# clintpgeorge/LDAGroupedGibbsSampler

Measured on AMD Instinct MI355X. Metric: M tokens sampled/sec (whole node) per Gibbs sweep at K=100, higher is better.
Workload: dtype f64

## Files before the change

include/ggs_hip.h:

```cpp
#ifndef GGS_HIP_H
#define GGS_HIP_H

#include <stdint.h>

#ifdef __cplusplus
extern "C" {
#endif

#define GGS_ABI_VERSION 6

typedef struct ggs_handle ggs_handle;

enum {
  GGS_OK = 0,
  GGS_ERR_NEGATIVE_COUNT = 1,
  GGS_ERR_INVALID_TOPIC = 2,
  GGS_ERR_RNG_EXHAUSTED = 3,
  GGS_ERR_BAD_ARG = 4,
  GGS_ERR_HIP = 5,
  GGS_ERR_STATE = 6,
  GGS_ERR_UNSUPPORTED = 7,
  GGS_ERR_INVARIANT = 8
};

// ... 38 lines not shown
} ggs_config;

typedef struct ggs_timings {
  double theta_ms;
  double z_ms;
  double merge_ms;
  double phi_ms;
  int64_t sweeps;
  int64_t tokens_sampled;
  double exchange_ms;
  double exchange_rs_ms;
  double exchange_ag_ms;
} ggs_timings;

int ggs_create(const ggs_config *cfg, ggs_handle **out);
void ggs_destroy(ggs_handle *h);
const char *ggs_last_error(const ggs_handle *h);
int ggs_abi_version(void);
int ggs_set_stream(ggs_handle *h, void *hip_stream);

int ggs_set_corpus(ggs_handle *h, int64_t num_docs, const int64_t *doc_ptr ,
                   const int32_t *tokens , int64_t doc_base, int64_t tok_base);
int ggs_init_z_java_lcg(ggs_handle *h, int32_t seed);
int ggs_java_lcg_next_ints(int32_t seed, int32_t bound, int64_t n, int32_t *out);
int ggs_set_z(ggs_handle *h, const int32_t *z , int32_t redraw_phi);
int ggs_init_phi(ggs_handle *h);
int ggs_set_iteration(ggs_handle *h, int32_t iteration);
int ggs_get_iteration(const ggs_handle *h, int32_t *iteration);

int ggs_sweep(ggs_handle *h, int32_t n_sweeps);
int ggs_sweep_begin(ggs_handle *h);
int ggs_sweep_end(ggs_handle *h);
int ggs_sweep_end_async(ggs_handle *h);
int ggs_collapsed_serial_sweep(ggs_handle *h, int32_t java_seed, int32_t n_sweeps);
int ggs_sample_z_given_phi(ggs_handle *h, int32_t n_sweeps);
int ggs_counts_device_ptr(ggs_handle *h, void **dev_ptr, int64_t *num_elems);
int ggs_set_global_token_count(ggs_handle *h, int64_t n_tokens);
int ggs_synchronize(ggs_handle *h);

typedef struct ggs_exchange_ops {
  int32_t struct_size;
  int32_t reserved;
  void *ctx;
  int (*reduce_scatter_i32)(void *ctx, const void *send, void *recv, int64_t recv_count, void *hip_stream);
  int (*all_gather_f64)(void *ctx, const void *send, void *recv, int64_t send_count, void *hip_stream);
  int (*all_gather_i32)(void *ctx, const void *send, void *recv, int64_t send_count, void *hip_stream);
  int (*all_to_all_v_i32)(void *ctx, const void *send, const int64_t *send_offsets, const int64_t *send_counts, void *recv,
                          const int64_t *recv_offsets, const int64_t *recv_counts, void *hip_stream);
} ggs_exchange_ops;
#define GGS_EXCHANGE_OPS_V3_SIZE ((int32_t)(sizeof(ggs_exchange_ops) - sizeof(void *)))
int ggs_attach_exchange(ggs_handle *h, int32_t rank, int32_t nranks, const ggs_exchange_ops *ops);
#define GGS_RCCL_UNIQUE_ID_BYTES 128
int ggs_rccl_unique_id(void *out_id );
int ggs_attach_rccl(ggs_handle *h, int32_t rank, int32_t nranks, const void *unique_id);
int ggs_attach_rccl_comm(ggs_handle *h, int32_t rank, int32_t nranks, void *nccl_comm);
int ggs_group_create(const ggs_config *cfg, int32_t n, const int32_t *device_ids, ggs_handle **out_handles );
void ggs_group_destroy(ggs_handle **handles, int32_t n);
int ggs_group_set_z(ggs_handle **handles, int32_t n, const int32_t *const *z , int32_t redraw_phi);
int ggs_group_sweep(ggs_handle **handles, int32_t n, int32_t n_sweeps);
int ggs_group_adopt(ggs_handle **handles, int32_t n);
int ggs_group_gather_counts(ggs_handle **handles, int32_t n);
int ggs_attach_null_exchange(ggs_handle *h, int32_t rank, int32_t nranks);
int ggs_set_count_exchange(ggs_handle *h, int32_t mode);
int ggs_get_count_exchange(const ggs_handle *h, int32_t *sparse, int64_t *pairs_last, int64_t *cells);
int ggs_get_exchange_info(const ggs_handle *h, int32_t *rank, int32_t *nranks, int32_t *k_begin, int32_t *k_end);
int ggs_get_exchange_provider(const ggs_handle *h, int32_t *provider, int32_t *comm_nranks, int32_t *comm_rank);

int ggs_get_z(ggs_handle *h, int32_t *z );
int ggs_get_type_topic_counts(ggs_handle *h, int32_t *n_wk );
int ggs_get_topic_totals(ggs_handle *h, int32_t *n_k );
int ggs_get_phi(ggs_handle *h, double *phi );
int ggs_set_phi(ggs_handle *h, const double *phi );
int ggs_get_phi_mean(ggs_handle *h, double *phi_mean , int32_t *n_sampled);
int ggs_get_theta(ggs_handle *h, int64_t doc_begin, int64_t doc_end, double *theta );
int ggs_get_doc_topic_counts(ggs_handle *h, int64_t doc_begin, int64_t doc_end, int32_t *n_dk);
int ggs_get_timings(ggs_handle *h, ggs_timings *out);
int ggs_reset_timings(ggs_handle *h);
int ggs_check_invariants(ggs_handle *h);
int ggs_get_launch_info(ggs_handle *h, int64_t *num_chunks, int32_t *lds_bytes_z, int32_t *docs_per_block_theta);
int ggs_get_num_hot_words(ggs_handle *h, int32_t *num_hot);
int ggs_get_warm_tiers(ggs_handle *h, int32_t *tiers, int32_t *warm_words, int32_t *docs_per_chunk);
int ggs_get_z_parts(ggs_handle *h, int32_t *parts);
int ggs_get_z_form(ggs_handle *h, int32_t *kernel, int32_t *form, int32_t *calibrated);
int ggs_debug_philox(int32_t device_id, int64_t n, const uint32_t *ctr , const uint32_t *key , uint32_t *out );
int ggs_debug_math(int32_t device_id, int32_t op , int64_t n, const double *x, const double *y, double *out);
int ggs_debug_draw(int32_t device_id, int32_t kind , uint64_t seed, uint32_t iteration,
                   uint32_t purpose, uint64_t elem0, int64_t n, const double *shape, double *out, int32_t *status);
int ggs_debug_poisson(int32_t device_id, double beta, int32_t threshold, uint64_t seed, uint32_t iteration, uint32_t purpose, uint64_t elem0,
                      int64_t n, const int32_t *counts, int32_t *out);
int ggs_debug_alias(int32_t device_id, int32_t V, int32_t K, const double *phi, const double *alpha, double *ps, int32_t *a, double *type_norm);
int ggs_get_alias_tables(ggs_handle *h, double *ps , int32_t *a , double *type_norm );
int ggs_set_topic_priors(ggs_handle *h, int64_t n_zero, const int32_t *topic, const int32_t *word);
int ggs_get_topic_priors(ggs_handle *h, double *priors );
int ggs_get_mh_stats(ggs_handle *h, int64_t out[3]);
int ggs_get_word_topic_lists(ggs_handle *h, int32_t *nw , int32_t *topics );
int ggs_get_sparse_stats(ggs_handle *h, int64_t out[4]);
int ggs_set_variable_selection_prior(ggs_handle *h, double pi);
int ggs_get_vs_stats(ggs_handle *h, int64_t out[3]);
int ggs_debug_vs_indicators(int32_t device_id, int32_t V, int32_t K, const int32_t *counts, const double *prev_phi, double beta, double pi, uint64_t seed,
                            uint32_t iteration, const double *u , uint8_t *drawn_out, int32_t *s_end, int32_t *rounds);
int ggs_model_log_likelihood(ggs_handle *h, double *doc_side, double *topic_side);
int ggs_log_posterior(ggs_handle *h, double *doc_side, double *topic_side);
int ggs_min_doc_distances(ggs_handle *h, const double *other , int64_t n_other, double *min_dist );
int ggs_min_topic_distance(ggs_handle *h, double *min_dist);
#define GGS_TOP_WORDS 0
#define GGS_TOP_RELEVANCE 1
#define GGS_TOP_DISTINCTIVE 2
#define GGS_TOP_SALIENT 3
#define GGS_TOP_K1 4
#define GGS_TOP_WORDS_MAX 128
int ggs_top_words(ggs_handle *h, int32_t kind, int32_t n_words, double lambda, int32_t *idx , double *score );
#define GGS_TOPIC_DIAGNOSTICS_MAX_TOPICS 3072
#define GGS_TOPIC_SCORE_ROWS 10
#define GGS_TOPIC_WORD_SCORE_ROWS 4
int ggs_topic_doc_statistics(ggs_handle *h, int32_t n_words, const int32_t *idx , const double *clogc_in ,
                             int32_t *codoc , int32_t *doc_stats , double *clogc_out );
int ggs_topic_scores(ggs_handle *h, int32_t n_words, const int32_t *idx , const int32_t *codoc, const int32_t *doc_stats,
                     const double *clogc, double *topic_scores , double *word_scores );
int ggs_set_test_corpus(ggs_handle *h, int64_t D, const int64_t *doc_ptr , const int32_t *tokens, int64_t doc_base);
int ggs_heldout_log_likelihood(ggs_handle *h, int32_t num_particles, double *doc_ll, double *total);
int ggs_debug_column_sum(int32_t device_id, int32_t V, int32_t K, const double *x , const int32_t *counts ,
                         double beta, double *out );
int ggs_debug_column_sum_guided(int32_t device_id, int32_t V, int32_t K, const double *x, const int32_t *counts, double beta,
                                const double *guess, double *out, double *pref_out, int32_t *n_k_out);
int ggs_debug_min_distances(int32_t device_id, const double *a, int64_t n, const double *b , int64_t m, int64_t len, int32_t element_major,
                            double *min_dist , double *min_sq );
int ggs_debug_topic_summaries(int32_t device_id, int32_t V, int32_t K, const int32_t *counts , double beta, double lambda, int32_t kind,
                              int32_t n_words, int32_t *idx , double *score , double *mass_k ,
                              double *rowsum_w , double *total , double *all_scores );
int ggs_debug_top_words_phases(ggs_handle *h, int32_t kind, int32_t n_words, double lambda, int32_t element_chain, double *ms );

int ggs_debug_topic_doc_statistics(int32_t device_id, int64_t D, const int64_t *doc_ptr, const int32_t *tokens, const int32_t *z, int32_t V, int32_t K,
                                   const double *alpha , int32_t n_words, const int32_t *idx, const double *clogc_in , int32_t *codoc,
                                   int32_t *doc_stats, double *clogc_out);
int ggs_debug_topic_scores(int32_t device_id, int32_t V, int32_t K, const int32_t *counts , double beta, int32_t n_words, const int32_t *idx,
                           const int32_t *codoc, const int32_t *doc_stats, const double *clogc, double *topic_scores, double *word_scores ,
                           int32_t *sorted_ids );
int ggs_debug_topic_diagnostics_phases(ggs_handle *h, int32_t n_words, double *ms );
#ifdef __cplusplus
}
#endif
#endif
```

ldagroupedgibbssampler_amd/_lib.py:

```python
import ctypes as C
import os
import subprocess

_HERE = os.path.dirname(os.path.abspath(__file__))
CSRC = os.path.join(_HERE, "csrc")
LIB_PATH = os.environ.get("GGS_HIP_LIB") or os.path.join(CSRC, "libggs_hip.so")
HEADER_PATH = os.path.join(os.path.dirname(_HERE), "include", "ggs_hip.h")

ABI_VERSION = 6


class GGSConfig(C.Structure):
    _fields_ = [
        ("struct_size", C.c_int32),
        ("num_topics", C.c_int32),
        ("num_types", C.c_int32),
        ("device_id", C.c_int32),
        ("alpha", C.POINTER(C.c_double)),
        ("alpha_scalar", C.c_double),
        ("beta", C.c_double),
        ("seed", C.c_uint64),
        ("flags", C.c_int32),
        ("phi_burn_in", C.c_int32),
        ("phi_mean_thin", C.c_int32),
        ("alias_poisson_threshold", C.c_int32),
    ]


class GGSTimings(C.Structure):
    _fields_ = [
        ("theta_ms", C.c_double),
        ("z_ms", C.c_double),
        ("merge_ms", C.c_double),
        ("phi_ms", C.c_double),
        ("sweeps", C.c_int64),
        ("tokens_sampled", C.c_int64),
        ("exchange_ms", C.c_double),
        ("exchange_rs_ms", C.c_double),
        ("exchange_ag_ms", C.c_double),
    ]


EXCHANGE_CB = C.CFUNCTYPE(C.c_int, C.c_void_p, C.c_void_p, C.c_void_p, C.c_int64, C.c_void_p)


A2AV_CB = C.CFUNCTYPE(C.c_int, C.c_void_p, C.c_void_p, C.POINTER(C.c_int64), C.POINTER(C.c_int64), C.c_void_p, C.POINTER(C.c_int64), C.POINTER(C.c_int64),
                      C.c_void_p)


class GGSExchangeOps(C.Structure):
    _fields_ = [
        ("struct_size", C.c_int32),
        ("reserved", C.c_int32),
        ("ctx", C.c_void_p),
        ("reduce_scatter_i32", EXCHANGE_CB),
        ("all_gather_f64", EXCHANGE_CB),
        ("all_gather_i32", EXCHANGE_CB),
        ("all_to_all_v_i32", A2AV_CB),
    ]


_vp = C.c_void_p
_dp = C.POINTER(C.c_double)
_ip = C.POINTER(C.c_int32)
_lp = C.POINTER(C.c_int64)
_up = C.POINTER(C.c_uint32)

SIGNATURES = {
    "ggs_create": (C.c_int, [C.POINTER(GGSConfig), C.POINTER(_vp)]),
    "ggs_destroy": (None, [_vp]),
    "ggs_last_error": (C.c_char_p, [_vp]),
    "ggs_abi_version": (C.c_int, []),
    "ggs_set_stream": (C.c_int, [_vp, _vp]),
    "ggs_set_corpus": (C.c_int, [_vp, C.c_int64, _lp, _ip, C.c_int64, C.c_int64]),
    "ggs_init_z_java_lcg": (C.c_int, [_vp, C.c_int32]),
    "ggs_java_lcg_next_ints": (C.c_int, [C.c_int32, C.c_int32, C.c_int64, _ip]),
    "ggs_set_z": (C.c_int, [_vp, _ip, C.c_int32]),
    "ggs_init_phi": (C.c_int, [_vp]),
    "ggs_set_iteration": (C.c_int, [_vp, C.c_int32]),
    "ggs_get_iteration": (C.c_int, [_vp, _ip]),
    "ggs_sweep": (C.c_int, [_vp, C.c_int32]),
    "ggs_sweep_begin": (C.c_int, [_vp]),
    "ggs_sweep_end": (C.c_int, [_vp]),
    "ggs_sweep_end_async": (C.c_int, [_vp]),
    "ggs_sample_z_given_phi": (C.c_int, [_vp, C.c_int32]),
    "ggs_collapsed_serial_sweep": (C.c_int, [_vp, C.c_int32, C.c_int32]),
    "ggs_counts_device_ptr": (C.c_int, [_vp, C.POINTER(_vp), _lp]),
    "ggs_set_global_token_count": (C.c_int, [_vp, C.c_int64]),
    "ggs_synchronize": (C.c_int, [_vp]),
    "ggs_get_z": (C.c_int, [_vp, _ip]),
    "ggs_get_type_topic_counts": (C.c_int, [_vp, _ip]),
    "ggs_get_topic_totals": (C.c_int, [_vp, _ip]),
    "ggs_get_phi": (C.c_int, [_vp, _dp]),
    "ggs_set_phi": (C.c_int, [_vp, _dp]),
    "ggs_get_phi_mean": (C.c_int, [_vp, _dp, _ip]),
    "ggs_get_theta": (C.c_int, [_vp, C.c_int64, C.c_int64, _dp]),
    "ggs_get_doc_topic_counts": (C.c_int, [_vp, C.c_int64, C.c_int64, _ip]),
    "ggs_get_timings": (C.c_int, [_vp, C.POINTER(GGSTimings)]),
    "ggs_reset_timings": (C.c_int, [_vp]),
    "ggs_check_invariants": (C.c_int, [_vp]),
    "ggs_get_launch_info": (C.c_int, [_vp, _lp, _ip, _ip]),
    "ggs_get_num_hot_words": (C.c_int, [_vp, _ip]),
    "ggs_get_z_parts": (C.c_int, [_vp, _ip]),
    "ggs_get_z_form": (C.c_int, [_vp, _ip, _ip, _ip]),
    "ggs_get_warm_tiers": (C.c_int, [_vp, _ip, _ip, _ip]),
    "ggs_attach_exchange": (C.c_int, [_vp, C.c_int32, C.c_int32, C.POINTER(GGSExchangeOps)]),
    "ggs_rccl_unique_id": (C.c_int, [_vp]),
    "ggs_attach_rccl": (C.c_int, [_vp, C.c_int32, C.c_int32, _vp]),
    "ggs_attach_rccl_comm": (C.c_int, [_vp, C.c_int32, C.c_int32, _vp]),
    "ggs_group_create": (C.c_int, [C.POINTER(GGSConfig), C.c_int32, _ip, C.POINTER(_vp)]),
    "ggs_group_destroy": (None, [C.POINTER(_vp), C.c_int32]),
    "ggs_group_adopt": (C.c_int, [C.POINTER(_vp), C.c_int32]),
    "ggs_group_set_z": (C.c_int, [C.POINTER(_vp), C.c_int32, C.POINTER(_ip), C.c_int32]),
    "ggs_group_sweep": (C.c_int, [C.POINTER(_vp), C.c_int32, C.c_int32]),
    "ggs_group_gather_counts": (C.c_int, [C.POINTER(_vp), C.c_int32]),
    "ggs_attach_null_exchange": (C.c_int, [_vp, C.c_int32, C.c_int32]),
    "ggs_get_exchange_info": (C.c_int, [_vp, _ip, _ip, _ip, _ip]),
    "ggs_get_exchange_provider": (C.c_int, [_vp, _ip, _ip, _ip]),
    "ggs_set_count_exchange": (C.c_int, [_vp, C.c_int32]),
    "ggs_get_count_exchange": (C.c_int, [_vp, _ip, _lp, _lp]),
    "ggs_debug_philox": (C.c_int, [C.c_int32, C.c_int64, _up, _up, _up]),
    "ggs_debug_math": (C.c_int, [C.c_int32, C.c_int32, C.c_int64, _dp, _dp, _dp]),
    "ggs_debug_draw": (C.c_int, [C.c_int32, C.c_int32, C.c_uint64, C.c_uint32, C.c_uint32, C.c_uint64, C.c_int64,
                                 _dp, _dp, _ip]),
    "ggs_debug_poisson": (C.c_int, [C.c_int32, C.c_double, C.c_int32, C.c_uint64, C.c_uint32, C.c_uint32, C.c_uint64, C.c_int64, _ip, _ip]),
    "ggs_debug_alias": (C.c_int, [C.c_int32, C.c_int32, C.c_int32, _dp, _dp, _dp, _ip, _dp]),
    "ggs_get_alias_tables": (C.c_int, [_vp, _dp, _ip, _dp]),
    "ggs_set_topic_priors": (C.c_int, [_vp, C.c_int64, _ip, _ip]),
    "ggs_get_topic_priors": (C.c_int, [_vp, _dp]),
    "ggs_get_mh_stats": (C.c_int, [_vp, _lp]),
    "ggs_get_word_topic_lists": (C.c_int, [_vp, _ip, _ip]),
    "ggs_get_sparse_stats": (C.c_int, [_vp, _lp]),
    "ggs_set_variable_selection_prior": (C.c_int, [_vp, C.c_double]),
    "ggs_get_vs_stats": (C.c_int, [_vp, _lp]),
    "ggs_debug_vs_indicators": (C.c_int, [C.c_int32, C.c_int32, C.c_int32, _ip, _dp, C.c_double, C.c_double, C.c_uint64, C.c_uint32, _dp,
                                          C.POINTER(C.c_uint8), _ip, _ip]),
    "ggs_model_log_likelihood": (C.c_int, [_vp, _dp, _dp]),
    "ggs_log_posterior": (C.c_int, [_vp, _dp, _dp]),
    "ggs_min_doc_distances": (C.c_int, [_vp, _dp, C.c_int64, _dp]),
    "ggs_min_topic_distance": (C.c_int, [_vp, _dp]),
    "ggs_top_words": (C.c_int, [_vp, C.c_int32, C.c_int32, C.c_double, _ip, _dp]),
    "ggs_topic_doc_statistics": (C.c_int, [_vp, C.c_int32, _ip, _dp, _ip, _ip, _dp]),
    "ggs_topic_scores": (C.c_int, [_vp, C.c_int32, _ip, _ip, _ip, _dp, _dp, _dp]),
    "ggs_set_test_corpus": (C.c_int, [_vp, C.c_int64, _lp, _ip, C.c_int64]),
    "ggs_heldout_log_likelihood": (C.c_int, [_vp, C.c_int32, _dp, _dp]),
    "ggs_debug_column_sum": (C.c_int, [C.c_int32, C.c_int32, C.c_int32, _dp, _ip, C.c_double, _dp]),
    "ggs_debug_column_sum_guided": (C.c_int, [C.c_int32, C.c_int32, C.c_int32, _dp, _ip, C.c_double, _dp, _dp, _dp, _ip]),
    "ggs_debug_min_distances": (C.c_int, [C.c_int32, _dp, C.c_int64, _dp, C.c_int64, C.c_int64, C.c_int32, _dp, _dp]),
    "ggs_debug_top_words_phases": (C.c_int, [_vp, C.c_int32, C.c_int32, C.c_double, C.c_int32, _dp]),
    "ggs_debug_topic_doc_statistics": (C.c_int, [C.c_int32, C.c_int64, _lp, _ip, _ip, C.c_int32, C.c_int32, _dp, C.c_int32, _ip, _dp, _ip, _ip, _dp]),
    "ggs_debug_topic_scores": (C.c_int, [C.c_int32, C.c_int32, C.c_int32, _ip, C.c_double, C.c_int32, _ip, _ip, _ip, _dp, _dp, _dp, _ip]),
    "ggs_debug_topic_diagnostics_phases": (C.c_int, [_vp, C.c_int32, _dp]),
    "ggs_debug_topic_summaries": (C.c_int, [C.c_int32, C.c_int32, C.c_int32, _ip, C.c_double, C.c_double, C.c_int32, C.c_int32, _ip, _dp, _dp, _dp, _dp, _dp]),
}


def build(force=False):
    srcs = [os.path.join(CSRC, f) for f in os.listdir(CSRC) if f.endswith((".hip", ".hpp"))] + [HEADER_PATH]
    if (not force and os.path.exists(LIB_PATH)
            and all(os.path.getmtime(LIB_PATH) >= os.path.getmtime(s) for s in srcs)):
        return LIB_PATH
    subprocess.check_call(["make", "-C", CSRC, "libggs_hip.so"])
    return LIB_PATH


_lib = None


def _share_hip_runtime_with_torch():
    import importlib.util
    import sys
    if "torch" in sys.modules:
        return
    try:
        spec = importlib.util.find_spec("torch")
    except (ImportError, ValueError):
        return
    if spec is None or not spec.origin:
        return
    cand = os.path.join(os.path.dirname(spec.origin), "lib", "libamdhip64.so")
    if os.path.exists(cand):
        C.CDLL(cand, mode=C.RTLD_GLOBAL)


def share_rccl_with_torch():
    import importlib.util
    import sys
    if "torch" in sys.modules:
# ... 29 lines not shown
```

ldagroupedgibbssampler_amd/csrc/ggs_api.hip:

```cpp
#include <hip/hip_runtime.h>

#include <algorithm>
#include <cctype>
#include <cmath>
#include <cstdio>
#include <cstdlib>
#include <cstring>
#include <new>
#include <string>
#include <vector>

#include "ggs_kernels.hpp"
#include "ggs_z_sliced.hpp"
#include "ggs_z_stream.hpp"
#include "ggs_exact_sum.hpp"
#include "ggs_z_pcgs.hpp"
#include "ggs_z_pcgs_wave.hpp"
#include "ggs_z_collapsed.hpp"
#include "ggs_phi_poisson.hpp"
#include "ggs_alias.hpp"
#include "ggs_z_spalias.hpp"
#include "ggs_z_polyaurn_sparse.hpp"
#include "ggs_phi_vs.hpp"
#include "ggs_z_lightpc.hpp"
#include "ggs_z_lightcollapsed.hpp"
#include "ggs_z_lightpcw2.hpp"
#include "ggs_z_adlda.hpp"
#include "ggs_loglik.hpp"
#include "ggs_heldout.hpp"
#include "ggs_exchange.hpp"
#include "ggs_corpus_lists.hpp"
#include "ggs_distances.hpp"
#include "ggs_topic_summaries.hpp"
#include "ggs_topic_diagnostics.hpp"

using namespace ggs;

namespace {

const char *debug_env(const char *name) {
  static const bool enabled = [] { const char *e = std::getenv("GGS_DEBUG"); return e && std::atoi(e) == 1; }();
  return enabled ? std::getenv(name) : nullptr;
}
int64_t debug_shrunk(const char *name, int64_t built_in) {
  const char *e = debug_env(name);
  return e ? std::max<int64_t>(1, std::min<int64_t>(built_in, std::atoll(e))) : built_in;
}

struct Knob {
  bool set = false;
  int v = 0;
  double f = 0;
  explicit Knob(const char *name) { if (const char *e = debug_env(name)) { set = true; v = std::atoi(e); f = std::atof(e); } }
  bool is(int x) const { return set && v == x; }
};
struct Knobs {
  Knob zkernel{"GGS_DEBUG_ZKERNEL"}, group{"GGS_DEBUG_GROUP"}, regck{"GGS_DEBUG_REGCK"}, tworows{"GGS_DEBUG_TWOROWS"}, wpc{"GGS_DEBUG_WPC"};
  Knob phi64{"GGS_DEBUG_PHI64"}, split{"GGS_DEBUG_SPLIT"}, hot{"GGS_DEBUG_HOT"}, tile{"GGS_DEBUG_TILE"};
  Knob warm{"GGS_DEBUG_WARM"}, warm_rows{"GGS_DEBUG_WARM_ROWS"}, warm_fill{"GGS_DEBUG_WARM_FILL"}, warm_cpw{"GGS_DEBUG_WARM_CPW"};
  Knob theta_b{"GGS_DEBUG_THETA_B"}, theta_wgs{"GGS_DEBUG_THETA_WGS"}, zparts{"GGS_DEBUG_ZPARTS"}, beside{"GGS_DEBUG_BESIDE"};
  Knob pcgs_wave{"GGS_DEBUG_PCGS_WAVE"}, pcgs_stream{"GGS_DEBUG_PCGS_STREAM"};
  Knob margin{"GGS_DEBUG_MARGIN"}, replays{"GGS_DEBUG_REPLAYS"}, chain{"GGS_DEBUG_CHAIN"}, guided{"GGS_DEBUG_GUIDED"};
  Knob no_overlap{"GGS_DEBUG_NO_OVERLAP"}, theta_main{"GGS_DEBUG_THETA_MAIN"}, gamma_queue{"GGS_DEBUG_GAMMA_QUEUE"};
  Knob num_cus{"GGS_DEBUG_NUM_CUS"}, vs_global{"GGS_DEBUG_VS_GLOBAL"};
};

constexpr int kThetaBlock = 256;

enum class Scheme { ggs, pcgs, collapsed, polyaurn, spalias, lightpclda, polyaurn_sparse, lightcollapsed, nzvsspalias, adlda, lightpcldaw2 };

struct KernelLaunch {
  const void *fn = nullptr;
  int block = 64, lds = 0, per_cu = 0;
};
struct LaunchPlan {
  int32_t kernel = 0;
  bool sliced() const { return kernel == 1; }
  bool stream() const { return kernel >= 2; }
  KernelLaunch z;
  int32_t tile_tokens = 64;
  bool two_rows = false;
  KernelLaunch cold, hot, warm;
  bool f32 = false;
  bool split = true, split_forced = false;
  int32_t wave_lds = 0, ring_base = 0, hot_wave_lds = 0, warm_wave_lds = 0, hot_pitch = 0, Kp32 = 0;
  int32_t hot_cap = 0, warm_cap = 0, warm_docs = 0;
  int32_t warm_tiers_max = 3, warm_min_fill_pct = 40, warm_min_chunks_per_wave = 3;
  struct ZCfg { int32_t parts = 1, z_per_cu = 0, theta_docs = 0, theta_lds = 0, theta_lds_beside_z = 0; } cfg_plain, cfg_parts;
  bool parts_forced = false;
  KernelLaunch theta;
  int32_t theta_docs_main = 0, theta_lds_main = 0;
  KernelLaunch lane, wave, alias, spalias, lightpc, serial, wordlist, pusparse, countalias, lightcol, lightpcw2;
  KernelLaunch vsbits, vschain, wordmask, nzvs;
  KernelLaunch adhead, adlists, adlda;
  bool wave_forced = false;
  int32_t alias_wpb = 0;
  std::vector<const KernelLaunch *> all() const { return {&z, &cold, &hot, &warm, &theta, &lane, &wave, &alias, &spalias, &lightpc, &serial, &wordlist, &pusparse, &countalias, &lightcol, &lightpcw2, &vsbits, &wordmask, &nzvs, &adlda}; }
};

enum : uint32_t { kHasAlias = 1, kHasTables = 2, kCountForm = 4, kCountsOnly = 8, kHasWordLists = 16, kDoublySparse = 32, kSparseWalk = 64, kHasMh = 128,
                  kPoissonPhi = 256, kSparseStats = 512, kCountTables = 1024, kNoTheta = 2048 };
struct SchemeRow {
  const char *name;
  int32_t flag, refused;
  int32_t z_kernel;
  KernelLaunch LaunchPlan::*entry;
  size_t (*corpus_lds)(int K, int cap);
  const char *invalid_topic;
  uint32_t caps;
};
constexpr const char *kGgsInvalidTopic = "LDAGroupedGibbsSampler: Topic sampled is invalid!";
constexpr int32_t kModelFlags = GGS_FLAG_COLLAPSED | GGS_FLAG_POLYAURN, kLightFlags = kModelFlags | GGS_FLAG_SPALIAS | GGS_FLAG_LIGHTPCLDA | GGS_FLAG_POLYAURN_SPARSE;
constexpr SchemeRow kSchemes[] = {
    {"ggs", 0, 0, 0, nullptr, nullptr, kGgsInvalidTopic, 0},
    {"pcgs", GGS_FLAG_PCGS, 0, 0, nullptr, nullptr, kGgsInvalidTopic, 0},
    {"collapsed", GGS_FLAG_COLLAPSED, 0, 0, nullptr, nullptr, "SimpleLDA: New topic not sampled." , kCountForm},
    {"polyaurn", GGS_FLAG_POLYAURN, 0, 0, nullptr, nullptr, kGgsInvalidTopic, kPoissonPhi},
    {"spalias", GGS_FLAG_SPALIAS, kModelFlags, 6, &LaunchPlan::spalias, spalias_lds_bytes, kGgsInvalidTopic, kHasAlias | kHasTables | kSparseWalk},
    {"lightpclda", GGS_FLAG_LIGHTPCLDA, kModelFlags | GGS_FLAG_SPALIAS, 7, &LaunchPlan::lightpc, nullptr, kGgsInvalidTopic, kHasAlias | kHasTables | kHasMh},
    {"polyaurn_sparse", GGS_FLAG_POLYAURN_SPARSE, kModelFlags | GGS_FLAG_SPALIAS | GGS_FLAG_LIGHTPCLDA, 8, &LaunchPlan::pusparse, spalias_lds_bytes, kGgsInvalidTopic,
     kHasAlias | kHasTables | kHasWordLists | kDoublySparse | kSparseWalk | kPoissonPhi | kSparseStats},
    {"lightcollapsed", GGS_FLAG_LIGHTCOLLAPSED, kLightFlags | GGS_FLAG_PCGS, 9, &LaunchPlan::lightcol, nullptr, "Collapsed Light-LDA: Sampled invalid topic." ,
     kHasTables | kCountForm | kCountsOnly | kHasWordLists | kHasMh | kCountTables},
    {"nzvsspalias", GGS_FLAG_NZVSSPALIAS, kLightFlags | GGS_FLAG_LIGHTCOLLAPSED, 10, &LaunchPlan::nzvs, spalias_lds_bytes, kGgsInvalidTopic,
     kHasAlias | kHasTables | kHasWordLists | kDoublySparse | kSparseWalk | kSparseStats},
    {"adlda", GGS_FLAG_ADLDA, kLightFlags | GGS_FLAG_PCGS | GGS_FLAG_LIGHTCOLLAPSED | GGS_FLAG_NZVSSPALIAS, 11, &LaunchPlan::adlda, adlda_lds_bytes, "ADLDA: New topic not sampled." ,
     kCountForm | kCountsOnly | kHasWordLists | kSparseStats},
    {"lightpcldaw2", GGS_FLAG_LIGHTPCLDAW2, kLightFlags | GGS_FLAG_LIGHTCOLLAPSED | GGS_FLAG_NZVSSPALIAS | GGS_FLAG_ADLDA, 12, &LaunchPlan::lightpcw2, nullptr,
     "Light PC-LDA (Type topic proposal): Sampled invalid topic." , kHasTables | kHasWordLists | kHasMh | kCountTables | kNoTheta},
};
constexpr int kNumSchemes = (int)(sizeof(kSchemes) / sizeof(kSchemes[0]));
static_assert(kNumSchemes == (int)Scheme::lightpcldaw2 + 1, "one row per Scheme, in the enum's order");
constexpr const SchemeRow &row_of(Scheme s) { return kSchemes[(int)s]; }
constexpr bool has(Scheme s, uint32_t cap) { return (row_of(s).caps & cap) != 0; }
constexpr bool pcgs_family(Scheme s) { return row_of(s).flag != 0; }
constexpr bool has_alias(Scheme s) { return has(s, kHasAlias); }
constexpr bool count_form(Scheme s) { return has(s, kCountForm); }
constexpr bool counts_only(Scheme s) { return has(s, kCountsOnly); }
constexpr bool has_tables(Scheme s) { return has(s, kHasTables); }
constexpr bool has_word_lists(Scheme s) { return has(s, kHasWordLists); }
constexpr bool doubly_sparse(Scheme s) { return has(s, kDoublySparse); }
constexpr bool sparse_walk(Scheme s) { return has(s, kSparseWalk); }
constexpr bool has_mh(Scheme s) { return has(s, kHasMh); }
constexpr bool poisson_phi(Scheme s) { return has(s, kPoissonPhi); }
constexpr bool has_sparse_stats(Scheme s) { return has(s, kSparseStats); }
constexpr bool count_tables(Scheme s) { return has(s, kCountTables); }
constexpr bool no_theta(Scheme s) { return has(s, kNoTheta); }
constexpr bool wave_only(Scheme s) { return row_of(s).entry != nullptr; }
std::string needs_flag(const char *fn, uint32_t cap) {
  std::vector<std::string> names;
  for (const SchemeRow &r : kSchemes)
    if (r.caps & cap) { names.push_back("GGS_FLAG_"); for (const char *c = r.name; *c; ++c) names.back() += (char)std::toupper((unsigned char)*c); }
  std::string msg = std::string(fn) + " needs ";
  for (size_t i = 0; i < names.size(); ++i) msg += (i == 0 ? "" : i + 1 == names.size() ? " or " : ", ") + names[i];
  return msg;
}

constexpr int kEvRing = 8;
struct Events {
  hipEvent_t e[6] = {nullptr, nullptr, nullptr, nullptr, nullptr, nullptr};
  hipEvent_t x[3] = {nullptr, nullptr, nullptr};
  hipEvent_t th0 = nullptr, th1 = nullptr;
  bool used_ahead = false, exchanged = false;
  bool e4_is_e3 = false;
  bool theta_on_main = false;
  bool light = false;
// ... 93 lines not shown
  int32_t sum_nseg = 0;
  bool exact_sum = true;
  bool sum_guided = true;
  const void *guess_src = nullptr;
  int32_t guess_cols = 0;
  uint32_t *d_status = nullptr;
  int64_t *d_test_ptr = nullptr;
  int32_t *d_test_tok = nullptr, *d_test_docs = nullptr;
  std::vector<int32_t> test_short, test_long, test_huge;
  void *d_heldout_spill = nullptr;
  size_t heldout_spill_bytes = 0;
  double *d_test_ll = nullptr;
  std::vector<int64_t> test_ptr;
  int64_t test_doc_base = 0;
  bool have_test = false;
  void *d_scratch = nullptr;
  size_t scratch_bytes = 0;

  Exchange *xg = nullptr;
  hipStream_t own_stream = nullptr;
  int32_t Ks = 0, Ksm = 0, k0 = 0;
  int64_t *d_koff = nullptr;
  int32_t *d_cnt_send = nullptr, *d_cnt_own = nullptr, *d_cnt_all = nullptr, *d_n_k_own = nullptr;
  double *d_phi_own = nullptr, *d_phi_all0 = nullptr, *d_phi_all1 = nullptr, *d_mag_own = nullptr;
  int32_t *d_krank = nullptr, *d_kcol = nullptr;
  int32_t seg_split = 0, v_split = 0;
  hipStream_t comm_stream = nullptr;
  hipEvent_t ev_half_drawn = nullptr, ev_half_gathered = nullptr;
  int32_t *d_hseg_word = nullptr, *d_hseg_begin = nullptr, *d_hseg_end = nullptr;
  int64_t HS = 0;
  int32_t detail_every = 4;
  bool force_detail = false;
  int64_t sweeps_enqueued = 0;
  bool have_frac = false;
  double frac[5] = {0, 0, 0, 0, 0};
  int32_t count_mode = 0;
  bool counted_sparse = false;
  bool in_group = false;
  int64_t *d_sp_count = nullptr;
  int32_t *d_sp_cnt32 = nullptr, *d_sp_all = nullptr;
  int32_t *d_sp_wg_count = nullptr;
  int64_t *d_sp_wg_off = nullptr;
  int64_t sp_wgs = 0;
  int32_t *d_sp_send = nullptr, *d_sp_recv = nullptr;
  size_t sp_send_cap = 0, sp_recv_cap = 0;
  int64_t sp_pairs_last = 0;
  bool hot_join_pending = false, hot_counted = false;
  bool z_counted = false;
  bool cnt_send_zeroed = false;
  bool z_counts_forced = false;
  bool z_counts = true;
  SliceMap smap{};
  bool counts_global = true;
  bool cnt_own_valid = false;
  bool n_k_valid = false;
  std::vector<ggs_handle *> group;

  std::vector<void **> owned;
  Events evs[kEvRing];
  int ev_head = 0, ev_pending = 0;
  ggs_timings tm{};
  std::string err;
};

namespace {

int set_err(ggs_handle *h, int code, const std::string &msg) {
  if (h) h->err = msg;
  return code;
}

#define HIP_TRY(h, expr)                                                                       \
  do {                                                                                          \
    hipError_t _e = (expr);                                                                     \
    if (_e != hipSuccess)                                                                       \
      return set_err((h), GGS_ERR_HIP, std::string(#expr) + ": " + hipGetErrorString(_e));      \
  } while (0)

int bind_device(ggs_handle *h) {
  HIP_TRY(h, hipSetDevice(h->device));
  return GGS_OK;
}

template <typename T>
int dev_alloc(ggs_handle *h, T **p, size_t count) {
  void **slot = reinterpret_cast<void **>(p);
  if (std::find(h->owned.begin(), h->owned.end(), slot) == h->owned.end()) h->owned.push_back(slot);
  if (*p) { (void)hipFree(*p); *p = nullptr; }
  HIP_TRY(h, hipMalloc(slot, std::max<size_t>(count, 1) * sizeof(T)));
  return GGS_OK;
}
template <typename T>
int dev_alloc_zeroed(ggs_handle *h, T **p, size_t count) {
  const int rc = dev_alloc(h, p, count);
  if (rc) return rc;
  HIP_TRY(h, hipMemset(*p, 0, sizeof(T) * count));
  return GGS_OK;
}
template <typename T>
int upload(ggs_handle *h, T **p, const T *src, size_t count) {
  const int rc = dev_alloc(h, p, count);
  if (rc) return rc;
  if (count) HIP_TRY(h, hipMemcpy(*p, src, sizeof(T) * count, hipMemcpyHostToDevice));
  return GGS_OK;
}
template <typename T>
int upload(ggs_handle *h, T **p, const std::vector<T> &v) { return upload(h, p, v.data(), v.size()); }

hipError_t launch(const ggs_handle *h, const KernelLaunch &l, int64_t items, void **args, hipStream_t st, int table_lds = 0) {
  const int waves = l.block / 64;
  const int64_t grid = std::max<int64_t>(1, std::min<int64_t>((items + waves - 1) / waves, (int64_t)h->num_cus * l.per_cu));
  return hipLaunchKernel(l.fn, dim3((unsigned)grid), dim3((unsigned)l.block), args, (size_t)(l.lds + table_lds), st);
}

void build_poisson_table(double beta, int32_t L, std::vector<double> &T) {
  const int n = 2 * L;
  T.assign((size_t)L * n, 0.0);
  std::vector<double> S((size_t)n);
  for (int32_t c = 0; c < L; ++c) {
    const double lambda = beta + (double)c;
    double pj = std::exp(-lambda), acc = 0.0;
    for (int j = 0; j < n; ++j) {
      if (j > 0) pj = pj * lambda / (double)j;
      acc += pj;
      S[(size_t)j] = acc;
    }
    for (int j = 0; j < n - 1; ++j) T[(size_t)c * n + j] = S[(size_t)j] / S[(size_t)n - 1];
    T[(size_t)c * n + n - 1] = 1.0;
  }
}

int ensure_scratch(ggs_handle *h, size_t bytes) {
  if (h->scratch_bytes >= bytes) return GGS_OK;
  if (h->d_scratch) (void)hipFree(h->d_scratch);
  h->d_scratch = nullptr; h->scratch_bytes = 0;
  HIP_TRY(h, hipMalloc(&h->d_scratch, bytes));
  h->scratch_bytes = bytes;
  return GGS_OK;
}

int grid_for(int64_t n, int block, int per_thread = 1) {
  const int64_t want = (n + (int64_t)block * per_thread - 1) / ((int64_t)block * per_thread);
  return (int)std::max<int64_t>(1, std::min<int64_t>(want, 256 * 8));
}

int check_status(ggs_handle *h) {
  uint32_t st = 0;
  HIP_TRY(h, hipMemcpyAsync(&st, h->d_status, sizeof st, hipMemcpyDeviceToHost, h->stream));
  HIP_TRY(h, hipStreamSynchronize(h->stream));
  if (!st) return GGS_OK;
  HIP_TRY(h, hipMemsetAsync(h->d_status, 0, sizeof(uint32_t), h->stream));
  if (st & ST_INVALID_TOPIC) return set_err(h, GGS_ERR_INVALID_TOPIC, row_of(h->scheme).invalid_topic);
  if (st & ST_NEGATIVE_COUNT) return set_err(h, GGS_ERR_NEGATIVE_COUNT, "Negative count for topic (Invalid count!)");
  if (st & ST_BAD_SHAPE) return set_err(h, GGS_ERR_BAD_ARG, "alpha and beta must be strictly positive (gamma shape <= 0)");
  if (st & ST_INVARIANT) return set_err(h, GGS_ERR_INVARIANT, "Inconsistent Indicator probability");
  return set_err(h, GGS_ERR_RNG_EXHAUSTED, "a gamma rejection loop exceeded GGS_MAX_BLOCKS Philox blocks");
}

int launch_permute_z(ggs_handle *h) {
  if (h->N > 0)
    hipLaunchKernelGGL(permute_z_kernel, dim3(grid_for(h->N, 256)), dim3(256), 0, h->stream, h->d_perm, h->d_z, h->d_zw, h->N);
  HIP_TRY(h, hipGetLastError());
  return GGS_OK;
}

bool use_sparse(const ggs_handle *h) {
// ... 163 lines not shown
  HIP_TRY(h, hipStreamSynchronize(h->stream));
  h->cnt_own_valid = true;
  return GGS_OK;
}
int launch_count_rebuild(ggs_handle *h);
int exchange_reduce_scatter(ggs_handle *h) {
  if (h->cnt_own_valid) return GGS_OK;
  if (use_sparse(h) != h->counted_sparse) {
    int rc = launch_count_rebuild(h);
    if (rc) return rc;
  }
  if (use_sparse(h)) return sparse_exchange(h);
  int rc = xcall(h, h->xg->ops.reduce_scatter_i32(h->xg->ops.ctx, h->d_cnt_send, h->d_cnt_own, (int64_t)h->V * h->Ksm, h->stream), "reduce_scatter_i32");
  if (rc) return rc;
  h->cnt_own_valid = true;
  h->cnt_send_zeroed = false;
  return GGS_OK;
}
int clear_send_buffer_if_dead(ggs_handle *h, hipStream_t on) {
  if (!h->xg || h->cnt_send_zeroed || !h->cnt_own_valid || use_sparse(h)) return GGS_OK;
  return clear_send_buffer(h, on);
}

int gather_counts_step_gather(ggs_handle *h) {
  const size_t cells = (size_t)h->xg->nranks * h->V * h->Ksm;
  int rc;
  if (!h->d_cnt_all && (rc = dev_alloc(h, &h->d_cnt_all, cells))) return rc;
  return xcall(h, h->xg->ops.all_gather_i32(h->xg->ops.ctx, h->d_cnt_own, h->d_cnt_all, (int64_t)h->V * h->Ksm, h->stream), "all_gather_i32");
}
int gather_counts_step_unslice(ggs_handle *h) {
  hipLaunchKernelGGL(counts_unslice_kernel, dim3(grid_for((int64_t)h->K * h->V, 256)), dim3(256), 0, h->stream, h->d_cnt_all, h->d_koff, h->Ksm, h->d_n_wk,
                     h->K, h->V);
  HIP_TRY(h, hipGetLastError());
  h->counts_global = true; h->n_k_valid = false;
  return GGS_OK;
}
int ensure_global_counts(ggs_handle *h) {
  if (!h->xg || h->counts_global) return GGS_OK;
  int rc;
  if ((rc = exchange_reduce_scatter(h)) || (rc = clear_send_buffer_if_dead(h, h->stream)) || (rc = gather_counts_step_gather(h))) return rc;
  return gather_counts_step_unslice(h);
}

int launch_magnitude(ggs_handle *h) {
  int rc = ensure_global_counts(h);
  if (rc) return rc;
  if (h->n_k_valid) return GGS_OK;
  if ((rc = launch_magnitude_on(h, h->d_n_wk, h->K, h->K, h->d_mag, h->d_n_k))) return rc;
  h->n_k_valid = true;
  return GGS_OK;
}

bool conditional_phi(const ggs_handle *h, bool initial) { return h->have_priors && !initial; }
bool vs_phi(const ggs_handle *h, bool initial) { return h->scheme == Scheme::nzvsspalias && !initial; }
void vs_note_draw(ggs_handle *h, bool initial) {
  if (h->scheme == Scheme::nzvsspalias) { h->vs_lists = initial ? ggs_handle::VsLists::empty : ggs_handle::VsLists::drawn; if (initial) h->vs_drawn = false; }
}
int launch_vs_chain(ggs_handle *h, const int32_t *cnt, int32_t cnt_pitch, int32_t Ks, int32_t k0, const int32_t *n_k) {
  if (Ks <= 0) return GGS_OK;
  VsBitsParams bp{};
  bp.cnt = cnt; bp.phiT = h->d_phiT; bp.cz = h->d_vs_cz; bp.pz = h->d_vs_pz;
  bp.cnt_pitch = cnt_pitch; bp.Kp = h->Kp; bp.k0 = k0; bp.Ks = Ks; bp.V = h->V; bp.W = h->vs_W;
  void *bargs[] = {&bp};
  HIP_TRY(h, launch(h, h->plan.vsbits, (int64_t)h->vs_W * ((Ks + 63) / 64), bargs, h->stream));
  VsChainParams cp{};
  cp.cz = h->d_vs_cz; cp.pz = h->d_vs_pz; cp.und = h->d_vs_und; cp.work = h->d_vs_work; cp.n_k = n_k; cp.u = nullptr;
  cp.s_end = h->d_vs_s_end; cp.rounds = h->d_vs_rounds; cp.status = h->d_status; cp.seed = h->seed; cp.iteration = (uint32_t)h->iteration;
  cp.Ks = Ks; cp.k0 = k0; cp.V = h->V; cp.W = h->vs_W; cp.beta = h->beta; cp.odds = h->vs_pi / (1 - h->vs_pi);
  void *cargs[] = {&cp};
  HIP_TRY(h, hipLaunchKernel(h->plan.vschain.fn, dim3((unsigned)Ks), dim3(kVsBlock), cargs, (size_t)h->plan.vschain.lds, h->stream));
  hipLaunchKernelGGL(vs_mask_kernel, dim3(grid_for((int64_t)h->V * h->vs_pitch, 256)), dim3(256), 0, h->stream, h->d_vs_und, h->vs_W, k0, Ks, h->V, h->vs_pitch,
                     h->d_vs_mask);
  HIP_TRY(h, hipGetLastError());
  h->vs_drawn = true;
  return GGS_OK;
}
int launch_sum_phi(ggs_handle *h) {
  launch_column_sum<double, false>(h, h->d_phiT, h->Kp, h->K, h->d_pr_sum_phi, nullptr, false, false, h->d_pr_pref, h->d_pr_fn);
  HIP_TRY(h, hipGetLastError());
  return GGS_OK;
}
int phi_apply_priors(ggs_handle *h) {
  hipLaunchKernelGGL(phi_apply_priors_kernel, dim3(grid_for((int64_t)h->K * h->V, 256, 2)), dim3(256), 0, h->stream, h->d_phiT, h->d_pr_mask, h->pr_pitch, h->K,
                     h->Kp, h->V, h->d_phiT32, h->plan.Kp32);
  HIP_TRY(h, hipGetLastError());
  h->alias_stale = true;
  return GGS_OK;
}

int phi_slice_gamma(ggs_handle *h, bool initial, const int32_t *cnt, int32_t cnt_pitch, int32_t Ks, int32_t k0, double *out, int32_t out_pitch,
                    const double *mag, int32_t seg0, int32_t seg1) {
  if (Ks <= 0 || seg1 <= seg0) return GGS_OK;
  PhiGammaParams gp{};
  gp.n_wk = cnt; gp.mag = mag; gp.phiT = out; gp.status = h->d_status;
  gp.seed = h->seed; gp.iteration = (uint32_t)h->iteration;
  gp.purpose = initial ? GGS_PURPOSE_INIT_PHI : GGS_PURPOSE_PHI;
  gp.K = Ks; gp.Kp = out_pitch; gp.V = h->V; gp.cnt_pitch = cnt_pitch; gp.k0 = k0; gp.beta = h->beta;
  gp.prior_pm = (1.0 / (double)h->V) * ((double)h->V * h->beta);
  gp.initial = initial ? 1 : 0;
  const int64_t want_tiles = (int64_t)h->num_cus * 4 * 4;
  int kc_cap = (int)std::min<int64_t>(kPhiCols, std::max<int64_t>(2, (int64_t)Ks * (seg1 - seg0) / want_tiles));
  if (const char *e = debug_env("GGS_DEBUG_PHICOLS")) kc_cap = std::max(1, std::min(kPhiCols, std::atoi(e)));
  gp.ncg = (Ks + kc_cap - 1) / kc_cap;
  gp.kc = (Ks + gp.ncg - 1) / gp.ncg;
  gp.ncg = (Ks + gp.kc - 1) / gp.kc;
  gp.seg_begin = seg0; gp.seg_end = seg1;
  gp.queue_cap = std::min(kPhiQueue, h->gamma_queue_cap);
  gp.prio = h->xg ? 1 : 0;
  gp.guess = h->exact_sum ? h->d_sum_pref : nullptr; gp.fn = h->d_sum_fn;
  const int64_t tiles = (int64_t)(seg1 - seg0) * gp.ncg;
  const dim3 grid((unsigned)std::min<int64_t>(tiles, (int64_t)h->num_cus * 32));
  if (conditional_phi(h, initial)) {
    gp.zero_mask = h->d_pr_mask; gp.mask_pitch = h->pr_pitch;
    hipLaunchKernelGGL(phi_gamma_kernel<true>, grid, dim3(64), 0, h->stream, gp);
  } else if (vs_phi(h, initial)) {
    gp.zero_mask = h->d_vs_mask; gp.mask_pitch = h->vs_pitch;
    gp.undrawn_negative = h->xg ? 1 : 0;
    hipLaunchKernelGGL(phi_gamma_vs_kernel, grid, dim3(64), 0, h->stream, gp);
  } else {
    hipLaunchKernelGGL(phi_gamma_kernel<false>, grid, dim3(64), 0, h->stream, gp);
  }
  HIP_TRY(h, hipGetLastError());
  return GGS_OK;
}
int phi_slice_total(ggs_handle *h, const double *out, int32_t out_pitch, int32_t Ks, double *tot) {
  if (Ks <= 0) return GGS_OK;
  if (h->exact_sum) {
    SumParams sp{};
    sp.src = out; sp.guess = h->d_sum_pref; sp.fn = h->d_sum_fn; sp.out = tot; sp.beta = h->beta; sp.n_k = nullptr;
    sp.pitch = out_pitch; sp.K = Ks; sp.V = h->V; sp.nseg = h->sum_nseg; sp.write_pref = 0;
    hipLaunchKernelGGL((sum_walk_kernel<double, false>), dim3((unsigned)Ks), dim3(64), 0, h->stream, sp);
  } else {
    launch_column_sum<double, false>(h, out, out_pitch, Ks, tot, nullptr, false, false);
  }
  HIP_TRY(h, hipGetLastError());
  return GGS_OK;
}
int phi_slice_poisson(ggs_handle *h, bool initial, const int32_t *cnt, int32_t cnt_pitch, int32_t Ks, int32_t k0, double *out, int32_t out_pitch,
                      int32_t seg0, int32_t seg1, bool first) {
  if (Ks <= 0) return GGS_OK;
  if (first) HIP_TRY(h, hipMemsetAsync(h->d_pa_acc, 0, sizeof(unsigned long long) * kPoissonAccStride * (size_t)Ks, h->stream));
  if (seg1 <= seg0) return GGS_OK;
  PhiPoissonParams pp{};
  pp.cnt = cnt; pp.out = out; pp.table = h->d_pa_table; pp.acc = h->d_pa_acc; pp.status = h->d_status;
  pp.seed = h->seed; pp.iteration = (uint32_t)h->iteration; pp.purpose = initial ? GGS_PURPOSE_INIT_PHI : GGS_PURPOSE_PHI;
  pp.Ks = Ks; pp.out_pitch = out_pitch; pp.cnt_pitch = cnt_pitch; pp.k0 = k0; pp.V = h->V;
  pp.row_begin = seg0 * kSumSegRows; pp.row_end = std::min(h->V, seg1 * kSumSegRows);
  pp.L = h->pa_L; pp.beta = h->beta; pp.t00 = h->pa_t00;
  const int64_t rows = pp.row_end - pp.row_begin, cells = rows * Ks;
  const int64_t want = std::max<int64_t>(kPoissonThreads, cells / ((int64_t)h->num_cus * 8));
  pp.rows_per_tile = (int32_t)std::max<int64_t>(1, std::min<int64_t>(rows, (want + Ks - 1) / Ks));
  const int64_t tiles = (rows + pp.rows_per_tile - 1) / pp.rows_per_tile;
  hipLaunchKernelGGL(phi_poisson_kernel, dim3((unsigned)std::min<int64_t>(tiles, (int64_t)h->num_cus * 2)), dim3(kPoissonThreads), (size_t)Ks * 12, h->stream, pp);
  HIP_TRY(h, hipGetLastError());
  return GGS_OK;
}
int phi_slice_poisson_totals(ggs_handle *h, int32_t Ks, double *tot, int32_t *n_k) {
  if (Ks <= 0) return GGS_OK;
  hipLaunchKernelGGL(phi_poisson_totals_kernel, dim3((unsigned)((Ks + 255) / 256)), dim3(256), 0, h->stream, h->d_pa_acc, Ks, tot, n_k);
  HIP_TRY(h, hipGetLastError());
  return GGS_OK;
}
int launch_phi_slice(ggs_handle *h, bool initial, const int32_t *cnt, int32_t cnt_pitch, int32_t Ks, int32_t k0, double *out, int32_t out_pitch,
                     double *mag, double *tot, int32_t *n_k, double *phi_mean) {
  if (Ks <= 0) return GGS_OK;
  int rc;
  if (poisson_phi(h->scheme)) {
    if ((rc = phi_slice_poisson(h, initial, cnt, cnt_pitch, Ks, k0, out, out_pitch, 0, h->sum_nseg, true)) || (rc = phi_slice_poisson_totals(h, Ks, tot, n_k)))
      return rc;
    hipLaunchKernelGGL(phi_normalise_polyaurn_kernel, dim3(grid_for((int64_t)Ks * h->V, 256, 2)), dim3(256), 0, h->stream, out, tot, Ks, out_pitch, h->V,
                       phi_mean, out == h->d_phiT ? h->d_phiT32 : nullptr, h->plan.Kp32);
    HIP_TRY(h, hipGetLastError());
    return GGS_OK;
  }
  if ((rc = launch_magnitude_on(h, cnt, cnt_pitch, Ks, mag, n_k)) || (vs_phi(h, initial) && (rc = launch_vs_chain(h, cnt, cnt_pitch, Ks, k0, n_k))) ||
      (rc = phi_slice_gamma(h, initial, cnt, cnt_pitch, Ks, k0, out, out_pitch, mag, 0, h->sum_nseg)) || (rc = phi_slice_total(h, out, out_pitch, Ks, tot)))
    return rc;
  if (vs_phi(h, initial))
    hipLaunchKernelGGL(phi_normalise_polyaurn_kernel, dim3(grid_for((int64_t)Ks * h->V, 256, 2)), dim3(256), 0, h->stream, out, tot, Ks, out_pitch, h->V,
                       static_cast<double *>(nullptr), out == h->d_phiT ? h->d_phiT32 : nullptr, h->plan.Kp32);
  else if (conditional_phi(h, initial))
    hipLaunchKernelGGL(phi_normalise_conditional_kernel, dim3(grid_for((int64_t)Ks * h->V, 256, 2)), dim3(256), 0, h->stream, out, tot, h->d_pr_sum_phi, Ks,
                       out_pitch, h->V, phi_mean, out == h->d_phiT ? h->d_phiT32 : nullptr, h->plan.Kp32);
  else
    hipLaunchKernelGGL(phi_normalise_kernel, dim3(grid_for((int64_t)Ks * h->V, 256, 2)), dim3(256), 0, h->stream, out, tot, Ks, out_pitch, h->V, phi_mean,
                       out == h->d_phiT ? h->d_phiT32 : nullptr, h->plan.Kp32);
  HIP_TRY(h, hipGetLastError());
  return GGS_OK;
}

size_t half0_elems(const ggs_handle *h) { return (size_t)h->v_split * h->Ksm; }
size_t half1_elems(const ggs_handle *h) { return (size_t)(h->V - h->v_split) * h->Ksm + (size_t)h->Ksm; }
int phi_step_a(ggs_handle *h) { return exchange_reduce_scatter(h); }
int phi_step_a_clear(ggs_handle *h) { return h->seg_split > 0 ? GGS_OK : clear_send_buffer_if_dead(h, h->stream); }
int phi_step_b1(ggs_handle *h, bool initial) {
  int rc;
  if (conditional_phi(h, initial) && (rc = launch_sum_phi(h))) return rc;
  if (poisson_phi(h->scheme)) {
    if ((rc = phi_slice_poisson(h, initial, h->d_cnt_own, h->Ksm, h->Ks, h->k0, h->d_phi_own, h->Ksm, 0, h->seg_split, true))) return rc;
  } else if ((rc = launch_magnitude_on(h, h->d_cnt_own, h->Ksm, h->Ks, h->d_mag_own, h->d_n_k_own))) {
    return rc;
  }
  if (vs_phi(h, initial) && (rc = launch_vs_chain(h, h->d_cnt_own, h->Ksm, h->Ks, h->k0, h->d_n_k_own))) return rc;
  if (h->seg_split > 0) {
    if (!poisson_phi(h->scheme) && (rc = phi_slice_gamma(h, initial, h->d_cnt_own, h->Ksm, h->Ks, h->k0, h->d_phi_own, h->Ksm, h->d_mag_own, 0, h->seg_split))) return rc;
    HIP_TRY(h, hipEventRecord(h->ev_half_drawn, h->stream));
    HIP_TRY(h, hipStreamWaitEvent(h->comm_stream, h->ev_half_drawn, 0));
  }
  return GGS_OK;
}
int phi_step_g0(ggs_handle *h) {
  if (h->seg_split <= 0) return GGS_OK;
  return xcall(h, h->xg->ops.all_gather_f64(h->xg->ops.ctx, h->d_phi_own, h->d_phi_all0, (int64_t)half0_elems(h), h->comm_stream), "all_gather_f64");
}
int phi_step_b2(ggs_handle *h, bool initial) {
  int rc;
  if (h->seg_split > 0) {
    if ((rc = clear_send_buffer_if_dead(h, h->comm_stream))) return rc;
    HIP_TRY(h, hipEventRecord(h->ev_half_gathered, h->comm_stream));
  }
  if (poisson_phi(h->scheme)) {
    if ((rc = phi_slice_poisson(h, initial, h->d_cnt_own, h->Ksm, h->Ks, h->k0, h->d_phi_own, h->Ksm, h->seg_split, h->sum_nseg, false))) return rc;
    return phi_slice_poisson_totals(h, h->Ks, h->d_phi_own + (size_t)h->V * h->Ksm, h->d_n_k_own);
  }
  if ((rc = phi_slice_gamma(h, initial, h->d_cnt_own, h->Ksm, h->Ks, h->k0, h->d_phi_own, h->Ksm, h->d_mag_own, h->seg_split, h->sum_nseg))) return rc;
  return phi_slice_total(h, h->d_phi_own, h->Ksm, h->Ks, h->d_phi_own + (size_t)h->V * h->Ksm);
}
int phi_step_g1(ggs_handle *h) {
  return xcall(h, h->xg->ops.all_gather_f64(h->xg->ops.ctx, h->d_phi_own + half0_elems(h), h->d_phi_all1, (int64_t)half1_elems(h), h->stream), "all_gather_f64");
}
int phi_join_halves(ggs_handle *h) {
  if (h->seg_split > 0) HIP_TRY(h, hipStreamWaitEvent(h->stream, h->ev_half_gathered, 0));
  return GGS_OK;
}
int phi_step_c(ggs_handle *h, bool initial, bool accumulate_mean) {
  PhiRepackParams rp{};
  rp.all0 = h->d_phi_all0; rp.all1 = h->d_phi_all1; rp.krank = h->d_krank; rp.kcol = h->d_kcol; rp.phiT = h->d_phiT;
  rp.phi_mean = accumulate_mean ? h->d_phi_mean : nullptr;
  rp.c0 = (int64_t)half0_elems(h); rp.c1 = (int64_t)half1_elems(h); rp.K = h->K; rp.Kp = h->Kp; rp.V = h->V; rp.Ksm = h->Ksm; rp.v_split = h->v_split;
  rp.phiT32 = h->d_phiT32; rp.Kp32 = h->plan.Kp32; rp.sum_phi = h->d_pr_sum_phi;
  if (vs_phi(h, initial)) {
    rp.phi_mean = nullptr;
    hipLaunchKernelGGL(vs_mask_gathered_kernel, dim3(grid_for((int64_t)h->V * h->vs_pitch, 256)), dim3(256), 0, h->stream, rp, h->d_vs_mask, h->vs_pitch);
    hipLaunchKernelGGL(phi_repack_vs_kernel, dim3(grid_for((int64_t)h->K * h->V, 256, 2)), dim3(256), 0, h->stream, rp);
  } else if (poisson_phi(h->scheme)) hipLaunchKernelGGL(phi_repack_polyaurn_kernel, dim3(grid_for((int64_t)h->K * h->V, 256, 2)), dim3(256), 0, h->stream, rp);
  else if (conditional_phi(h, initial)) hipLaunchKernelGGL(phi_repack_conditional_kernel, dim3(grid_for((int64_t)h->K * h->V, 256, 2)), dim3(256), 0, h->stream, rp);
  else hipLaunchKernelGGL(phi_repack_kernel, dim3(grid_for((int64_t)h->K * h->V, 256, 2)), dim3(256), 0, h->stream, rp);
  HIP_TRY(h, hipGetLastError());
  h->have_phi = true;
  h->alias_stale = true;
  vs_note_draw(h, initial);
  if (h->have_priors && initial) return phi_apply_priors(h);
  return GGS_OK;
}

int launch_alias_build(ggs_handle *h) {
  if (!has_alias(h->scheme)) return GGS_OK;
  AliasParams ap{};
  ap.phiT = h->d_phiT; ap.alpha = h->d_alpha; ap.ps = h->d_alias_ps; ap.a = h->d_alias_a; ap.type_norm = h->d_alias_tn;
  ap.V = h->V; ap.K = h->K; ap.Kp = h->Kp; ap.wpb = h->plan.alias_wpb;
  void *args[] = {&ap};
  HIP_TRY(h, launch(h, h->plan.alias, ((int64_t)h->V + ap.wpb - 1) / ap.wpb, args, h->stream));
  if (h->scheme == Scheme::nzvsspalias && h->vs_lists == ggs_handle::VsLists::empty) {
    HIP_TRY(h, hipMemsetAsync(h->d_nw, 0, (size_t)h->V * sizeof(int32_t), h->stream));
  } else if (doubly_sparse(h->scheme)) {
    const bool from_mask = h->vs_lists == ggs_handle::VsLists::drawn;
    WordListParams wp{};
    wp.phiT = h->d_phiT; wp.nzw = h->d_nzw; wp.nw = h->d_nw; wp.V = h->V; wp.K = h->K; wp.Kp = h->Kp;
    wp.zero_mask = h->d_vs_mask; wp.mask_pitch = h->vs_pitch;
    void *wargs[] = {&wp};
    HIP_TRY(h, launch(h, from_mask ? h->plan.wordmask : h->plan.wordlist, h->V, wargs, h->stream));
  }
  h->alias_stale = false;
  return GGS_OK;
}

int launch_count_alias_build(ggs_handle *h) {
  CountAliasParams cp{};
  cp.n_wk = h->d_n_wk; cp.n_k = h->d_n_k; cp.ps = h->d_alias_ps; cp.a = h->d_alias_a; cp.type_norm = h->d_alias_tn;
  cp.nzw = h->d_nzw; cp.nw = h->d_nw; cp.tpt = h->d_tpt; cp.beta_sum = h->beta * (double)h->V;
  cp.V = h->V; cp.K = h->K; cp.wpb = h->plan.alias_wpb;
  void *args[] = {&cp};
  HIP_TRY(h, launch(h, h->plan.countalias, ((int64_t)h->V + cp.wpb - 1) / cp.wpb, args, h->stream));
  return GGS_OK;
}

int launch_adlda_head(ggs_handle *h) {
  AdldaHeadParams hp{};
  hp.n_k = h->d_n_k; hp.alpha = h->d_alpha; hp.den0 = h->d_ad_den0; hp.s0 = h->d_ad_s0; hp.beta = h->beta; hp.beta_sum = h->beta * (double)h->V; hp.K = h->K;
  void *hargs[] = {&hp};
  HIP_TRY(h, launch(h, h->plan.adhead, 1, hargs, h->stream));
  WordListParams wp{};
  wp.counts = h->d_n_wk; wp.nzw = h->d_nzw; wp.nw = h->d_nw; wp.V = h->V; wp.K = h->K; wp.Kp = h->Kp;
  void *wargs[] = {&wp};
  HIP_TRY(h, launch(h, h->plan.adlists, h->V, wargs, h->stream));
  return GGS_OK;
}

int launch_sweep_head(ggs_handle *h) {
  const int rc = launch_magnitude(h);
  if (rc) return rc;
  if (count_tables(h->scheme)) return launch_count_alias_build(h);
  if (h->scheme == Scheme::adlda) return launch_adlda_head(h);
  hipLaunchKernelGGL(psi_kernel, dim3(grid_for((int64_t)h->K * h->V, 256, 2)), dim3(256), 0, h->stream, h->d_n_wk, h->d_n_k, h->beta, h->beta * (double)h->V, h->d_phiT,
                     h->K, h->Kp, h->V);
  HIP_TRY(h, hipGetLastError());
  return GGS_OK;
}

int launch_phi(ggs_handle *h, bool initial, bool accumulate_mean, Events *E = nullptr) {
  int rc;
  if (h->xg) {
    if ((rc = phi_step_a(h)) || (rc = phi_step_a_clear(h))) return rc;
    if (E) HIP_TRY(h, hipEventRecord(E->x[0], h->stream));
    if ((rc = phi_step_b1(h, initial)) || (rc = phi_step_g0(h)) || (rc = phi_step_b2(h, initial))) return rc;
    if (E) HIP_TRY(h, hipEventRecord(E->x[1], h->stream));
    if ((rc = phi_join_halves(h)) || (rc = phi_step_g1(h))) return rc;
    if (E) HIP_TRY(h, hipEventRecord(E->x[2], h->stream));
    if ((rc = phi_step_c(h, initial, accumulate_mean))) return rc;
    return launch_alias_build(h);
  }
  if (conditional_phi(h, initial) && (rc = launch_sum_phi(h))) return rc;
  if ((rc = launch_phi_slice(h, initial, h->d_n_wk, h->K, h->K, 0, h->d_phiT, h->Kp, h->d_mag, h->d_tot, h->d_n_k, accumulate_mean ? h->d_phi_mean : nullptr)))
// ... 32 lines not shown
    case 15: return reinterpret_cast<const void *>(KERNEL<120>);   case 16: return reinterpret_cast<const void *>(KERNEL<128>);     \
    case 17: return reinterpret_cast<const void *>(KERNEL<136>);   case 18: return reinterpret_cast<const void *>(KERNEL<144>);     \
    case 19: return reinterpret_cast<const void *>(KERNEL<152>);   case 20: return reinterpret_cast<const void *>(KERNEL<160>);     \
    case 21: return reinterpret_cast<const void *>(KERNEL<168>);   case 22: return reinterpret_cast<const void *>(KERNEL<176>);     \
    case 23: return reinterpret_cast<const void *>(KERNEL<184>);   default: return reinterpret_cast<const void *>(KERNEL<192>);     \
  }
const void *sliced_kernel_for(int K) { GGS_KMAX_SWITCH(z_sliced_kernel) }
const void *sliced32_kernel_for(int K) { GGS_KMAX_SWITCH(z_sliced32_kernel) }

const void *hot_kernel_for(int K) { GGS_KMAX_SWITCH(z_hot_kernel) }
const void *warm_kernel_for(int K) { GGS_KMAX_SWITCH(z_warm_kernel) }
const void *pcgs_kernel_for(int K) { GGS_KMAX_SWITCH(pcgs_sliced_kernel) }
const void *polyaurn_kernel_for(int K) { GGS_KMAX_SWITCH(polyaurn_sliced_kernel) }
const void *collapsed_kernel_for(int K) {
  switch ((K + 7) / 8) {
#define GGS_CK(N) case N: return reinterpret_cast<const void *>(pcgs_sliced_kernel<8 * N, true>);
    GGS_CK(1) GGS_CK(2) GGS_CK(3) GGS_CK(4) GGS_CK(5) GGS_CK(6) GGS_CK(7) GGS_CK(8) GGS_CK(9) GGS_CK(10) GGS_CK(11) GGS_CK(12)
    GGS_CK(13) GGS_CK(14) GGS_CK(15) GGS_CK(16) GGS_CK(17) GGS_CK(18) GGS_CK(19) GGS_CK(20) GGS_CK(21) GGS_CK(22) GGS_CK(23)
#undef GGS_CK
    default: return reinterpret_cast<const void *>(pcgs_sliced_kernel<192, true>);
  }
}

const void *pcgs_wave_kernel_for(int nb, bool collapsed, bool polyaurn) {
#define GGS_WK(N) if (nb <= N) return polyaurn ? reinterpret_cast<const void *>(polyaurn_wave_kernel<N>) : collapsed ? reinterpret_cast<const void *>(pcgs_wave_kernel<N, true>) : reinterpret_cast<const void *>(pcgs_wave_kernel<N, false>);
  GGS_WK(1) GGS_WK(2) GGS_WK(4) GGS_WK(8) GGS_WK(16)
#undef GGS_WK
  return polyaurn ? reinterpret_cast<const void *>(polyaurn_wave_kernel<32>) : collapsed ? reinterpret_cast<const void *>(pcgs_wave_kernel<32, true>) : reinterpret_cast<const void *>(pcgs_wave_kernel<32, false>);
}
constexpr int kPcgsWaveMaxTopics = 32 * 128;
constexpr int kPcgsWaveFromTopics = 176, kCollapsedWaveFromTopics = 96;
constexpr int kPolyaurnWaveFromTopics = 168;

const void *tile_kernel_for(int K) {
  const int nt = (K + 63) / 64;
  return nt <= 1 ? reinterpret_cast<const void *>(z_kernel<1>) : nt <= 2 ? reinterpret_cast<const void *>(z_kernel<2>)
       : nt <= 4 ? reinterpret_cast<const void *>(z_kernel<4>) : nt <= 8 ? reinterpret_cast<const void *>(z_kernel<8>)
       : nt <= 16 ? reinterpret_cast<const void *>(z_kernel<16>) : reinterpret_cast<const void *>(z_kernel<20>);
}
const void *stream_kernel_for(bool two_pass, bool regck, int group) {
  if (two_pass) return reinterpret_cast<const void *>(z_stream_kernel);
  if (!regck) return reinterpret_cast<const void *>(z_stream1_kernel<false, 4>);
  return group == 1 ? reinterpret_cast<const void *>(z_stream1_kernel<true, 1>) : group == 2 ? reinterpret_cast<const void *>(z_stream1_kernel<true, 2>)
                                                                                             : reinterpret_cast<const void *>(z_stream1_kernel<true, 4>);
}
const void *pcgs_lane_kernel_for(int K, bool sliced, bool collapsed, bool polyaurn) {
  if (sliced) return collapsed ? collapsed_kernel_for(K) : polyaurn ? polyaurn_kernel_for(K) : pcgs_kernel_for(K);
  return collapsed ? reinterpret_cast<const void *>(pcgs_z_kernel<true>) : polyaurn ? reinterpret_cast<const void *>(polyaurn_z_kernel) : reinterpret_cast<const void *>(pcgs_z_kernel<false>);
}

int resident_waves_per_cu(const void *fn, int lds) {
  int by_regs = 0;
  if (hipOccupancyMaxActiveBlocksPerMultiprocessor(&by_regs, fn, 64, (size_t)lds) != hipSuccess || by_regs < 1) by_regs = 1;
  return lds_workgroups_per_cu(lds, std::min(by_regs, 32));
}

int plan_launches(const int K, const int V, const Scheme scheme, const Knobs &kn, LaunchPlan &pl) {
  const int Kp = (K + 1) & ~1, pitch16 = (Kp / 2) | 1;
  if (scheme == Scheme::ggs) {
    const bool sliced_ok = K <= kSlicedMaxTopics && V < (1 << kSlotShift);
    bool sliced = sliced_ok && K <= kSlicedDefaultTopics, stream = !sliced && K > 2 * kSliceTopics, two_pass = false;
    if (kn.zkernel.set) {
      const int mode = kn.zkernel.v;
      sliced = sliced_ok && mode == 1;
      stream = (mode == 2 || mode == 3) ? K > 2 * kSliceTopics : (stream && mode != 0);
      two_pass = mode == 3;
      if (sliced) stream = false;
    }
    pl.kernel = sliced ? 1 : stream ? (two_pass ? 3 : 2) : 0;
    if (stream) {
      const int ns = stream_slices(K);
      int group = ns <= kRegCheckpoints ? 1 : ns <= 2 * kRegCheckpoints ? 2 : 4;
      if (kn.group.set && (kn.group.v == 1 || kn.group.v == 2 || kn.group.v == 4)) group = kn.group.v;
      bool regck = !two_pass && z_stream1_groups(K, group) <= kRegCheckpoints;
      if (kn.regck.set) regck = regck && kn.regck.v != 0;
      if (!regck) group = 4;
      pl.two_rows = !two_pass && (kn.tworows.set ? kn.tworows.v != 0 : K <= 512);
      pl.z.fn = stream_kernel_for(two_pass, regck, group);
      pl.z.lds = two_pass ? z_stream_lds_bytes(K) : z_stream1_lds_bytes(K, group, pl.two_rows, regck);
      if (pl.z.lds > kMaxLdsBytes) return GGS_ERR_UNSUPPORTED;
    } else if (sliced) {
      pl.f32 = !kn.phi64.is(1);
      pl.Kp32 = round_up(K, kSlice32Topics);
      pl.ring_base = sliced_ring_base(K); pl.wave_lds = sliced_wave_lds(K); pl.hot_pitch = table_row_pitch(K);
      pl.hot_wave_lds = hot_wave_lds(K); pl.warm_wave_lds = warm_wave_lds(K);
      if (kn.split.set) { pl.split = kn.split.v != 0; pl.split_forced = kn.split.v == 2; }
      pl.hot_cap = pl.split ? table_rows_beside_cold(K, pl.hot_wave_lds) : table_rows_fused(K);
      if (kn.hot.set) pl.hot_cap = std::max(0, std::min(pl.hot_cap, kn.hot.v));
      pl.cold = {pl.f32 ? sliced32_kernel_for(K) : sliced_kernel_for(K), kSlicedWaves * 64, sliced_cold_lds(K), 1};
      pl.hot = {hot_kernel_for(K), kSlicedWaves * 64, table_lds(K, pl.hot_wave_lds, 0), 1};
      pl.warm = {warm_kernel_for(K), kSlicedWaves * 64, table_lds(K, pl.warm_wave_lds, 0), 1};
      pl.warm_docs = warm_docs_for(sliced_kmax(K));
      pl.warm_cap = table_rows_beside_cold(K, pl.warm_wave_lds);
      if (pl.warm_cap < 16) pl.warm_cap = 0;
      if (kn.warm.set) pl.warm_tiers_max = std::max(0, std::min(kWarmMaxTiers, kn.warm.v));
      if (kn.warm_rows.set) pl.warm_cap = std::max(0, std::min(pl.warm_cap, kn.warm_rows.v));
      if (kn.warm_fill.set) pl.warm_min_fill_pct = std::max(1, std::min(100, kn.warm_fill.v));
      if (kn.warm_cpw.set) pl.warm_min_chunks_per_wave = std::max(0, kn.warm_cpw.v);
    } else {
      int T = z_tile_rows_in(kMaxLdsBytes / 6 / kLdsGranule * kLdsGranule, Kp, pitch16);
      if (kn.tile.set) T = kn.tile.v;
      pl.tile_tokens = std::max(8, std::min(64, T));
      pl.z.fn = tile_kernel_for(K);
      pl.z.lds = z_tile_lds_bytes(Kp, pitch16, pl.tile_tokens);
      if (pl.z.lds > kMaxLdsBytes) return GGS_ERR_UNSUPPORTED;
    }
    if (!sliced) {
      pl.z.per_cu = lds_workgroups_per_cu(pl.z.lds, 8);
      if (kn.wpc.set) pl.z.per_cu = std::max(1, kn.wpc.v);
    }
  }
  const int theta_quarter = (kMaxLdsBytes - 24 * 1024) / 4;
  int B = 64;
  while (B > 1 && (theta_cells_lds_bytes(K, B) > 32 * 1024 || (B > 16 && theta_lds_bytes(K, B) > theta_quarter))) B >>= 1;
  if (theta_lds_bytes(K, B) > kMaxLdsBytes) return GGS_ERR_UNSUPPORTED;
  pl.theta.fn = reinterpret_cast<const void *>(theta_kernel<kThetaBlock>); pl.theta.block = kThetaBlock;
  pl.cfg_plain = {1, pl.z.per_cu, B, std::max(theta_lds_bytes(K, B), theta_quarter), 0};
  pl.theta_docs_main = kn.theta_b.set ? std::max(1, std::min(B, kn.theta_b.v)) : std::min(B, 16);
  pl.theta_lds_main = std::max(theta_lds_bytes(K, pl.theta_docs_main), (kMaxLdsBytes - 24 * 1024) / (kn.theta_wgs.set ? std::max(1, kn.theta_wgs.v) : 5));
  pl.cfg_parts = pl.cfg_plain;
  if (scheme == Scheme::ggs) {
    pl.parts_forced = kn.zparts.set;
    int parts = kn.zparts.set ? std::max(1, std::min(8, kn.zparts.v)) : pl.kernel == 2 ? 8 : 1;
    if (parts > 1 && pl.kernel == 2) {
      const int kBeside = kn.beside.set ? std::max(1, kn.beside.v) : 4;
      const int z_alloc = lds_alloc_of(pl.z.lds);
      auto z_waves_beside = [&](int theta_lds) { return std::min(pl.z.per_cu, (kMaxLdsBytes - kLdsGranule - kBeside * lds_alloc_of(theta_lds)) / z_alloc); };
      int Bt = 64;
      while (Bt > 1 && theta_cells_lds_bytes(K, Bt) > 10 * 1024) Bt >>= 1;
      const int zw = z_waves_beside(theta_cells_lds_bytes(K, Bt));
      const int t_lds = theta_lds_bytes(K, Bt);
      if (theta_cells_lds_bytes(K, Bt) <= 12 * 1024 && zw >= 2)
        pl.cfg_parts = {parts, zw, Bt, std::max(t_lds, theta_quarter), std::max(t_lds, (kMaxLdsBytes - kLdsGranule - zw * z_alloc) / kBeside / kLdsGranule * kLdsGranule)};
      else
        parts = 1;
    }
    pl.cfg_parts.parts = parts;
    return GGS_OK;
  }

  const bool collapsed = scheme == Scheme::collapsed, polyaurn = scheme == Scheme::polyaurn;
  if (K <= kPcgsWaveMaxTopics) {
    const int nb = pcgs_wave_blocks(Kp);
    pl.wave.fn = pcgs_wave_kernel_for(nb, collapsed, polyaurn);
    pl.wave.lds = pcgs_wave_lds_bytes(nb);
    pl.wave.per_cu = resident_waves_per_cu(pl.wave.fn, pl.wave.lds);
  }
  pl.wave_forced = kn.pcgs_wave.set ? kn.pcgs_wave.v != 0 : K > (collapsed ? kCollapsedWaveFromTopics : polyaurn ? kPolyaurnWaveFromTopics : kPcgsWaveFromTopics);
  if (pl.wave_forced && !pl.wave.fn) return GGS_ERR_UNSUPPORTED;
  const bool lane_sliced = K <= kSlicedMaxTopics && !(kn.pcgs_stream.set && kn.pcgs_stream.v != 0);
  pl.lane.lds = lane_sliced ? pcgs_sliced_lds_bytes(K) : pcgs_z_lds_bytes(K);
  if (pl.lane.lds > kMaxLdsBytes && !pl.wave_forced) return GGS_ERR_UNSUPPORTED;
  pl.lane.per_cu = lds_workgroups_per_cu(pl.lane.lds, 8);
  if (!pl.wave_forced) pl.lane.fn = pcgs_lane_kernel_for(K, lane_sliced, collapsed, polyaurn);
  if (collapsed) pl.serial.fn = reinterpret_cast<const void *>(collapsed_serial_kernel);
  if (has_alias(scheme)) {
    pl.alias_wpb = alias_words_per_block(K);
    pl.alias = {reinterpret_cast<const void *>(alias_build_kernel), 64, (int)alias_lds_bytes(K, pl.alias_wpb), 0};
    pl.alias.per_cu = lds_workgroups_per_cu(pl.alias.lds, 16);
  }
  if (doubly_sparse(scheme)) pl.wordlist = {reinterpret_cast<const void *>(word_list_build_kernel), kWordListBlock, 0, 8};
  if (scheme == Scheme::spalias) pl.spalias.fn = reinterpret_cast<const void *>(spalias_wave_kernel);
  if (scheme == Scheme::polyaurn_sparse) pl.pusparse.fn = reinterpret_cast<const void *>(polyaurn_sparse_wave_kernel);
  if (scheme == Scheme::nzvsspalias) {
    pl.wordmask = {reinterpret_cast<const void *>(word_list_mask_kernel), kWordListBlock, 0, 8};
    pl.vsbits = {reinterpret_cast<const void *>(vs_bits_kernel), 64, 0, 32};
// ... 9 lines not shown
  if (count_tables(scheme)) {
    pl.alias_wpb = alias_words_per_block(K);
    pl.countalias = {reinterpret_cast<const void *>(count_alias_build_kernel), 64, (int)count_alias_lds_bytes(K, pl.alias_wpb), 0};
    pl.countalias.per_cu = lds_workgroups_per_cu(pl.countalias.lds, 16);
  }
  if (scheme == Scheme::lightpcldaw2) {
    pl.lightpcw2 = {reinterpret_cast<const void *>(lightpcw2_wave_kernel), 64, (int)light_lds_bytes(K), 0};
    pl.lightpcw2.per_cu = resident_waves_per_cu(pl.lightpcw2.fn, pl.lightpcw2.lds);
  }
  if (scheme == Scheme::lightcollapsed) {
    pl.lightcol = {reinterpret_cast<const void *>(lightcollapsed_wave_kernel), 64, (int)light_lds_bytes(K), 0};
    pl.lightcol.per_cu = resident_waves_per_cu(pl.lightcol.fn, pl.lightcol.lds);
  }
  if (scheme == Scheme::adlda) {
    pl.adhead = {reinterpret_cast<const void *>(adlda_head_kernel), 64, 0, 1};
    pl.adlists = {reinterpret_cast<const void *>(word_list_counts_kernel), kWordListBlock, 0, 8};
    pl.adlda.fn = reinterpret_cast<const void *>(adlda_wave_kernel);
  }
  return GGS_OK;
}

const KernelLaunch &pcgs_entry(const LaunchPlan &pl, Scheme s, bool wave) {
  return row_of(s).entry ? pl.*row_of(s).entry : wave ? pl.wave : pl.lane;
}
int launch_pcgs_z(ggs_handle *h) {
  if (h->N == 0) return GGS_OK;
  PcgsParams pp{};
  pp.tok = h->d_tok; pp.inv_perm = h->d_inv_perm; pp.z = h->d_z; pp.zw = h->d_zw; pp.doc_ptr = h->d_doc_ptr; pp.order = h->d_order;
  pp.alpha = h->d_alpha; pp.phiT = h->d_phiT; pp.status = h->d_status;
  pp.num_docs = h->pcgs_order_len; pp.tok_base = h->tok_base; pp.seed = h->seed; pp.iteration = (uint32_t)h->iteration;
  pp.K = h->K; pp.Kp = h->Kp;
  int rc;
  if (h->alias_stale && (rc = launch_alias_build(h))) return rc;
  if (count_form(h->scheme)) {
    if ((rc = launch_sweep_head(h))) return rc;
    pp.n_wk = h->d_n_wk; pp.n_k = h->d_n_k; pp.beta = h->beta; pp.beta_sum = h->beta * (double)h->V;
  } else if (count_tables(h->scheme)) {
    if ((rc = launch_sweep_head(h))) return rc;
    pp.n_wk = h->d_n_wk; pp.n_k = h->d_n_k; pp.beta = h->beta; pp.beta_sum = h->beta * (double)h->V;
  }
  PolyaurnSparseParams sp{};
  LightCountParams lp{};
  AdldaParams ad{};
  void *args[] = {&pp, &h->margin_scale};
  if (sparse_walk(h->scheme)) {
    sp.b = pp; sp.ps = h->d_alias_ps; sp.a = h->d_alias_a; sp.type_norm = h->d_alias_tn; sp.cap = h->sp_cap; sp.margin_scale = h->margin_scale;
    sp.nzw = h->d_nzw; sp.nw = h->d_nw; sp.stats = h->d_ps_stats;
    args[0] = static_cast<SpaliasParams *>(&sp);
  } else if (has_mh(h->scheme)) {
    lp.b = pp; lp.ps = h->d_alias_ps; lp.a = h->d_alias_a; lp.mh = h->d_mh; lp.alpha_sum = h->alpha_sum;
    lp.nzw = h->d_nzw; lp.nw = h->d_nw; lp.tpt = h->d_tpt;
    args[0] = static_cast<LightpcParams *>(&lp);
  } else if (h->scheme == Scheme::adlda) {
    ad.b = pp; ad.den0 = h->d_ad_den0; ad.s0 = h->d_ad_s0; ad.nzw = h->d_nzw; ad.nw = h->d_nw; ad.stats = h->d_ps_stats; ad.cap = h->sp_cap; ad.margin_scale = h->margin_scale;
    args[0] = &ad;
  }
  HIP_TRY(h, launch(h, h->pcgs_z, h->pcgs_items, args, h->stream));
  return GGS_OK;
}

bool z_counts_itself(const ggs_handle *h) {
  return h->xg && h->z_counts && h->plan.sliced() && (h->z_counts_forced || h->N <= (int64_t)64 * h->V) && !use_sparse(h);
}
int launch_count_hot(ggs_handle *h);
int launch_z(ggs_handle *h, bool force_fused = false, int64_t c0 = 0, int64_t c1 = -1, bool count = false, bool defer_join = false) {
  h->hot_join_pending = false;
  if (h->N == 0) return GGS_OK;
  const LaunchPlan &pl = h->plan;
  ZParams zp{};
  zp.tok = h->d_tok; zp.inv_perm = h->d_inv_perm; zp.z = h->d_z; zp.zw = h->d_zw; zp.chunk_start = h->d_chunk_start; zp.chunk_doc = h->d_chunk_doc; zp.chunk_len = h->d_chunk_len;
  zp.theta = h->d_theta; zp.phiT = h->d_phiT; zp.status = h->d_status;
  zp.tok_base = h->tok_base; zp.seed = h->seed; zp.iteration = (uint32_t)h->iteration;
  zp.K = h->K; zp.Kp = h->Kp; zp.pitch16 = h->pitch16; zp.tile_tokens = pl.tile_tokens;
  zp.margin_scale = h->margin_scale;
  zp.chunk_doc1 = h->d_chunk_doc1; zp.two_rows = (pl.two_rows && h->d_chunk_doc1) ? 1 : 0;
  zp.ct_tok = h->d_ct_tok; zp.ct_idx = h->d_ct_idx; zp.ct_ip = h->d_ct_ip; zp.c_docs = h->d_c_docs; zp.num_cold = h->Cc;
  zp.hot_words = h->d_hot_words; zp.num_hot = h->num_hot; zp.hot_pitch = pl.hot_pitch;
  zp.wave_lds = pl.wave_lds; zp.hot_off = kSlicedWaves * pl.wave_lds; zp.ring_base = pl.ring_base;
  zp.cnt_send = (count && z_counts_itself(h)) ? h->d_cnt_send : nullptr;
  zp.smap = h->smap;
  zp.ht_pack = reinterpret_cast<const int4 *>(h->d_ht_pack); zp.h_docs = h->d_h_docs;
  zp.wt_pack = reinterpret_cast<const int4 *>(h->d_wt_pack); zp.w_docs = h->d_w_docs; zp.warm_words = h->d_warm_words;
  zp.warm_meta = h->d_warm_meta; zp.warm_tiers = h->warm_tiers; zp.warm_rows = pl.warm_cap;
  zp.phiT32 = h->d_phiT32; zp.Kp32 = pl.Kp32; zp.replays = h->d_replays; zp.margin_scale32 = h->margin_scale32;
  void *args[] = {&zp};
  if (!pl.sliced()) {
    if (c1 < 0) c1 = h->C;
    if (c1 <= c0) return GGS_OK;
    zp.chunk_start += c0; zp.chunk_doc += c0; zp.chunk_len += c0; zp.num_chunks = c1 - c0;
    if (zp.chunk_doc1) zp.chunk_doc1 += c0;
    KernelLaunch z = pl.z;
    z.per_cu = h->cfg->z_per_cu;
    HIP_TRY(h, launch(h, z, zp.num_chunks, args, h->stream));
    return GGS_OK;
  }
  zp.num_chunks = h->Cs;
  const int hot_rows_lds = h->num_hot * pl.hot_pitch;
  ZParams wp = zp;
  wp.wave_lds = pl.warm_wave_lds; wp.hot_off = kSlicedWaves * pl.warm_wave_lds;
  void *wargs[] = {&wp};
  auto launch_warm = [&](hipStream_t st) { return h->Cw == 0 ? hipSuccess : launch(h, pl.warm, h->warm_chunks_max, wargs, st, h->warm_rows_max * pl.hot_pitch); };
  if (h->z_split && !force_fused && h->Cs > h->Cc && h->Cc > 0) {
    ZParams hp = zp;
    hp.wave_lds = pl.hot_wave_lds; hp.hot_off = kSlicedWaves * pl.hot_wave_lds;
    void *hargs[] = {&hp};
    if (h->hot_fork_from) {
      HIP_TRY(h, hipStreamWaitEvent(h->side_hot, h->hot_fork_from, 0));
    } else {
      HIP_TRY(h, hipEventRecord(h->ev_hot_fork, h->stream));
      HIP_TRY(h, hipStreamWaitEvent(h->side_hot, h->ev_hot_fork, 0));
    }
    zp.num_chunks = h->Cc; zp.num_hot = 0;
    HIP_TRY(h, launch(h, pl.cold, h->Cc, args, h->stream));
    HIP_TRY(h, launch(h, pl.hot, h->Cs - h->Cc, hargs, h->side_hot, hot_rows_lds));
    HIP_TRY(h, launch_warm(h->side_hot));
    if (defer_join && zp.cnt_send) {
      hipStream_t main_stream = h->stream;
      h->stream = h->side_hot;
      const int rc = launch_count_hot(h);
      h->stream = main_stream;
      if (rc) return rc;
      h->hot_counted = true;
    }
    HIP_TRY(h, hipEventRecord(h->ev_hot_join, h->side_hot));
    if (defer_join) h->hot_join_pending = true;
    else HIP_TRY(h, hipStreamWaitEvent(h->stream, h->ev_hot_join, 0));
  } else {
    HIP_TRY(h, launch(h, pl.cold, std::max(h->Cc, h->Cs - h->Cc), args, h->stream, hot_rows_lds));
    HIP_TRY(h, launch_warm(h->stream));
  }
  if (pl.f32) ++h->z_f32_launches;
  return GGS_OK;
}

bool sample_phi_this_iteration(const ggs_handle *h) {
  return h->phi_burn_in > 0 && h->iteration > h->phi_burn_in && (h->iteration % h->phi_thin) == 0;
}

uint64_t java_lcg_next_ints(int32_t seed, int32_t bound, int64_t n, int32_t *out) {
  constexpr uint64_t kMult = 0x5DEECE66DULL, kMask = (1ULL << 48) - 1;
  uint64_t s = ((uint64_t)(int64_t)seed ^ kMult) & kMask;
  auto next31 = [&]() { s = (s * kMult + 0xBULL) & kMask; return (int32_t)(s >> 17); };
  const int32_t m = bound - 1;
  for (int64_t i = 0; i < n; ++i) {
    int32_t r = next31();
    if ((bound & m) == 0) r = (int32_t)(((int64_t)bound * (int64_t)r) >> 31);
    else
      for (int32_t u = r;; u = next31()) {
        r = u % bound;
        if ((int32_t)((uint32_t)u - (uint32_t)r + (uint32_t)m) >= 0) break;
      }
    out[i] = r;
  }
  return s;
}

int require_ready(ggs_handle *h, bool need_phi) {
  if (!h) return GGS_ERR_BAD_ARG;
  if (!h->have_corpus) return set_err(h, GGS_ERR_STATE, "no corpus: call ggs_set_corpus first");
  if (need_phi && !h->have_phi) return set_err(h, GGS_ERR_STATE, "no Phi: call ggs_init_phi / ggs_set_z / ggs_set_phi first");
  return bind_device(h);
}

int drop_theta_ahead(ggs_handle *h) {
  if (h->side) HIP_TRY(h, hipStreamSynchronize(h->side));
  h->theta_ahead_iter = INT64_MIN;
  return GGS_OK;
// ... 308 lines not shown
  return r;
}

int scheme_of(const ggs_config *cfg, Scheme &scheme, int32_t &poisson_L) {
  const int32_t f = cfg->flags;
  scheme = Scheme::ggs;
  for (int i = 0; i < kNumSchemes; ++i) {
    if (!(f & kSchemes[i].flag)) continue;
    if (f & kSchemes[i].refused) return GGS_ERR_BAD_ARG;
    scheme = (Scheme)i;
  }
  poisson_L = cfg->alias_poisson_threshold == 0 ? 100 : cfg->alias_poisson_threshold;
  if (poisson_phi(scheme) && ((f & GGS_FLAG_COLLAPSED) || poisson_L < 1 || poisson_L > kPoissonMaxThreshold)) return GGS_ERR_BAD_ARG;
  if (wave_only(scheme) && cfg->num_topics > kPcgsWaveMaxTopics) return GGS_ERR_UNSUPPORTED;
  return GGS_OK;
}

}

extern "C" {

int ggs_abi_version(void) { return GGS_ABI_VERSION; }

const char *ggs_last_error(const ggs_handle *h) { return h ? h->err.c_str() : "null handle"; }

int ggs_create(const ggs_config *cfg, ggs_handle **out) {
  if (!cfg || !out) return GGS_ERR_BAD_ARG;
  *out = nullptr;
  if (cfg->struct_size != (int32_t)sizeof(ggs_config)) return GGS_ERR_BAD_ARG;
  if (cfg->num_topics <= 0 || cfg->num_types <= 0 || !(cfg->beta > 0)) return GGS_ERR_BAD_ARG;
  Scheme scheme = Scheme::ggs; int32_t poisson_L = 0;
  if (const int rc = scheme_of(cfg, scheme, poisson_L)) return rc;
  int ndev = 0;
  if (hipGetDeviceCount(&ndev) != hipSuccess || ndev <= 0 || cfg->device_id < 0 || cfg->device_id >= ndev) return GGS_ERR_HIP;
  ggs_handle *h = new (std::nothrow) ggs_handle();
  if (!h) return GGS_ERR_HIP;
  const Knobs kn;
  h->K = cfg->num_topics; h->V = cfg->num_types; h->device = cfg->device_id;
  h->Ks = h->Ksm = h->K; h->k0 = 0;
  h->Kp = (h->K + 1) & ~1;
  h->pitch16 = (h->Kp / 2) | 1;
  h->beta = cfg->beta; h->seed = cfg->seed; h->flags = cfg->flags;
  h->scheme = scheme; h->pa_L = poisson_L;
  h->phi_burn_in = cfg->phi_burn_in; h->phi_thin = cfg->phi_mean_thin > 0 ? cfg->phi_mean_thin : 1;
  h->alpha.assign(h->K, cfg->alpha_scalar);
  if (cfg->alpha) std::copy(cfg->alpha, cfg->alpha + h->K, h->alpha.begin());
  for (double a : h->alpha)
    if (!(a > 0)) { delete h; return GGS_ERR_BAD_ARG; }
  for (double a : h->alpha) h->alpha_sum = h->alpha_sum + a;
  h->alpha_symmetric = std::all_of(h->alpha.begin(), h->alpha.end(), [&](double a) { return std::memcmp(&a, &h->alpha[0], sizeof a) == 0; });
  if (kn.margin.set) { h->margin_scale = std::max(1.0, kn.margin.f); h->margin_scale32 = std::max(0.0, kn.margin.f); }
  if (kn.chain.set) h->exact_sum = kn.chain.v == 0;
  if (kn.guided.set) h->sum_guided = kn.guided.v != 0;
  if (kn.no_overlap.set) h->overlap_theta = kn.no_overlap.v == 0;
  if (kn.theta_main.set) { h->theta_main = kn.theta_main.v != 0; h->theta_main_always = kn.theta_main.v == 2; }
  if (kn.gamma_queue.set) h->gamma_queue_cap = std::max(0, kn.gamma_queue.v);
  h->sum_nseg = (h->V + kSumSegRows - 1) / kSumSegRows;

  int rc = GGS_OK;
  auto bail = [&](int code) { ggs_destroy(h); return code; };
  if (hipSetDevice(h->device) != hipSuccess) return bail(GGS_ERR_HIP);
  {
    hipDeviceProp_t prop;
    if (hipGetDeviceProperties(&prop, h->device) != hipSuccess) return bail(GGS_ERR_HIP);
    h->num_cus = prop.multiProcessorCount > 0 ? prop.multiProcessorCount : 256;
    if (kn.num_cus.set) h->num_cus = std::max(1, std::min(h->num_cus, kn.num_cus.v));
  }
  if ((rc = plan_launches(h->K, h->V, h->scheme, kn, h->plan))) return bail(rc);
  h->cfg = &h->plan.cfg_parts;
  h->z_split = h->plan.split;
  if (pcgs_family(h->scheme)) h->pcgs_z = pcgs_entry(h->plan, h->scheme, h->plan.wave_forced);
  for (const KernelLaunch *l : h->plan.all())
    if (l->fn && hipFuncSetAttribute(l->fn, hipFuncAttributeMaxDynamicSharedMemorySize, kMaxLdsBytes) != hipSuccess) return bail(GGS_ERR_HIP);
  for (const void *f : {reinterpret_cast<const void *>(ll_docs_kernel), reinterpret_cast<const void *>(lp_docs_kernel)})
    if (hipFuncSetAttribute(f, hipFuncAttributeMaxDynamicSharedMemorySize, kMaxLdsBytes) != hipSuccess) return bail(GGS_ERR_HIP);
  const bool with_phi = !counts_only(h->scheme);
  const size_t kv = (size_t)h->K * h->V, phi_elems = (size_t)h->V * h->Kp + kPhiTailPadBytes / 8;
  if ((rc = upload(h, &h->d_alpha, h->alpha)) || (with_phi && (rc = dev_alloc_zeroed(h, &h->d_phiT, phi_elems))) ||
      (rc = dev_alloc(h, &h->d_mag, h->K)) || (rc = dev_alloc(h, &h->d_tot, h->K)) || (rc = dev_alloc_zeroed(h, &h->d_n_wk, kv)) ||
      (rc = dev_alloc_zeroed(h, &h->d_n_k, h->K)) || (rc = dev_alloc_zeroed(h, &h->d_status, 4)))
    return bail(rc);
  if ((h->flags & GGS_FLAG_SAVE_PHI_MEAN) && (rc = dev_alloc_zeroed(h, &h->d_phi_mean, kv))) return bail(rc);
  if (h->plan.sliced() && h->plan.f32) {
    if ((rc = dev_alloc_zeroed(h, &h->d_phiT32, (size_t)h->V * h->plan.Kp32 + kPhiTailPadBytes / 4))) return bail(rc);
    if (kn.replays.is(1) && (rc = dev_alloc_zeroed(h, &h->d_replays, 1))) return bail(rc);
  }
  if (h->exact_sum && ((rc = dev_alloc(h, &h->d_sum_pref, ((size_t)h->sum_nseg + 1) * h->K)) ||
                       (rc = dev_alloc(h, &h->d_sum_fn, (size_t)h->sum_nseg * h->K * 4))))
    return bail(rc);
  if (has_tables(h->scheme) && ((rc = dev_alloc_zeroed(h, &h->d_alias_ps, kv)) || (rc = dev_alloc_zeroed(h, &h->d_alias_a, kv)) || (rc = dev_alloc_zeroed(h, &h->d_alias_tn, (size_t)h->V)))) return bail(rc);
  if (has_mh(h->scheme) && (rc = dev_alloc_zeroed(h, &h->d_mh, 3))) return bail(rc);
  if (has_word_lists(h->scheme) && ((rc = dev_alloc_zeroed(h, &h->d_nzw, kv)) || (rc = dev_alloc_zeroed(h, &h->d_nw, (size_t)h->V)))) return bail(rc);
  if (has_sparse_stats(h->scheme) && (rc = dev_alloc_zeroed(h, &h->d_ps_stats, 4))) return bail(rc);
  if (h->scheme == Scheme::nzvsspalias) {
    h->vs_W = (h->V + 31) / 32; h->vs_pitch = (h->K + 31) / 32;
    h->vs_global = h->plan.vschain.lds == 0;
    const size_t kw = (size_t)h->K * h->vs_W, vm = (size_t)h->V * h->vs_pitch;
    if ((rc = dev_alloc(h, &h->d_vs_cz, kw)) || (rc = dev_alloc(h, &h->d_vs_pz, kw)) || (rc = dev_alloc_zeroed(h, &h->d_vs_und, kw)) ||
        (rc = dev_alloc_zeroed(h, &h->d_vs_mask, vm)) || (rc = dev_alloc(h, &h->d_vs_s_end, (size_t)h->K)) || (rc = dev_alloc_zeroed(h, &h->d_vs_rounds, (size_t)h->K)) ||
        (rc = dev_alloc(h, &h->d_vs_zero, 1)) || (h->vs_global && (rc = dev_alloc(h, &h->d_vs_work, 2 * kw))))
      return bail(rc);
  }
  if (poisson_phi(h->scheme)) {
    std::vector<double> T;
    build_poisson_table(h->beta, h->pa_L, T);
    h->pa_t00 = T[0];
    if ((rc = upload(h, &h->d_pa_table, T)) || (rc = dev_alloc(h, &h->d_pa_acc, (size_t)h->K * kPoissonAccStride))) return bail(rc);
  }
  if (count_tables(h->scheme) && (rc = dev_alloc_zeroed(h, &h->d_tpt, (size_t)h->V))) return bail(rc);
  if (h->scheme == Scheme::adlda && ((rc = dev_alloc_zeroed(h, &h->d_ad_den0, (size_t)h->K)) || (rc = dev_alloc_zeroed(h, &h->d_ad_s0, 1)))) return bail(rc);
  if (h->scheme == Scheme::collapsed && (rc = dev_alloc(h, &h->d_lcg, 2))) return bail(rc);
  for (auto &e : h->ev_part)
    if (hipEventCreateWithFlags(&e, hipEventDisableTiming) != hipSuccess) return bail(GGS_ERR_HIP);
  for (auto &E : h->evs) {
    for (auto &e : E.e)
      if (hipEventCreate(&e) != hipSuccess) return bail(GGS_ERR_HIP);
    for (auto &e : E.x)
      if (hipEventCreate(&e) != hipSuccess) return bail(GGS_ERR_HIP);
    if (hipEventCreate(&E.th0) != hipSuccess || hipEventCreate(&E.th1) != hipSuccess) return bail(GGS_ERR_HIP);
  }
  {
    int lo = 0, hi = 0;
    (void)hipDeviceGetStreamPriorityRange(&lo, &hi);
    if (hipStreamCreateWithPriority(&h->side, hipStreamNonBlocking, lo) != hipSuccess) return bail(GGS_ERR_HIP);
    if (hipStreamCreateWithPriority(&h->side_hot, hipStreamNonBlocking, hi) != hipSuccess || hipEventCreate(&h->ev_hot_fork) != hipSuccess ||
        hipEventCreate(&h->ev_hot_join) != hipSuccess || hipEventCreateWithFlags(&h->ev_chain_done, hipEventDisableTiming) != hipSuccess)
      return bail(GGS_ERR_HIP);
  }
  if (hipDeviceSynchronize() != hipSuccess) return bail(GGS_ERR_HIP);
  *out = h;
  return GGS_OK;
}

void ggs_destroy(ggs_handle *h) {
  if (!h) return;
  (void)hipSetDevice(h->device);
  (void)hipDeviceSynchronize();
  if (h->d_replays) {
    unsigned long long n = 0;
    if (hipMemcpy(&n, h->d_replays, sizeof(n), hipMemcpyDeviceToHost) == hipSuccess)
      fprintf(stderr, "[ggs] z replays: %llu tokens in %lld launches of z_sliced32_kernel (%.2f per launch)\n", n, (long long)h->z_f32_launches,
              h->z_f32_launches ? (double)n / (double)h->z_f32_launches : 0.0);
  }
  for (void **slot : h->owned)
    if (*slot) (void)hipFree(*slot);
  if (h->d_scratch) (void)hipFree(h->d_scratch);
  if (h->d_heldout_spill) (void)hipFree(h->d_heldout_spill);
  exchange_free(h->xg);
  if (h->own_stream) (void)hipStreamDestroy(h->own_stream);
  if (h->comm_stream) (void)hipStreamDestroy(h->comm_stream);
  if (h->ev_half_drawn) (void)hipEventDestroy(h->ev_half_drawn);
  if (h->ev_half_gathered) (void)hipEventDestroy(h->ev_half_gathered);
  for (auto &e : h->ev_part)
    if (e) (void)hipEventDestroy(e);
  for (auto &E : h->evs) {
    for (auto &e : E.e)
      if (e) (void)hipEventDestroy(e);
    for (auto &e : E.x)
      if (e) (void)hipEventDestroy(e);
    if (E.th0) (void)hipEventDestroy(E.th0);
    if (E.th1) (void)hipEventDestroy(E.th1);
  }
  if (h->side) (void)hipStreamDestroy(h->side);
  if (h->side_hot) (void)hipStreamDestroy(h->side_hot);
  if (h->ev_hot_fork) (void)hipEventDestroy(h->ev_hot_fork);
  if (h->ev_hot_join) (void)hipEventDestroy(h->ev_hot_join);
  if (h->ev_chain_done) (void)hipEventDestroy(h->ev_chain_done);
// ... 538 lines not shown
      }
    } else if ((rc = group_phi(hs, n, false, true))) return rc;
    if (s == n_sweeps - 1 || (hs[0]->flags & GGS_FLAG_PARANOID))
      for (int32_t i = 0; i < n; ++i)
        if ((rc = bind_device(hs[i])) || (rc = check_status(hs[i])) || (rc = settle_sweeps(hs[i]))) return rc;
  }
  return GGS_OK;
}

static int copy_out(ggs_handle *h, void *dst, const void *src, size_t bytes) {
  if (!bytes) return GGS_OK;
  HIP_TRY(h, hipMemcpyAsync(dst, src, bytes, hipMemcpyDeviceToHost, h->stream));
  HIP_TRY(h, hipStreamSynchronize(h->stream));
  return GGS_OK;
}

int ggs_synchronize(ggs_handle *h) {
  if (!h) return GGS_ERR_BAD_ARG;
  int rc = bind_device(h);
  if (rc) return rc;
  return check_status(h);
}

int ggs_get_z(ggs_handle *h, int32_t *z) {
  int rc = require_ready(h, false);
  if (rc) return rc;
  if (h->N > 0 && !z) return GGS_ERR_BAD_ARG;
  return copy_out(h, z, h->d_z, sizeof(int32_t) * (size_t)h->N);
}
int ggs_get_type_topic_counts(ggs_handle *h, int32_t *n_wk) {
  if (!h || !n_wk) return GGS_ERR_BAD_ARG;
  int rc = bind_device(h);
  if (rc) return rc;
  if ((rc = ensure_global_counts(h))) return rc;
  return copy_out(h, n_wk, h->d_n_wk, sizeof(int32_t) * (size_t)h->K * h->V);
}
int ggs_get_topic_totals(ggs_handle *h, int32_t *n_k) {
  if (!h || !n_k) return GGS_ERR_BAD_ARG;
  int rc = bind_device(h);
  if (rc) return rc;
  h->n_k_valid = h->n_k_valid && h->xg != nullptr;
  if ((rc = launch_magnitude(h))) return rc;
  return copy_out(h, n_k, h->d_n_k, sizeof(int32_t) * (size_t)h->K);
}

static int phi_out(ggs_handle *h, const double *src_T, int32_t pitch, double *dst, double scale) {
  const size_t kv = (size_t)h->K * h->V;
  int rc = ensure_scratch(h, kv * sizeof(double));
  if (rc) return rc;
  hipLaunchKernelGGL(phiT_to_phi_kernel, dim3(grid_for((int64_t)kv, 256)), dim3(256), 0, h->stream, src_T, static_cast<double *>(h->d_scratch),
                     h->K, pitch, h->V, scale);
  HIP_TRY(h, hipGetLastError());
  return copy_out(h, dst, h->d_scratch, kv * sizeof(double));
}
int ggs_get_phi(ggs_handle *h, double *phi) {
  if (!h || !phi) return GGS_ERR_BAD_ARG;
  int rc = bind_device(h);
  if (rc) return rc;
  if (count_form(h->scheme)) {
    if (!h->d_phiT && (rc = dev_alloc(h, &h->d_phiT, (size_t)h->V * h->Kp + kPhiTailPadBytes / 8))) return rc;
    if ((rc = launch_magnitude(h))) return rc;
    hipLaunchKernelGGL(psi_kernel, dim3(grid_for((int64_t)h->K * h->V, 256, 2)), dim3(256), 0, h->stream, h->d_n_wk, h->d_n_k, h->beta, h->beta * (double)h->V,
                       h->d_phiT, h->K, h->Kp, h->V);
    HIP_TRY(h, hipGetLastError());
  }
  return phi_out(h, h->d_phiT, h->Kp, phi, 1.0);
}
int ggs_set_phi(ggs_handle *h, const double *phi) {
  if (!h || !phi) return GGS_ERR_BAD_ARG;
  int rc = bind_device(h);
  if (rc) return rc;
  if (counts_only(h->scheme)) return set_err(h, GGS_ERR_UNSUPPORTED, "scheme=lightcollapsed and scheme=adlda have no Phi to set");
  const size_t kv = (size_t)h->K * h->V;
  if (h->have_priors) {
    for (int32_t v = 0; v < h->V; ++v)
      for (int32_t j = 0; j < h->pr_pitch; ++j)
        for (uint32_t bits = h->pr_mask[(size_t)v * h->pr_pitch + j]; bits; bits &= bits - 1)
          if (phi[(size_t)(j * 32 + __builtin_ctz(bits)) * h->V + v] != 0.0)
            return set_err(h, GGS_ERR_BAD_ARG, "ggs_set_phi: phi is not zero in a cell the topic priors zero");
  }
  if ((rc = ensure_scratch(h, kv * sizeof(double)))) return rc;
  HIP_TRY(h, hipMemcpyAsync(h->d_scratch, phi, kv * sizeof(double), hipMemcpyHostToDevice, h->stream));
  hipLaunchKernelGGL(phi_to_phiT_kernel, dim3(grid_for((int64_t)kv, 256)), dim3(256), 0, h->stream, static_cast<const double *>(h->d_scratch),
                     h->d_phiT, h->K, h->Kp, h->V, h->d_phiT32, h->plan.Kp32);
  HIP_TRY(h, hipGetLastError());
  if (h->d_phi_mean) HIP_TRY(h, hipMemsetAsync(h->d_phi_mean, 0, kv * sizeof(double), h->stream));
  h->alias_stale = true;
  h->vs_lists = ggs_handle::VsLists::nonzero;
  h->vs_drawn = false;
  if ((rc = launch_alias_build(h))) return rc;
  HIP_TRY(h, hipStreamSynchronize(h->stream));
  h->have_phi = true;
  return GGS_OK;
}

int ggs_set_topic_priors(ggs_handle *h, int64_t n_zero, const int32_t *topic, const int32_t *word) {
  if (!h) return GGS_ERR_BAD_ARG;
  int rc = bind_device(h);
  if (rc) return rc;
  if (h->scheme != Scheme::spalias) return set_err(h, GGS_ERR_STATE, "ggs_set_topic_priors needs GGS_FLAG_SPALIAS");
  if (h->have_phi) return set_err(h, GGS_ERR_STATE, "ggs_set_topic_priors: the handle already has a Phi");
  if (n_zero < 0 || (n_zero > 0 && (!topic || !word))) return set_err(h, GGS_ERR_BAD_ARG, "bad topic prior arguments");
  const int32_t pitch = (h->K + 31) / 32;
  std::vector<uint32_t> mask((size_t)h->V * pitch, 0u);
  std::vector<int32_t> per_topic((size_t)h->K, 0), per_word((size_t)h->V, 0);
  for (int64_t i = 0; i < n_zero; ++i) {
    const int32_t k = topic[i], v = word[i];
    if (k < 0 || k >= h->K || v < 0 || v >= h->V) return set_err(h, GGS_ERR_BAD_ARG, "topic prior cell outside [0, num_topics) x [0, num_types)");
    uint32_t &m = mask[(size_t)v * pitch + (k >> 5)];
    if (m & (1u << (k & 31))) continue;
    m |= 1u << (k & 31);
    per_topic[(size_t)k] += 1; per_word[(size_t)v] += 1;
  }
  for (int32_t k = 0; k < h->K; ++k)
    if (per_topic[(size_t)k] == h->V) return set_err(h, GGS_ERR_BAD_ARG, "Inconsistent prior spec, one topic has all Zero priors!");
  for (int32_t v = 0; v < h->V; ++v)
    if (per_word[(size_t)v] == h->K) return set_err(h, GGS_ERR_BAD_ARG, "Inconsistent prior spec, word " + std::to_string(v) + " has all Zero priors!");
  HIP_TRY(h, hipStreamSynchronize(h->stream));
  if ((rc = upload(h, &h->d_pr_mask, mask)) || (rc = dev_alloc(h, &h->d_pr_sum_phi, (size_t)h->K))) return rc;
  if (h->exact_sum && ((rc = dev_alloc(h, &h->d_pr_pref, ((size_t)h->sum_nseg + 1) * h->K)) || (rc = dev_alloc(h, &h->d_pr_fn, (size_t)h->sum_nseg * h->K * 4))))
    return rc;
  h->pr_mask.swap(mask);
  h->pr_pitch = pitch;
  h->have_priors = true;
  return GGS_OK;
}

int ggs_get_topic_priors(ggs_handle *h, double *priors) {
  if (!h || !priors) return GGS_ERR_BAD_ARG;
  int rc = bind_device(h);
  if (rc) return rc;
  if (h->scheme != Scheme::spalias) return set_err(h, GGS_ERR_STATE, "ggs_get_topic_priors needs GGS_FLAG_SPALIAS");
  std::fill(priors, priors + (size_t)h->K * h->V, 1.0);
  if (!h->have_priors) return GGS_OK;
  std::vector<uint32_t> mask((size_t)h->V * h->pr_pitch);
  if ((rc = copy_out(h, mask.data(), h->d_pr_mask, mask.size() * sizeof(uint32_t)))) return rc;
  for (int32_t v = 0; v < h->V; ++v)
    for (int32_t j = 0; j < h->pr_pitch; ++j)
      for (uint32_t bits = mask[(size_t)v * h->pr_pitch + j]; bits; bits &= bits - 1)
        priors[(size_t)(j * 32 + __builtin_ctz(bits)) * h->V + v] = 0.0;
  return GGS_OK;
}

static int refresh_tables(ggs_handle *h) {
  int rc;
  if (count_form(h->scheme) || count_tables(h->scheme)) return (rc = require_ready(h, false)) ? rc : launch_sweep_head(h);
  if (!h->have_phi) return set_err(h, GGS_ERR_STATE, "no Phi yet: call ggs_init_phi or ggs_set_phi first");
  return h->alias_stale ? launch_alias_build(h) : GGS_OK;
}
int ggs_get_alias_tables(ggs_handle *h, double *ps, int32_t *a, double *type_norm) {
  if (!h) return GGS_ERR_BAD_ARG;
  int rc = bind_device(h);
  if (rc) return rc;
  if (!has_tables(h->scheme))
    return counts_only(h->scheme) ? set_err(h, GGS_ERR_UNSUPPORTED, "scheme=adlda builds no alias tables") : set_err(h, GGS_ERR_STATE, needs_flag("ggs_get_alias_tables", kHasTables));
  if ((rc = refresh_tables(h))) return rc;
  const size_t kv = (size_t)h->K * h->V;
  std::vector<int32_t> n(count_tables(h->scheme) ? (size_t)h->V : 0);
  if (!n.empty()) HIP_TRY(h, hipMemcpyAsync(n.data(), h->d_nw, n.size() * sizeof(int32_t), hipMemcpyDeviceToHost, h->stream));
  if (ps) HIP_TRY(h, hipMemcpyAsync(ps, h->d_alias_ps, kv * sizeof(double), hipMemcpyDeviceToHost, h->stream));
  if (a) HIP_TRY(h, hipMemcpyAsync(a, h->d_alias_a, kv * sizeof(int32_t), hipMemcpyDeviceToHost, h->stream));
  if (type_norm) HIP_TRY(h, hipMemcpyAsync(type_norm, h->d_alias_tn, (size_t)h->V * sizeof(double), hipMemcpyDeviceToHost, h->stream));
  HIP_TRY(h, hipStreamSynchronize(h->stream));
  for (size_t w = 0; w < n.size(); ++w)
    for (int32_t i = n[w]; i < h->K; ++i) {
      if (ps) ps[w * h->K + i] = 1.0;
      if (a) a[w * h->K + i] = i;
// ... 687 lines not shown
  }
  HIP_TRY(h, hipGetLastError());
  std::vector<double> ll((size_t)D);
  if (D) HIP_TRY(h, hipMemcpyAsync(ll.data(), h->d_test_ll, sizeof(double) * (size_t)D, hipMemcpyDeviceToHost, h->stream));
  if ((rc = check_status(h))) return rc;
  double t = 0;
  for (int64_t d = 0; d < D; ++d) t += ll[(size_t)d];
  *total = t;
  if (doc_ll && D) std::memcpy(doc_ll, ll.data(), sizeof(double) * (size_t)D);
  return GGS_OK;
}

int ggs_get_timings(ggs_handle *h, ggs_timings *out) { if (!h || !out) return GGS_ERR_BAD_ARG; *out = h->tm; return GGS_OK; }
int ggs_reset_timings(ggs_handle *h) { if (!h) return GGS_ERR_BAD_ARG; h->tm = ggs_timings{}; return GGS_OK; }

int ggs_check_invariants(ggs_handle *h) {
  int rc = require_ready(h, false);
  if (rc) return rc;
  const int K = h->K;
  const size_t bytes = 16 + sizeof(int32_t) * (size_t)K;
  if ((rc = ensure_global_counts(h))) return rc;
  if ((rc = ensure_scratch(h, bytes))) return rc;
  auto *d_total = static_cast<unsigned long long *>(h->d_scratch);
  auto *d_flags = reinterpret_cast<uint32_t *>(static_cast<char *>(h->d_scratch) + 8);
  auto *d_col = reinterpret_cast<int32_t *>(static_cast<char *>(h->d_scratch) + 16);
  HIP_TRY(h, hipMemsetAsync(h->d_scratch, 0, bytes, h->stream));
  const int64_t kv = (int64_t)K * h->V;
  hipLaunchKernelGGL(invariants_kernel, dim3(grid_for(kv, 256)), dim3(256), 0, h->stream, h->d_n_wk, kv, K, d_total, d_col, d_flags);
  HIP_TRY(h, hipGetLastError());
  if ((rc = launch_magnitude(h))) return rc;
  std::vector<unsigned char> host(bytes);
  std::vector<int32_t> nk((size_t)K);
  if ((rc = copy_out(h, host.data(), h->d_scratch, bytes))) return rc;
  if ((rc = copy_out(h, nk.data(), h->d_n_k, sizeof(int32_t) * (size_t)K))) return rc;
  unsigned long long total; uint32_t fl;
  std::memcpy(&total, host.data(), 8); std::memcpy(&fl, host.data() + 8, 4);
  const int32_t *col = reinterpret_cast<const int32_t *>(host.data() + 16);
  if (fl & 1u) return set_err(h, GGS_ERR_INVARIANT, "negative type-topic count");
  if ((int64_t)total != (h->global_tokens >= 0 ? h->global_tokens : h->N)) return set_err(h, GGS_ERR_INVARIANT, "type-topic counts do not sum to the corpus size");
  for (int k = 0; k < K; ++k)
    if (col[k] != nk[(size_t)k]) return set_err(h, GGS_ERR_INVARIANT, "column sum differs from tokensPerTopic");
  return GGS_OK;
}

int ggs_get_launch_info(ggs_handle *h, int64_t *num_chunks, int32_t *lds_bytes_z, int32_t *docs_per_block_theta) {
  if (!h) return GGS_ERR_BAD_ARG;
  const LaunchPlan &pl = h->plan;
  const bool pcgs = pcgs_family(h->scheme);
  if (num_chunks) *num_chunks = pcgs ? h->pcgs_items : pl.sliced() ? h->Cs + h->Cw : h->C;
  if (lds_bytes_z) *lds_bytes_z = pcgs ? h->pcgs_z.lds : pl.sliced() ? sliced_fused_lds(h->K, pl.hot_cap) : pl.z.lds;
  if (docs_per_block_theta) *docs_per_block_theta = h->cfg->theta_docs;
  return GGS_OK;
}

int ggs_get_num_hot_words(ggs_handle *h, int32_t *num_hot) {
  if (!h || !num_hot) return GGS_ERR_BAD_ARG;
  *num_hot = h->plan.sliced() ? h->num_hot + h->num_warm : 0;
  return GGS_OK;
}

int ggs_get_z_parts(ggs_handle *h, int32_t *parts) {
  if (!h || !parts) return GGS_ERR_BAD_ARG;
  const int32_t P = (int32_t)h->part_doc.size() - 1;
  *parts = (h->plan.stream() && h->overlap_theta && P > 1) ? P : 1;
  return GGS_OK;
}

int ggs_get_warm_tiers(ggs_handle *h, int32_t *tiers, int32_t *warm_words, int32_t *docs_per_chunk) {
  if (!h) return GGS_ERR_BAD_ARG;
  const bool on = h->have_corpus && h->plan.sliced();
  if (tiers) *tiers = on ? h->warm_tiers : 0;
  if (warm_words) *warm_words = on ? h->num_warm : 0;
  if (docs_per_chunk) *docs_per_chunk = on && h->warm_tiers ? h->plan.warm_docs : 0;
  return GGS_OK;
}

int ggs_get_z_form(ggs_handle *h, int32_t *kernel, int32_t *form, int32_t *calibrated) {
  if (!h) return GGS_ERR_BAD_ARG;
  const bool splittable = h->plan.sliced() && h->Cs > h->Cc && h->Cc > 0;
  const int32_t own = row_of(h->scheme).z_kernel;
  if (kernel) *kernel = own ? own : pcgs_family(h->scheme) ? (h->pcgs_wave ? 5 : 4) : h->plan.kernel;
  if (form) *form = h->plan.sliced() ? (splittable && h->z_split ? 1 : 2) : 0;
  if (calibrated) *calibrated = (splittable && h->z_split_tried && !h->plan.split_forced && h->plan.split) ? 1 : 0;
  return GGS_OK;
}

int ggs_java_lcg_next_ints(int32_t seed, int32_t bound, int64_t n, int32_t *out) {
  if (bound <= 0 || n < 0 || (n > 0 && !out)) return GGS_ERR_BAD_ARG;
  java_lcg_next_ints(seed, bound, n, out);
  return GGS_OK;
}

namespace {
struct TmpDev {
  std::vector<void *> p;
  ~TmpDev() { for (void *q : p) if (q) (void)hipFree(q); }
  void *get(size_t bytes) { void *q = nullptr; if (hipMalloc(&q, std::max<size_t>(bytes, 16)) != hipSuccess) return nullptr; p.push_back(q); return q; }
};
}

int ggs_debug_philox(int32_t device_id, int64_t n, const uint32_t *ctr, const uint32_t *key, uint32_t *out) {
  if (n <= 0 || !ctr || !key || !out || hipSetDevice(device_id) != hipSuccess) return GGS_ERR_BAD_ARG;
  TmpDev t;
  auto *dc = static_cast<uint32_t *>(t.get(n * 16)); auto *dk = static_cast<uint32_t *>(t.get(n * 8)); auto *dou = static_cast<uint32_t *>(t.get(n * 16));
  if (!dc || !dk || !dou) return GGS_ERR_HIP;
  if (hipMemcpy(dc, ctr, n * 16, hipMemcpyHostToDevice) != hipSuccess || hipMemcpy(dk, key, n * 8, hipMemcpyHostToDevice) != hipSuccess) return GGS_ERR_HIP;
  hipLaunchKernelGGL(debug_philox_kernel, dim3((unsigned)((n + 255) / 256)), dim3(256), 0, nullptr, n, dc, dk, dou);
  if (hipMemcpy(out, dou, n * 16, hipMemcpyDeviceToHost) != hipSuccess) return GGS_ERR_HIP;
  return GGS_OK;
}

int ggs_debug_math(int32_t device_id, int32_t op, int64_t n, const double *x, const double *y, double *out) {
  if (n <= 0 || !x || !out || hipSetDevice(device_id) != hipSuccess) return GGS_ERR_BAD_ARG;
  TmpDev t;
  auto *dx = static_cast<double *>(t.get(n * 8)); auto *dy = static_cast<double *>(t.get(n * 8)); auto *dou = static_cast<double *>(t.get(n * 8));
  if (!dx || !dy || !dou) return GGS_ERR_HIP;
  if (hipMemcpy(dx, x, n * 8, hipMemcpyHostToDevice) != hipSuccess) return GGS_ERR_HIP;
  if (hipMemcpy(dy, y ? y : x, n * 8, hipMemcpyHostToDevice) != hipSuccess) return GGS_ERR_HIP;
  hipLaunchKernelGGL(debug_math_kernel, dim3((unsigned)((n + 255) / 256)), dim3(256), 0, nullptr, op, n, dx, dy, dou);
  if (hipMemcpy(out, dou, n * 8, hipMemcpyDeviceToHost) != hipSuccess) return GGS_ERR_HIP;
  return GGS_OK;
}

int ggs_debug_draw(int32_t device_id, int32_t kind, uint64_t seed, uint32_t iteration, uint32_t purpose, uint64_t elem0, int64_t n,
                   const double *shape, double *out, int32_t *status) {
  if (n <= 0 || !out || (kind == 2 && !shape) || hipSetDevice(device_id) != hipSuccess) return GGS_ERR_BAD_ARG;
  TmpDev t;
  auto *ds = static_cast<double *>(t.get(n * 8)); auto *dou = static_cast<double *>(t.get(n * 8)); auto *dst = static_cast<uint32_t *>(t.get(16));
  if (!ds || !dou || !dst) return GGS_ERR_HIP;
  if (shape && hipMemcpy(ds, shape, n * 8, hipMemcpyHostToDevice) != hipSuccess) return GGS_ERR_HIP;
  if (hipMemset(dst, 0, 16) != hipSuccess) return GGS_ERR_HIP;
  hipLaunchKernelGGL(debug_draw_kernel, dim3((unsigned)((n + 255) / 256)), dim3(256), 0, nullptr, kind, seed, iteration, purpose, elem0, n, ds, dou, dst);
  uint32_t st = 0;
  if (hipMemcpy(out, dou, n * 8, hipMemcpyDeviceToHost) != hipSuccess || hipMemcpy(&st, dst, 4, hipMemcpyDeviceToHost) != hipSuccess) return GGS_ERR_HIP;
  if (status) *status = (int32_t)st;
  return GGS_OK;
}

int ggs_debug_poisson(int32_t device_id, double beta, int32_t threshold, uint64_t seed, uint32_t iteration, uint32_t purpose, uint64_t elem0, int64_t n,
                      const int32_t *counts, int32_t *out) {
  const int32_t L = threshold == 0 ? 100 : threshold;
  if (n <= 0 || !counts || !out || !(beta > 0) || L < 1 || L > kPoissonMaxThreshold || hipSetDevice(device_id) != hipSuccess) return GGS_ERR_BAD_ARG;
  for (int64_t i = 0; i < n; ++i)
    if (counts[i] < 0) return GGS_ERR_BAD_ARG;
  std::vector<double> T;
  build_poisson_table(beta, L, T);
  TmpDev t;
  auto *dt = static_cast<double *>(t.get(T.size() * 8)); auto *dc = static_cast<int32_t *>(t.get(n * 4));
  auto *dou = static_cast<int32_t *>(t.get(n * 4)); auto *dst = static_cast<uint32_t *>(t.get(16));
  if (!dt || !dc || !dou || !dst) return GGS_ERR_HIP;
  if (hipMemcpy(dt, T.data(), T.size() * 8, hipMemcpyHostToDevice) != hipSuccess || hipMemcpy(dc, counts, n * 4, hipMemcpyHostToDevice) != hipSuccess ||
      hipMemset(dst, 0, 16) != hipSuccess)
    return GGS_ERR_HIP;
  hipLaunchKernelGGL(debug_poisson_kernel, dim3((unsigned)((n + 255) / 256)), dim3(256), 0, nullptr, seed, iteration, purpose, elem0, n, dc, L, beta, dt, T[0],
                     dou, dst);
  uint32_t st = 0;
  if (hipGetLastError() != hipSuccess || hipMemcpy(out, dou, n * 4, hipMemcpyDeviceToHost) != hipSuccess || hipMemcpy(&st, dst, 4, hipMemcpyDeviceToHost) != hipSuccess)
    return GGS_ERR_HIP;
  return st ? GGS_ERR_RNG_EXHAUSTED : GGS_OK;
}

int ggs_debug_alias(int32_t device_id, int32_t V, int32_t K, const double *phi, const double *alpha, double *ps, int32_t *a, double *type_norm) {
  if (V <= 0 || K <= 0 || K > kPcgsWaveMaxTopics || !phi || !alpha || !ps || !a || !type_norm || hipSetDevice(device_id) != hipSuccess) return GGS_ERR_BAD_ARG;
  const size_t kv = (size_t)K * V;
  std::vector<double> phiT(kv);
  for (int32_t k = 0; k < K; ++k)
// ... 197 lines not shown
```

ldagroupedgibbssampler_amd/csrc/ggs_kernels.hpp:

```cpp
#pragma once
#include "ggs_device_math.hpp"
#include "ggs_exact_sum.hpp"

namespace ggs {

constexpr double kJavaMinValue = 4.9e-324;

__device__ __forceinline__ uint32_t udiv_magic(uint32_t d) { return d > 1 ? (uint32_t)((0x100000000ull + d - 1) / d) : 0u; }
__device__ __forceinline__ int udiv_small(int x, uint32_t m) { return m ? (int)__umulhi((uint32_t)x, m) : x; }

enum StatusBits : uint32_t {
  ST_NEGATIVE_COUNT = 1u << 0,
  ST_INVALID_TOPIC = 1u << 1,
  ST_RNG_EXHAUSTED = 1u << 2,
  ST_BAD_SHAPE = 1u << 3,
  ST_INVARIANT = 1u << 4,
};

struct ThetaParams {
  const int64_t *doc_ptr;
  const int32_t *z;
  const double *alpha;
  double *theta;
  uint32_t *status;
// ... 398 lines not shown
    const int si = udiv_small((int)tile, m_ncg), cg = (int)tile - si * p.ncg;
    const int seg = p.seg_begin + si, v0 = seg * 64, kb = cg * p.kc, kw = min(p.kc, p.K - kb);
    const int rows = min(64, p.V - v0), n = rows * kw;
    const uint32_t m_kw = udiv_magic((uint32_t)kw);
    __syncthreads();
    if (lane < kw) {
      SegCand c{kSegNoGuess, true};
      if (p.guess) c = seg_candidates(p.guess[(size_t)seg * p.K + kb + lane], p.guess[(size_t)(seg + 1) * p.K + kb + lane]);
      e_los[lane] = c.e_lo; aheads[lane] = c.ahead ? 1 : 0; acc_lo[lane] = 0; acc_hi[lane] = 0; flag_s[lane] = 0;
      ctab[lane] = gamma_consts(shape_of_count(0, kb + lane));
    }
    if (lane == 0) qn = 0;
    int n_a = 0, n_b = 0;
#pragma unroll 1
    for (int j0 = 0; j0 < n; j0 += 64) {
      const int j = j0 + lane;
      bool listed = false, a = false;
      if (j < n) {
        const int dv = udiv_small(j, m_kw), v = v0 + dv, k = kb + (j - dv * kw);
        listed = true;
        if constexpr (MASKED) {
          const int kg = p.k0 + k;
          if ((p.zero_mask[(size_t)v * p.mask_pitch + (kg >> 5)] >> (kg & 31)) & 1u) {
            p.phiT[(size_t)v * p.Kp + k] = (MODE == kDrawVS && p.undrawn_negative) ? -0.0 : 0.0;
            listed = false;
          }
        }
        a = listed && p.n_wk[(size_t)v * p.cnt_pitch + k] == 0;
      }
      const unsigned long long ma = __ballot(a), mb = __ballot(listed && !a), mine = a ? ma : mb;
      const int rank = (int)__builtin_amdgcn_mbcnt_hi((uint32_t)(mine >> 32), __builtin_amdgcn_mbcnt_lo((uint32_t)mine, 0u));
      if (a) list[n_a + rank] = (uint16_t)j;
      else if (listed) list[n - 1 - (n_b + rank)] = (uint16_t)j;
      n_a += (int)__popcll(ma); n_b += (int)__popcll(mb);
    }
    __syncthreads();
    auto emit = [&](int v, int c, double g) {
      if constexpr (PRIORS) { if (g <= 0) g = kConditionalMinGamma; }
      p.phiT[(size_t)v * p.Kp + kb + c] = g;
      const int e_lo = e_los[c];
      if (e_lo == kSegNoGuess) return;
      double q_lo, q_hi;
      int fl;
      seg_quantise(g, e_lo, q_lo, q_hi, fl);
      seg_accumulate(&acc_lo[c], &acc_hi[c], &flag_s[c], q_lo, q_hi, fl);
    };
#pragma unroll 1
    for (int pos = lane; pos < n_a + n_b; pos += 64) {
      const int j = list[pos < n_a ? pos : n - n_b + (pos - n_a)];
      const int dv = udiv_small(j, m_kw), v = v0 + dv, c = j - dv * kw, k = kb + c;
      const bool table = __ballot(pos >= n_a) == 0;
      const double shape = table ? ctab[c].shape : shape_of(v, k);
      double g;
      if (shape > 0) {
        const uint64_t elem = (uint64_t)(p.k0 + k) * (uint64_t)p.V + (uint64_t)v;
        const bool drawn = table ? rgamma_first_try(p.seed, p.iteration, p.purpose, elem, ctab[c], g)
                                 : rgamma_first_try(p.seed, p.iteration, p.purpose, elem, shape, g);
        if (!drawn) {
          const int slot = atomicAdd(&qn, 1);
          if (slot < p.queue_cap) { queue[slot] = (uint16_t)j; continue; }
          g = draw_general(v, k, shape);
        }
      } else {
        g = __builtin_nan("");
        atomicOr(p.status, ST_BAD_SHAPE);
      }
      emit(v, c, g);
    }
    __syncthreads();
    for (int q = lane, m = min(qn, p.queue_cap); q < m; q += 64) {
      const int j = queue[q], dv = udiv_small(j, m_kw), v = v0 + dv, c = j - dv * kw;
      emit(v, c, draw_general(v, kb + c, shape_of(v, kb + c)));
    }
    __syncthreads();
    if (p.guess && lane < kw)
      seg_compose(SegCand{e_los[lane], aheads[lane] != 0}, acc_lo[lane], acc_hi[lane], flag_s[lane], 0.0, p.fn + ((size_t)seg * p.K + kb + lane) * 4);
  }
}
template <bool PRIORS>
__global__ __launch_bounds__(64) void phi_gamma_kernel(PhiGammaParams p) { phi_gamma_body<PRIORS ? kDrawPriors : kDrawPlain>(p); }
__global__ __launch_bounds__(64) void phi_gamma_vs_kernel(PhiGammaParams p) { phi_gamma_body<kDrawVS>(p); }

__device__ __forceinline__ float phi32_of(const double x) { return (x >= 0.0 && x <= 1.0) ? (float)x : __builtin_nanf(""); }

enum PhiNorm { kPhiDirichlet, kPhiPolyaurn, kPhiConditional, kPhiVS };
template <int MODE>
__device__ __forceinline__ void phi_normalise_body(double *phiT, const double *tot, int32_t K, int32_t Kp, int32_t V, double *phi_mean, float *phiT32,
                                                   int32_t Kp32, const double *sum_phi = nullptr) {
  __builtin_amdgcn_s_setprio(3);
  const int64_t n = (int64_t)V * K;
  const int64_t stride = (int64_t)gridDim.x * blockDim.x;
  for (int64_t i = (int64_t)blockIdx.x * blockDim.x + threadIdx.x; i < n; i += stride) {
    const int v = (int)(i / K), k = (int)(i - (int64_t)v * K);
    double x = phiT[(size_t)v * Kp + k];
    const double s = tot[k];
    if constexpr (MODE == kPhiPolyaurn) {
      x = s > 0 ? x / s : 0.0;
      phiT[(size_t)v * Kp + k] = x;
    } else if constexpr (MODE == kPhiConditional) {
      x = (x / s) * sum_phi[k];
      phiT[(size_t)v * Kp + k] = x;
    } else if (s != 0) {
      x = x / s;
      if (x <= 0) x = kJavaMinValue;
      phiT[(size_t)v * Kp + k] = x;
    }
    if (phiT32) phiT32[(size_t)v * Kp32 + k] = phi32_of(x);
    if (phi_mean) phi_mean[i] += x;
  }
}
__global__ __launch_bounds__(256) void phi_normalise_kernel(double *phiT, const double *tot, int32_t K, int32_t Kp, int32_t V,
                                                            double *phi_mean , float *phiT32 , int32_t Kp32) {
  phi_normalise_body<kPhiDirichlet>(phiT, tot, K, Kp, V, phi_mean, phiT32, Kp32);
}
__global__ __launch_bounds__(256) void phi_normalise_polyaurn_kernel(double *phiT, const double *tot, int32_t K, int32_t Kp, int32_t V, double *phi_mean,
                                                                     float *phiT32, int32_t Kp32) {
  phi_normalise_body<kPhiPolyaurn>(phiT, tot, K, Kp, V, phi_mean, phiT32, Kp32);
}
__global__ __launch_bounds__(256) void phi_normalise_conditional_kernel(double *phiT, const double *tot, const double *sum_phi, int32_t K, int32_t Kp, int32_t V,
                                                                        double *phi_mean, float *phiT32, int32_t Kp32) {
  phi_normalise_body<kPhiConditional>(phiT, tot, K, Kp, V, phi_mean, phiT32, Kp32, sum_phi);
}
__global__ __launch_bounds__(256) void phi_apply_priors_kernel(double *phiT, const uint32_t *zero_mask, int32_t mask_pitch, int32_t K, int32_t Kp, int32_t V,
                                                               float *phiT32, int32_t Kp32) {
  const int64_t n = (int64_t)V * K;
  const int64_t stride = (int64_t)gridDim.x * blockDim.x;
  for (int64_t i = (int64_t)blockIdx.x * blockDim.x + threadIdx.x; i < n; i += stride) {
    const int v = (int)(i / K), k = (int)(i - (int64_t)v * K);
    const double prior = ((zero_mask[(size_t)v * mask_pitch + (k >> 5)] >> (k & 31)) & 1u) ? 0.0 : 1.0;
    const double x = phiT[(size_t)v * Kp + k] * prior;
    phiT[(size_t)v * Kp + k] = x;
    if (phiT32) phiT32[(size_t)v * Kp32 + k] = phi32_of(x);
  }
}

struct PhiRepackParams {
  const double *all0, *all1;
  const int32_t *krank, *kcol;
  double *phiT, *phi_mean;
  int64_t c0, c1;
  int32_t K, Kp, V, Ksm, v_split;
  float *phiT32;
  int32_t Kp32;
  const double *sum_phi;
};
template <int MODE>
__device__ __forceinline__ void phi_repack_body(const PhiRepackParams &p) {
  __builtin_amdgcn_s_setprio(3);
  const int64_t n = (int64_t)p.V * p.K;
  const int64_t stride = (int64_t)gridDim.x * blockDim.x;
  const int64_t tot_off = (int64_t)(p.V - p.v_split) * p.Ksm;
  for (int64_t i = (int64_t)blockIdx.x * blockDim.x + threadIdx.x; i < n; i += stride) {
    const int v = (int)(i / p.K), k = (int)(i - (int64_t)v * p.K);
    const int r = p.krank[k], j = p.kcol[k];
    const double *h1 = p.all1 + (int64_t)r * p.c1;
    double x = v < p.v_split ? p.all0[(int64_t)r * p.c0 + (int64_t)v * p.Ksm + j] : h1[(int64_t)(v - p.v_split) * p.Ksm + j];
    const double s = h1[tot_off + j];
    if constexpr (MODE == kPhiPolyaurn) {
      x = s > 0 ? x / s : 0.0;
    } else if constexpr (MODE == kPhiVS) {
      x = (s > 0 && x != 0.0) ? x / s : 0.0;
    } else if constexpr (MODE == kPhiConditional) {
      x = (x / s) * p.sum_phi[k];
    } else if (s != 0) {
      x = x / s;
      if (x <= 0) x = kJavaMinValue;
    }
    p.phiT[(size_t)v * p.Kp + k] = x;
    if (p.phiT32) p.phiT32[(size_t)v * p.Kp32 + k] = phi32_of(x);
    if (p.phi_mean) p.phi_mean[i] += x;
  }
}
__global__ __launch_bounds__(256) void phi_repack_kernel(PhiRepackParams p) { phi_repack_body<kPhiDirichlet>(p); }
__global__ __launch_bounds__(256) void phi_repack_polyaurn_kernel(PhiRepackParams p) { phi_repack_body<kPhiPolyaurn>(p); }
__global__ __launch_bounds__(256) void phi_repack_conditional_kernel(PhiRepackParams p) { phi_repack_body<kPhiConditional>(p); }
__global__ __launch_bounds__(256) void phi_repack_vs_kernel(PhiRepackParams p) { phi_repack_body<kPhiVS>(p); }
__global__ __launch_bounds__(256) void vs_mask_gathered_kernel(PhiRepackParams p, uint32_t *mask, int32_t pitch) {
  const int64_t n = (int64_t)p.V * pitch, stride = (int64_t)gridDim.x * blockDim.x;
  for (int64_t i = (int64_t)blockIdx.x * blockDim.x + threadIdx.x; i < n; i += stride) {
    const int v = (int)(i / pitch), m = (int)(i - (int64_t)v * pitch);
    uint32_t word = 0;
    for (int b = 0; b < 32; ++b) {
      const int k = m * 32 + b;
      if (k >= p.K) break;
      const int r = p.krank[k], j = p.kcol[k];
      const double x = v < p.v_split ? p.all0[(int64_t)r * p.c0 + (int64_t)v * p.Ksm + j] : p.all1[(int64_t)r * p.c1 + (int64_t)(v - p.v_split) * p.Ksm + j];
      word |= (uint32_t)(x == 0.0 && __builtin_signbit(x)) << b;
    }
    mask[i] = word;
  }
}
__global__ __launch_bounds__(256) void counts_unslice_kernel(const int32_t *cnt_all, const int64_t *koff, int32_t Ksm, int32_t *n_wk, int32_t K,
                                                             int32_t V) {
  const int64_t n = (int64_t)V * K;
  const int64_t stride = (int64_t)gridDim.x * blockDim.x;
  for (int64_t i = (int64_t)blockIdx.x * blockDim.x + threadIdx.x; i < n; i += stride) {
    const int v = (int)(i / K), k = (int)(i - (int64_t)v * K);
    n_wk[i] = cnt_all[koff[k] + (int64_t)v * Ksm];
  }
}
__global__ __launch_bounds__(256) void counts_slice_kernel(const int32_t *n_wk, const int64_t *koff, int32_t Ksm, int32_t *cnt_send, int32_t K,
                                                           int32_t V) {
  const int64_t n = (int64_t)V * K;
  const int64_t stride = (int64_t)gridDim.x * blockDim.x;
  for (int64_t i = (int64_t)blockIdx.x * blockDim.x + threadIdx.x; i < n; i += stride) {
    const int v = (int)(i / K), k = (int)(i - (int64_t)v * K);
    cnt_send[koff[k] + (int64_t)v * Ksm] = n_wk[i];
  }
}

__global__ __launch_bounds__(256) void phiT_to_phi_kernel(const double *phiT, double *phi, int32_t K, int32_t Kp, int32_t V, double scale) {
  const int64_t n = (int64_t)V * K;
  const int64_t stride = (int64_t)gridDim.x * blockDim.x;
  for (int64_t i = (int64_t)blockIdx.x * blockDim.x + threadIdx.x; i < n; i += stride) {
    const int k = (int)(i / V), v = (int)(i - (int64_t)k * V);
    const double x = phiT[(size_t)v * Kp + k];
    phi[i] = (scale == 1.0) ? x : x / scale;
  }
}
__global__ __launch_bounds__(256) void phi_to_phiT_kernel(const double *phi, double *phiT, int32_t K, int32_t Kp, int32_t V, float *phiT32, int32_t Kp32) {
  const int64_t n = (int64_t)V * K;
  const int64_t stride = (int64_t)gridDim.x * blockDim.x;
  for (int64_t i = (int64_t)blockIdx.x * blockDim.x + threadIdx.x; i < n; i += stride) {
    const int v = (int)(i / K), k = (int)(i - (int64_t)v * K);
    const double x = phi[(size_t)k * V + v];
    phiT[(size_t)v * Kp + k] = x;
    if (phiT32) phiT32[(size_t)v * Kp32 + k] = phi32_of(x);
  }
}

__global__ __launch_bounds__(64) void doc_topic_kernel(const int64_t *doc_ptr, const int32_t *z, int64_t d_begin, int32_t K, int32_t *n_dk) {
  const int64_t d = d_begin + blockIdx.x;
  int32_t *row = n_dk + (size_t)blockIdx.x * K;
  for (int64_t i = doc_ptr[d] + threadIdx.x; i < doc_ptr[d + 1]; i += 64) atomicAdd(&row[z[i]], 1);
}

__global__ __launch_bounds__(256) void invariants_kernel(const int32_t *n_wk, int64_t n, int32_t K, unsigned long long *total,
                                                         int32_t *colsum, uint32_t *flags) {
  const int64_t stride = (int64_t)gridDim.x * blockDim.x;
  unsigned long long t = 0;
  for (int64_t i = (int64_t)blockIdx.x * blockDim.x + threadIdx.x; i < n; i += stride) {
    const int32_t c = n_wk[i];
    if (c < 0) atomicOr(flags, 1u);
    if (c) { t += (unsigned long long)c; atomicAdd(&colsum[i % K], c); }
  }
  if (t) atomicAdd(total, t);
}

__global__ void debug_philox_kernel(int64_t n, const uint32_t *ctr, const uint32_t *key, uint32_t *out) {
  const int64_t i = (int64_t)blockIdx.x * blockDim.x + threadIdx.x;
  if (i >= n) return;
  const U4 o = philox4x32_10(ctr[4 * i], ctr[4 * i + 1], ctr[4 * i + 2], ctr[4 * i + 3], key[2 * i], key[2 * i + 1]);
  out[4 * i] = o.x; out[4 * i + 1] = o.y; out[4 * i + 2] = o.z; out[4 * i + 3] = o.w;
}
__global__ void debug_math_kernel(int op, int64_t n, const double *x, const double *y, double *out) {
  const int64_t i = (int64_t)blockIdx.x * blockDim.x + threadIdx.x;
  if (i >= n) return;
  double r;
  switch (op) {
    case 0: r = strict_log(x[i]); break;
    case 1: r = strict_pow(x[i], y[i]); break;
    case 2: r = sqrt(x[i]); break;
    case 4: r = strict_exp(x[i]); break;
    case 5: r = boost_pow(x[i], y[i]); break;
    case 6: r = u53((uint32_t)x[i], (uint32_t)y[i]); break;
    default: r = x[i] / y[i]; break;
  }
  out[i] = r;
}
__global__ void debug_draw_kernel(int kind, uint64_t seed, uint32_t iteration, uint32_t purpose, uint64_t elem0, int64_t n,
                                  const double *shape, double *out, uint32_t *status) {
  const int64_t i = (int64_t)blockIdx.x * blockDim.x + threadIdx.x;
  if (i >= n) return;
  DrawStream rs(seed, iteration, purpose, elem0 + (uint64_t)i);
  double r;
  if (kind == 0) r = rs.next_double();
  else if (kind == 1) r = rs.next_gaussian();
  else if (kind == 2 || !(shape[i] > 0)) {
    if (shape[i] > 0) r = rgamma(rs, shape[i]);
    else { r = __builtin_nan(""); atomicOr(status, ST_BAD_SHAPE); }
  } else {
    if (!rgamma_first_try(seed, iteration, purpose, elem0 + (uint64_t)i, shape[i], r)) r = rgamma(rs, shape[i]);
    else if (kind == 4) r = -r;
  }
  if (rs.exhausted) atomicOr(status, ST_RNG_EXHAUSTED);
  out[i] = r;
}

}

#include "ggs_z_kernel.hpp"
```

ldagroupedgibbssampler_amd/csrc/ggs_z_kernel.hpp:

```cpp
#pragma once
#include "ggs_kernels.hpp"

namespace ggs {

struct SliceMap {
  int32_t rem, size, ksm;
  uint32_t m_size, m_size1;
  int64_t rank_stride;
};
__device__ __forceinline__ int64_t slice_cell(const SliceMap &m, int k, int w) {
  const int cut = m.rem * (m.size + 1);
  int r, c;
  if (k < cut) { r = udiv_small(k, m.m_size1); c = k - r * (m.size + 1); }
  else { const int q = udiv_small(k - cut, m.m_size); r = m.rem + q; c = k - cut - q * m.size; }
  return (int64_t)r * m.rank_stride + (int64_t)w * m.ksm + c;
}

__device__ __forceinline__ void slice_rank_col(const SliceMap &m, int k, int &r, int &c) {
  const int cut = m.rem * (m.size + 1);
  if (k < cut) { r = udiv_small(k, m.m_size1); c = k - r * (m.size + 1); }
  else { const int q = udiv_small(k - cut, m.m_size); r = m.rem + q; c = k - cut - q * m.size; }
}

struct ZParams {
  const int32_t *tok;
  const int32_t *inv_perm;
  int32_t *z;
  int32_t *zw;
  const int64_t *chunk_start;
  const int32_t *chunk_doc;
  const int32_t *chunk_len;
  const double *theta;
  const double *phiT;
  uint32_t *status;
  int64_t num_chunks;
  int64_t tok_base;
  uint64_t seed;
  uint32_t iteration;
  int32_t K, Kp, pitch16, tile_tokens;
  const int32_t *ct_tok;
  const int32_t *ct_idx;
  const int32_t *ct_ip;
  const int32_t *c_docs;
  int64_t num_cold;
  const int32_t *hot_words;
  int32_t num_hot, hot_pitch;
  int32_t hot_off, wave_lds;
  int32_t ring_base;
  double margin_scale;
  const int32_t *chunk_doc1;
  int32_t two_rows;
  int32_t *cnt_send;
  SliceMap smap;
  const int4 *ht_pack;
  const int32_t *h_docs;
  const int4 *wt_pack;
  const int32_t *w_docs;
  const int32_t *warm_words;
  const int64_t *warm_meta;
  int32_t warm_tiers, warm_rows;
  const float *phiT32;
  int32_t Kp32;
  unsigned long long *replays;
  double margin_scale32;
};

struct alignas(16) D2 { double a, b; };

typedef __attribute__((address_space(3))) void lds_void_t;
typedef __attribute__((address_space(1))) const void glb_cvoid_t;
typedef __attribute__((address_space(4))) const int64_t const_i64_t;
typedef __attribute__((address_space(4))) const int32_t const_i32_t;

__device__ __forceinline__ D2 lds_d2(const unsigned char *p) { return *reinterpret_cast<const D2 *>(p); }

constexpr int z_tile_theta_bytes(const int Kp) { return (Kp * 8 + 15) / 16 * 16; }
constexpr int z_tile_lds_bytes(const int Kp, const int pitch16, const int T) { return T * pitch16 * 16 + z_tile_theta_bytes(Kp); }
constexpr int z_tile_rows_in(const int bytes, const int Kp, const int pitch16) { return (bytes - z_tile_theta_bytes(Kp)) / (pitch16 * 16); }

template <int NT>
__global__ __launch_bounds__(64) void z_kernel(ZParams p) {
  extern __shared__ __align__(16) unsigned char smem[];
  const int lane = threadIdx.x;
  const int K = p.K, Kp = p.Kp;
  const int upr = Kp >> 1;
  const int pitch = p.pitch16 * 16;
  unsigned char *thb = smem + (size_t)p.tile_tokens * pitch;
  const unsigned char *phib = reinterpret_cast<const unsigned char *>(p.phiT);
  const size_t rowbytes = (size_t)Kp * 8;
  const const_i64_t *cstart = (const const_i64_t *)p.chunk_start;
  const const_i32_t *clen = (const const_i32_t *)p.chunk_len;
  const const_i32_t *cdoc = (const const_i32_t *)p.chunk_doc;
  const int64_t stride = gridDim.x;
  const int64_t C = p.num_chunks;

  int64_t c = blockIdx.x;
  if (c >= C) return;
  int64_t start = cstart[c];
  int len = clen[c], doc = cdoc[c];
  int64_t nstart = 0;
  int nlen = 0, ndoc = 0;
  if (c + stride < C) { nstart = cstart[c + stride]; nlen = clen[c + stride]; ndoc = cdoc[c + stride]; }
  int w = (lane < len) ? p.tok[start + lane] : 0;
  double tv[NT];
  {
    const double *thg = p.theta + (size_t)doc * K;
#pragma unroll
    for (int t = 0; t < NT; ++t) tv[t] = (t * 64 + lane < K) ? thg[t * 64 + lane] : 0.0;
  }

  for (;;) {
#pragma unroll
    for (int t = 0; t < NT; ++t)
      if (t * 64 + lane < Kp) reinterpret_cast<double *>(thb)[t * 64 + lane] = tv[t];

    const bool has_next = c + stride < C;
    int64_t nnstart = 0;
    int nnlen = 0, nndoc = 0, wn = 0;
    if (has_next) {
      if (c + 2 * stride < C) { nnstart = cstart[c + 2 * stride]; nnlen = clen[c + 2 * stride]; nndoc = cdoc[c + 2 * stride]; }
      wn = (lane < nlen) ? p.tok[nstart + lane] : 0;
      const double *thg = p.theta + (size_t)ndoc * K;
#pragma unroll
      for (int t = 0; t < NT; ++t) tv[t] = (t * 64 + lane < K) ? thg[t * 64 + lane] : 0.0;
    }

    for (int i = 0; i < len; ++i) {
      const int wi = __builtin_amdgcn_readlane(w, i);
      const unsigned char *rb = phib + (size_t)wi * rowbytes;
      unsigned char *dst = smem + (size_t)i * pitch;
      for (int u0 = 0; u0 < upr; u0 += 64) {
        const int u = u0 + lane;
        if (u < upr)
          __builtin_amdgcn_global_load_lds((glb_cvoid_t *)(rb + (size_t)u * 16), (lds_void_t *)(dst + (size_t)u0 * 16), 16, 0, 0);
      }
    }
    asm volatile("s_waitcnt vmcnt(0)");
    __syncthreads();

    if (lane < len) {
      const unsigned char *rowp = smem + lane * pitch;

#define GGS_LD8(A, P) { A##0 = lds_d2(P); A##1 = lds_d2((P) + 16); A##2 = lds_d2((P) + 32); A##3 = lds_d2((P) + 48); }
#define GGS_SUM8(A, S) { \
        sum += (S##0).a * (A##0).a; sum += (S##0).b * (A##0).b; sum += (S##1).a * (A##1).a; sum += (S##1).b * (A##1).b; \
// ... 90 lines not shown
```

ldagroupedgibbssampler_amd/csrc/ggs_z_sliced.hpp:

```cpp
#pragma once
#include <type_traits>

#include "ggs_z_kernel.hpp"

#ifndef GGS_ABL
#define GGS_ABL 0
#endif

namespace ggs {

constexpr int kSliceTopics = 16;
constexpr int kSliceUnits = 8;
constexpr int kSlice32Topics = 32;
constexpr int kSliceBytes = 64 * 128;
#ifndef GGS_RING_SLOTS
#define GGS_RING_SLOTS 2
#endif
constexpr int kRingSlots = GGS_RING_SLOTS;
constexpr int kSlicedMaxTopics = 192;
constexpr int kSlicedDefaultTopics = 160;
constexpr int kPhiTailPadBytes = 1024;
constexpr int kHotTailBytes = 64;

constexpr int kWarmThetaPad = 16;
#ifndef GGS_WARM_UNITS
#define GGS_WARM_UNITS 4
#endif
#ifndef GGS_WARM_LANE_DOUBLES
#define GGS_WARM_LANE_DOUBLES 12
#endif
constexpr int warm_docs_for(const int kmax) {
  const int rowd = (kmax + kSliceTopics - 1) / kSliceTopics * kSliceTopics;
  const int d = rowd <= 112 ? GGS_WARM_LANE_DOUBLES / 2 : rowd <= 128 ? GGS_WARM_LANE_DOUBLES / 2 - 1 : 2;
  return d < 2 ? 2 : d > 8 ? 8 : d;
}

constexpr int sliced_kmax(const int K) { return (K + 7) / 8 * 8; }
constexpr int sliced_slices(const int K) { return (sliced_kmax(K) + kSliceTopics - 1) / kSliceTopics; }
constexpr int sliced_ring_base(const int K) { return round_up(imax(kChunkDocs * sliced_kmax(K) * 8, sliced_slices(K) * 128), 256); }
constexpr int sliced_wave_lds(const int K) { return sliced_ring_base(K) + kRingSlots * kSliceBytes; }
constexpr int sliced_cold_lds(const int K) { return kSlicedWaves * sliced_wave_lds(K); }
constexpr int table_row_pitch(const int K) { return sliced_kmax(K) / 8 * 64 + 16; }
constexpr int sliced_fused_lds(const int K, const int rows) { return sliced_cold_lds(K) + rows * table_row_pitch(K); }
constexpr int hot_wave_lds(const int K) { return round_up(kChunkDocs * sliced_slices(K) * kSliceTopics * 8, 256); }
constexpr int warm_wave_lds(const int K) { return round_up(warm_docs_for(sliced_kmax(K)) * (sliced_slices(K) * kSliceTopics * 8 + kWarmThetaPad), 256); }
constexpr int table_lds(const int K, const int wave_lds, const int rows) { return kSlicedWaves * wave_lds + rows * table_row_pitch(K) + kHotTailBytes; }
constexpr int table_rows_beside_cold(const int K, const int wave_lds) {
  return imax(0, imin(255, ((kMaxLdsBytes - lds_alloc_of(sliced_cold_lds(K)) - kSlicedWaves * wave_lds) / kLdsGranule * kLdsGranule - kHotTailBytes) / table_row_pitch(K)));
}
constexpr int table_rows_fused(const int K) { return imax(0, imin(255, (kMaxLdsBytes - sliced_cold_lds(K)) / table_row_pitch(K))); }

struct alignas(8) D2u { double a, b; };

template <int S, int N, class F>
__device__ __forceinline__ void static_for(F &&f) {
  if constexpr (S < N) {
    f(std::integral_constant<int, S>{});
    static_for<S + 1, N>(f);
  }
}

typedef float f2_t __attribute__((ext_vector_type(2)));
typedef float f4_t __attribute__((ext_vector_type(4)));
template <int KMAX>
__device__ __forceinline__ void cold_chunks32(const ZParams &p, unsigned char *thb, unsigned char *ring, const int64_t wid, const int64_t stride, const int lane) {
  constexpr int NS = (KMAX + kSlice32Topics - 1) / kSlice32Topics;
  constexpr int kAhead = NS < kRingSlots - 1 ? NS : kRingSlots - 1;
  constexpr int NT = (KMAX + 63) / 64;
  constexpr int kThetaRow = KMAX * 4;
  const int K = p.K;
  const unsigned char *phib = reinterpret_cast<const unsigned char *>(p.phiT32);
  const size_t rowbytes = (size_t)p.Kp32 * 4;
  const const_i32_t *cdocs = (const const_i32_t *)p.c_docs;
  double *prod = reinterpret_cast<double *>(thb + kChunkDocs * kThetaRow);
  const int lrow = lane >> 3, lslot = lane & 7;
  const unsigned char *my_row = ring + lane * 128;
  const int rot = lane >> 1;
  const float mscale = (float)p.margin_scale32;

  auto load_theta = [&](const int d0, const int d1, double (&tv)[kChunkDocs][NT]) {
    const double *t0 = p.theta + (size_t)d0 * K, *t1 = p.theta + (size_t)d1 * K;
#pragma unroll
    for (int t = 0; t < NT; ++t) {
      tv[0][t] = (t * 64 + lane < K) ? t0[t * 64 + lane] : 0.0;
      tv[1][t] = (t * 64 + lane < K) ? t1[t * 64 + lane] : 0.0;
    }
  };
  auto stage_theta = [&](const double (&tv)[kChunkDocs][NT]) {
#pragma unroll
    for (int r = 0; r < kChunkDocs; ++r)
#pragma unroll
      for (int t = 0; t < NT; ++t)
        if (t * 64 + lane < KMAX) reinterpret_cast<float *>(thb + r * kThetaRow)[t * 64 + lane] = phi32_of(tv[r][t]);
  };
  auto row_addresses = [&](const int w, const unsigned char *(&ra)[8]) {
#pragma unroll
    for (int m = 0; m < 8; ++m) {
      const int row = 8 * m + lrow;
      const int wm = __shfl(w, row) & ((1 << kSlotShift) - 1);
      ra[m] = phib + (size_t)wm * rowbytes + (size_t)(((lslot - (row >> 1)) & 7) << 4);
    }
  };
  auto issue_slice = [&](auto sc, const int slot, const unsigned char *const (&ra)[8]) {
    constexpr int s = decltype(sc)::value;
#pragma unroll
    for (int m = 0; m < 8; ++m)
      __builtin_amdgcn_global_load_lds((glb_cvoid_t *)ra[m], (lds_void_t *)(ring + slot * kSliceBytes + m * 1024 - s * 128), 16, s * 128, 0);
  };
  auto finish = [&](const float (&a)[KMAX], const int64_t c, const int idx, const int ip, const int w) {
    const uint64_t gtok = (uint64_t)(p.tok_base + idx);
    const double U = z_uniform(gtok, p.iteration, p.seed);
    const float A = a[KMAX - 1];
    const float t0 = (float)(U * (double)A);
    const float delta = ((float)(2 * K + 8) * 0x1p-24f * A) * mscale;
    const f2_t nt0 = {-t0, -t0};
    int cnt = 0;
    float m = t0;
    bool live = true;
#pragma unroll
    for (int kb = 0; kb < KMAX; kb += 16) {
// ... 62 lines not shown
  if (c + stride < C) {
    const int64_t c1 = c + stride;
    w1 = p.ct_tok[c1 * 64 + lane]; id1 = p.ct_idx[c1 * 64 + lane]; ip1 = p.ct_ip[c1 * 64 + lane];
    load_theta(cdocs[2 * c1], cdocs[2 * c1 + 1], tv1);
  } else {
    load_theta(0, 0, tv1);
  }
#pragma unroll
  for (int r = 0; r < kChunkDocs; ++r)
#pragma unroll
    for (int t = 0; t < NT; ++t) tv2[r][t] = 0.0;
  const unsigned char *ra[8], *ran[8];
  row_addresses(w0, ra);
  row_addresses(w1, ran);
  int g = 0;
  static_for<0, kAhead>([&](auto sc) { issue_slice(sc, decltype(sc)::value % kRingSlots, ra); });

  for (;;) {
    const bool has1 = c + stride < C, has2 = c + 2 * stride < C;
    g = __builtin_amdgcn_readfirstlane(g);
    stage_theta(tv0);
    const unsigned char *trow = thb + ((unsigned)w0 >> kSlotShift) * kThetaRow;

    float a[KMAX];
    float acc = 0.0f;
    static_for<0, NS>([&](auto sidx) {
      constexpr int s = decltype(sidx)::value;
      const int cur = (g + s) % kRingSlots;
      const int nxt = (g + s + kAhead) % kRingSlots;
      if constexpr (s + kAhead < NS) issue_slice(std::integral_constant<int, s + kAhead>{}, nxt, ra);
      else if (has1) issue_slice(std::integral_constant<int, s + kAhead - NS>{}, nxt, ran);
      if (has1 || s + kAhead < NS) asm volatile("s_waitcnt vmcnt(%0)" ::"n"(8 * kAhead) : "memory");
      else asm volatile("s_waitcnt vmcnt(%0)" ::"n"(8 * (NS - 1 - s)) : "memory");
      {
        const unsigned char *rb = my_row + cur * kSliceBytes;
        f4_t ph[kSliceUnits], th[kSliceUnits];
#pragma unroll
        for (int u = 0; u < kSliceUnits; ++u)
          if (s * kSlice32Topics + 4 * u < KMAX) {
            ph[u] = *reinterpret_cast<const f4_t *>(rb + (((u + rot) & 7) << 4));
            th[u] = *reinterpret_cast<const f4_t *>(trow + s * (kSlice32Topics * 4) + u * 16);
          }
#pragma unroll
        for (int u = 0; u < kSliceUnits; ++u) {
          constexpr int k0 = s * kSlice32Topics;
          const int k = k0 + 4 * u;
          if (k < KMAX) {
            const f2_t q0 = f2_t{th[u].x, th[u].y} * f2_t{ph[u].x, ph[u].y};
            const f2_t q1 = f2_t{th[u].z, th[u].w} * f2_t{ph[u].z, ph[u].w};
            acc += q0.x; a[k] = acc;
            acc += q0.y; a[k + 1] = acc;
            acc += q1.x; a[k + 2] = acc;
            acc += q1.y; a[k + 3] = acc;
          }
        }
      }
      asm volatile("s_waitcnt lgkmcnt(0)" ::: "memory");
    });
    g = (g + NS) % kRingSlots;

    if (has2) {
      const int64_t c2 = c + 2 * stride;
      w2 = p.ct_tok[c2 * 64 + lane]; id2 = p.ct_idx[c2 * 64 + lane]; ip2 = p.ct_ip[c2 * 64 + lane];
      load_theta(cdocs[2 * c2], cdocs[2 * c2 + 1], tv2);
    } else {
      w2 = 0; id2 = -1; ip2 = 0;
    }

    finish(a, c, id0, ip0, w0);
    if (!has1) break;
    c += stride;
    w0 = w1; id0 = id1; ip0 = ip1;
    w1 = w2; id1 = id2; ip1 = ip2;
#pragma unroll
    for (int r = 0; r < kChunkDocs; ++r)
#pragma unroll
      for (int t = 0; t < NT; ++t) { tv0[r][t] = tv1[r][t]; tv1[r][t] = tv2[r][t]; }
#pragma unroll
    for (int m = 0; m < 8; ++m) ra[m] = ran[m];
    row_addresses(w1, ran);
  }
}

template <int KMAX, bool F32>
__device__ __forceinline__ void z_sliced_body(const ZParams &p) {
  constexpr int NS = (KMAX + kSliceTopics - 1) / kSliceTopics;
  constexpr int kAhead = NS < kRingSlots - 1 ? NS : kRingSlots - 1;
  constexpr int NT = (KMAX + 63) / 64;
  constexpr int kThetaRow = KMAX * 8;
  extern __shared__ __align__(16) unsigned char smem[];
  const int lane = threadIdx.x & 63, wave = __builtin_amdgcn_readfirstlane(threadIdx.x >> 6);
  const int K = p.K;
  unsigned char *thb = smem + wave * p.wave_lds;
  unsigned char *ring = thb + p.ring_base;
  const unsigned char *phib = reinterpret_cast<const unsigned char *>(p.phiT);
  const size_t rowbytes = (size_t)p.Kp * 8;
  const const_i32_t *cdocs = (const const_i32_t *)p.c_docs;
  const int64_t stride = (int64_t)gridDim.x * kSlicedWaves;
  const int64_t wid = (int64_t)blockIdx.x * kSlicedWaves + wave;

  {
    constexpr int upr = KMAX / 2;
    for (int i = threadIdx.x; i < p.num_hot * upr; i += kSlicedWaves * 64) {
      const int r = i / upr, u = i - r * upr;
      *reinterpret_cast<D2 *>(smem + p.hot_off + r * p.hot_pitch + u * 16) =
          *reinterpret_cast<const D2 *>(phib + (size_t)p.hot_words[r] * rowbytes + (size_t)u * 16);
    }
  }
  __syncthreads();

  const int lrow = lane >> 3, lslot = lane & 7;
  const unsigned char *my_row = ring + lane * 128;
  const int rot = lane >> 1;

  auto load_theta = [&](const int d0, const int d1, double (&tv)[kChunkDocs][NT]) {
    const double *t0 = p.theta + (size_t)d0 * K, *t1 = p.theta + (size_t)d1 * K;
#pragma unroll
    for (int t = 0; t < NT; ++t) {
      tv[0][t] = (t * 64 + lane < K) ? t0[t * 64 + lane] : 0.0;
      tv[1][t] = (t * 64 + lane < K) ? t1[t * 64 + lane] : 0.0;
    }
  };
  auto stage_theta = [&](const double (&tv)[kChunkDocs][NT]) {
#pragma unroll
    for (int r = 0; r < kChunkDocs; ++r)
#pragma unroll
      for (int t = 0; t < NT; ++t)
        if (t * 64 + lane < KMAX) reinterpret_cast<double *>(thb + r * kThetaRow)[t * 64 + lane] = tv[r][t];
  };
  auto finish = [&](const double (&sc)[KMAX], const double sum, const int idx, const int ip, const int word) {
    if (idx < 0) return;
    const uint64_t gtok = (uint64_t)(p.tok_base + idx);
    const double U = z_uniform(gtok, p.iteration, p.seed);
    double t = 0.0 - U * sum;
    int cnt = 0;
    bool live = true;
#pragma unroll
    for (int kb = 0; kb < KMAX; kb += 16) {
      if (live) {
        uint32_t bits = 0;
#pragma unroll
        for (int j = 0; j < 16; ++j)
          if (kb + j < KMAX) {
            bits = __builtin_amdgcn_alignbit(bits, (uint32_t)hi32(t), 31);
            t += sc[kb + j];
          }
        cnt += __popc(bits);
        live = __any(hi32(t) < 0);
      }
    }
    int new_topic = cnt - 1;
    if (new_topic < 0 || hi32(t) < 0) {
      if (!GGS_ABL) atomicOr(p.status, ST_INVALID_TOPIC);
      new_topic = new_topic < 0 ? 0 : K - 1;
    }
    p.z[idx] = new_topic;
    p.zw[ip] = new_topic;
    if (p.cnt_send && word >= 0) __hip_atomic_fetch_add(&p.cnt_send[slice_cell(p.smap, new_topic, word)], 1, __ATOMIC_RELAXED, __HIP_MEMORY_SCOPE_AGENT);
  };

  auto cold_chunks = [&]() {
    const int64_t C = p.num_cold;
    auto row_addresses = [&](const int w, const unsigned char *(&ra)[8]) {
#pragma unroll
      for (int m = 0; m < 8; ++m) {
        const int row = 8 * m + lrow;
// ... 78 lines not shown
        const int64_t c2 = c + 2 * stride;
        w2 = p.ct_tok[c2 * 64 + lane]; id2 = p.ct_idx[c2 * 64 + lane]; ip2 = p.ct_ip[c2 * 64 + lane];
        load_theta(cdocs[2 * c2], cdocs[2 * c2 + 1], tv2);
      } else {
        w2 = 0; id2 = -1; ip2 = 0;
      }

      finish(sc, sum, id0, ip0, w0 & ((1 << kSlotShift) - 1));
      if (!has1) break;
      c += stride;
      w0 = w1; id0 = id1; ip0 = ip1;
      w1 = w2; id1 = id2; ip1 = ip2;
#pragma unroll
      for (int r = 0; r < kChunkDocs; ++r)
#pragma unroll
        for (int t = 0; t < NT; ++t) { tv0[r][t] = tv1[r][t]; tv1[r][t] = tv2[r][t]; }
#pragma unroll
      for (int m = 0; m < 8; ++m) ra[m] = ran[m];
      row_addresses(w1, ran);
    }
  };

  auto hot_chunks = [&]() {
    const int64_t C = p.num_chunks;
    int64_t c = p.num_cold + wid;
    if (c >= C) return;
    int w0 = p.ct_tok[c * 64 + lane], id0 = p.ct_idx[c * 64 + lane], ip0 = p.ct_ip[c * 64 + lane];
    double tv0[kChunkDocs][NT];
    load_theta(cdocs[2 * c], cdocs[2 * c + 1], tv0);
    for (;;) {
      const bool has1 = c + stride < C;
      int w1 = 0, id1 = -1, ip1 = 0;
      double tv1[kChunkDocs][NT];
      if (has1) {
        const int64_t c1 = c + stride;
        w1 = p.ct_tok[c1 * 64 + lane]; id1 = p.ct_idx[c1 * 64 + lane]; ip1 = p.ct_ip[c1 * 64 + lane];
        load_theta(cdocs[2 * c1], cdocs[2 * c1 + 1], tv1);
      } else {
        load_theta(0, 0, tv1);
      }
      stage_theta(tv0);
      const unsigned char *trow = thb + ((unsigned)w0 >> kSlotShift) * kThetaRow;
      const unsigned char *hrow = smem + p.hot_off + (w0 & ((1 << kSlotShift) - 1)) * p.hot_pitch;

      double sc[KMAX];
      double sum = 0.0;
      if (id0 >= 0) {
        static_for<0, NS>([&](auto sidx) {
          constexpr int s = decltype(sidx)::value;
          D2 ph[kSliceUnits], th[kSliceUnits];
#pragma unroll
          for (int u = 0; u < kSliceUnits; ++u)
            if (s * kSliceTopics + 2 * u + 1 < KMAX) {
              ph[u] = lds_d2(hrow + s * (kSliceTopics * 8) + u * 16);
              th[u] = lds_d2(trow + s * (kSliceTopics * 8) + u * 16);
            }
#pragma unroll
          for (int u = 0; u < kSliceUnits; ++u) {
            constexpr int k0 = s * kSliceTopics;
            const int k = k0 + 2 * u;
            if (k + 1 < KMAX) {
              sc[k] = th[u].a * ph[u].a;
              sum += sc[k];
              sc[k + 1] = th[u].b * ph[u].b;
              sum += sc[k + 1];
            }
          }
        });
      }
      finish(sc, sum, id0, ip0, -1);
      if (!has1) break;
      c += stride;
      w0 = w1; id0 = id1; ip0 = ip1;
#pragma unroll
      for (int r = 0; r < kChunkDocs; ++r)
#pragma unroll
        for (int t = 0; t < NT; ++t) tv0[r][t] = tv1[r][t];
    }
  };

#pragma unroll 1
  for (int phase = 0; phase < 2; ++phase) {
    if ((phase ^ wave) & 1) hot_chunks();
    else if constexpr (F32) cold_chunks32<KMAX>(p, thb, ring, wid, stride, lane);
    else cold_chunks();
  }
}

template <int KMAX>
__global__ __launch_bounds__(kSlicedWaves * 64) void z_sliced_kernel(ZParams p) { z_sliced_body<KMAX, false>(p); }
template <int KMAX>
__global__ __launch_bounds__(kSlicedWaves * 64) void z_sliced32_kernel(ZParams p) { z_sliced_body<KMAX, true>(p); }

template <int KMAX>
__device__ __forceinline__ void load_phi_table(unsigned char *table, const int pitch, const unsigned char *phib, const size_t rowbytes,
                                               const int32_t *words_g, const int nrows, const int wave, const int lane, const int tid) {
  constexpr int upr = KMAX / 2 + 1, kRowsAhead = 6, NP = (upr + 63) / 64;
  const const_i32_t *words = (const const_i32_t *)words_g;
  for (int r0 = wave; r0 < nrows; r0 += kSlicedWaves * kRowsAhead) {
    D2 v[kRowsAhead][NP];
#pragma unroll
    for (int a = 0; a < kRowsAhead; ++a) {
      const int r = r0 + kSlicedWaves * a;
      const unsigned char *src = phib + (size_t)words[r < nrows ? r : r0] * rowbytes;
#pragma unroll
      for (int q = 0; q < NP; ++q) {
        const int u = q * 64 + lane;
        v[a][q] = u < upr - 1 ? *reinterpret_cast<const D2 *>(src + (size_t)u * 16) : D2{0.0, 0.0};
      }
    }
#pragma unroll
    for (int a = 0; a < kRowsAhead; ++a) {
      const int r = r0 + kSlicedWaves * a;
#pragma unroll
      for (int q = 0; q < NP; ++q) {
        const int u = q * 64 + lane;
        if (r < nrows && u < upr) *reinterpret_cast<D2 *>(table + r * pitch + u * 16) = v[a][q];
      }
    }
  }
  if (tid < kHotTailBytes / 8) reinterpret_cast<double *>(table + nrows * pitch)[tid] = 0.0;
}

template <int KMAX, int UB = kSliceUnits>
__device__ __forceinline__ int hot_token(const ZParams &p, const int K, const unsigned char *hrow, const unsigned char *trow, const int id0) {
  constexpr int NS = (KMAX + kSliceTopics - 1) / kSliceTopics;
  double sum = 0.0, ck[NS];
  static_for<0, NS>([&](auto sidx) {
    constexpr int s = decltype(sidx)::value;
#pragma unroll
    for (int b = 0; b < kSliceUnits / UB; ++b) {
      D2 ph[UB], th[UB];
#pragma unroll
      for (int u = 0; u < UB; ++u)
        if (s * kSliceTopics + 2 * (b * UB + u) + 1 < KMAX) {
          ph[u] = lds_d2(hrow + s * (kSliceTopics * 8) + (b * UB + u) * 16);
          th[u] = lds_d2(trow + s * (kSliceTopics * 8) + (b * UB + u) * 16);
        }
#pragma unroll
      for (int u = 0; u < UB; ++u)
        if (s * kSliceTopics + 2 * (b * UB + u) + 1 < KMAX) {
          sum += th[u].a * ph[u].a;
          sum += th[u].b * ph[u].b;
        }
      asm volatile("" : "+v"(sum) : : "memory");
    }
    ck[s] = sum;
  });
  const uint64_t gtok = (uint64_t)(p.tok_base + id0);
  const double t0 = z_uniform(gtok, p.iteration, p.seed) * sum;
  const double delta = (sum * (double)K) * 0x1p-51 * p.margin_scale;
  int gsel = NS;
  static_for<0, NS>([&](auto sidx) {
    constexpr int s = NS - 1 - decltype(sidx)::value;
    if (t0 - ck[s] < -delta) gsel = s;
  });
  bool undecided = gsel == NS;
  if (undecided) gsel = 0;
  double s = 0.0;
  static_for<0, NS - 1>([&](auto sidx) {
    constexpr int q = decltype(sidx)::value;
    if (gsel == q + 1) s = ck[q];
  });
  undecided |= fabs(t0 - s) <= delta;
  int ahead = 0;
  {
// ... 162 lines not shown
```

ldagroupedgibbssampler_amd/native.py:

```python
import ctypes as C

import numpy as np

from . import _lib

OK = 0
ERR_NEGATIVE_COUNT, ERR_INVALID_TOPIC, ERR_RNG_EXHAUSTED, ERR_BAD_ARG = 1, 2, 3, 4
ERR_HIP, ERR_STATE, ERR_UNSUPPORTED, ERR_INVARIANT = 5, 6, 7, 8
FLAG_PARANOID, FLAG_SAVE_PHI_MEAN, FLAG_PCGS, FLAG_COLLAPSED, FLAG_POLYAURN, FLAG_SPALIAS, FLAG_LIGHTPCLDA = 1, 2, 4, 8, 16, 32, 64
FLAG_POLYAURN_SPARSE = 128
FLAG_LIGHTCOLLAPSED = 256
FLAG_NZVSSPALIAS = 512
FLAG_ADLDA = 1024
FLAG_LIGHTPCLDAW2 = 2048
SCHEME_FLAGS = {"ggs": 0, "pcgs": FLAG_PCGS, "collapsed": FLAG_COLLAPSED, "polyaurn": FLAG_POLYAURN, "spalias": FLAG_SPALIAS, "lightpclda": FLAG_LIGHTPCLDA,
                "polyaurn_sparse": FLAG_POLYAURN_SPARSE, "lightcollapsed": FLAG_LIGHTCOLLAPSED, "nzvsspalias": FLAG_NZVSSPALIAS, "adlda": FLAG_ADLDA}
PURPOSE_Z, PURPOSE_THETA, PURPOSE_PHI, PURPOSE_INIT_PHI = 1, 2, 3, 4
TOP_KINDS = {"top": 0, "relevance": 1, "distinctive": 2, "salient": 3, "k1": 4}
TOP_WORDS_MAX = 128
TOPIC_DIAGNOSTIC_NAMES = ("tokens", "document_entropy", "word-length", "coherence", "uniform_dist", "corpus_dist", "eff_num_words", "token-doc-diff",
                          "rank_1_docs", "allocation_ratio", "allocation_count")
TOPIC_SCORE_ROWS = tuple(x for x in TOPIC_DIAGNOSTIC_NAMES if x != "word-length")
TOPIC_WORD_SCORE_ROWS = ("coherence", "uniform_dist", "corpus_dist", "token-doc-diff")

# ... 326 lines not shown
        self._chk(self._L.ggs_log_posterior(self._h, C.byref(a), C.byref(b)))
        return a.value, b.value

    def min_doc_distances(self, other=None):
        out = np.empty(self.D, np.float64)
        if other is None:
            op, n = None, 0
        else:
            other = np.ascontiguousarray(other, np.float64)
            if other.ndim != 2 or other.shape[1] != self.K:
                raise ValueError("other must be [n][K]")
            op, n = _dp(other), other.shape[0]
        self._chk(self._L.ggs_min_doc_distances(self._h, op, n, _dp(out)))
        return out

    def min_topic_distance(self):
        v = C.c_double()
        self._chk(self._L.ggs_min_topic_distance(self._h, C.byref(v)))
        return v.value

    def top_words(self, kind, n, lam=0.6, scores=False):
        idx = np.empty((self.K, int(n)), np.int32)
        sc = np.empty((self.K, int(n)), np.float64) if scores else None
        self._chk(self._L.ggs_top_words(self._h, _top_kind(kind), int(n), float(lam), _ip(idx), _dp(sc) if scores else None))
        return (idx, sc) if scores else idx

    def top_words_phases(self, kind, n, lam=0.6, element_chain=False):
        ms = np.zeros(4, np.float64)
        self._chk(self._L.ggs_debug_top_words_phases(self._h, _top_kind(kind), int(n), float(lam), int(bool(element_chain)), _dp(ms)))
        return dict(zip(("mass_k", "total", "words", "select_merge"), ms.tolist()))

    def topic_doc_statistics(self, n, idx=None, clogc_in=None):
        n = int(n)
        if idx is not None:
            idx = np.ascontiguousarray(idx, np.int32)
            if idx.shape != (self.K, n):
                raise ValueError("idx must be [K][n]")
        if clogc_in is not None:
            clogc_in = np.ascontiguousarray(clogc_in, np.float64)
            if clogc_in.shape != (self.K,):
                raise ValueError("clogc_in must be [K]")
        m = max(n, 0)
        codoc, stats, clogc = np.empty((self.K, m, m), np.int32), np.empty((self.K, 9), np.int32), np.empty(self.K, np.float64)
        self._chk(self._L.ggs_topic_doc_statistics(self._h, n, _ip(idx) if idx is not None else None, _dp(clogc_in) if clogc_in is not None else None,
                                                   _ip(codoc), _ip(stats), _dp(clogc)))
        return codoc, stats, clogc

    def topic_scores(self, n, idx, codoc, doc_stats, clogc, word_scores=False):
        n = int(n)
        m = max(n, 0)
        idx, codoc = np.ascontiguousarray(idx, np.int32), np.ascontiguousarray(codoc, np.int32)
        doc_stats, clogc = np.ascontiguousarray(doc_stats, np.int32), np.ascontiguousarray(clogc, np.float64)
        if idx.shape != (self.K, m) or codoc.shape != (self.K, m, m) or doc_stats.shape != (self.K, 9) or clogc.shape != (self.K,):
            raise ValueError("idx [K][n], codoc [K][n][n], doc_stats [K][9], clogc [K]")
        ts = np.empty((len(TOPIC_SCORE_ROWS), self.K), np.float64)
        ws = np.empty((len(TOPIC_WORD_SCORE_ROWS), self.K, m), np.float64) if word_scores else None
        self._chk(self._L.ggs_topic_scores(self._h, n, _ip(idx), _ip(codoc), _ip(doc_stats), _dp(clogc), _dp(ts), _dp(ws) if word_scores else None))
        return (ts, ws) if word_scores else ts

    def topic_diagnostics(self, n, alphabet=None):
        idx = self.top_words("top", n)
        codoc, stats, clogc = self.topic_doc_statistics(n, idx)
        ts, ws = self.topic_scores(n, idx, codoc, stats, clogc, word_scores=True)
        return TopicDiagnostics(idx, codoc, stats, clogc, ts, ws, alphabet)

    def topic_diagnostics_phases(self, n):
        ms = np.zeros(7, np.float64)
        self._chk(self._L.ggs_debug_topic_diagnostics_phases(self._h, int(n), _dp(ms)))
        return dict(zip(("membership", "document_pass", "column_statistics", "clogc_chain", "totals", "sort_and_sorted_chains", "small_scores"), ms.tolist()))

    def set_test_corpus(self, doc_ptr, tokens, doc_base=0):
        doc_ptr = np.ascontiguousarray(doc_ptr, np.int64)
        tokens = np.ascontiguousarray(tokens, np.int32)
        self._test_docs = doc_ptr.size - 1
        self._chk(self._L.ggs_set_test_corpus(self._h, self._test_docs, doc_ptr.ctypes.data_as(C.POINTER(C.c_int64)),
                                              tokens.ctypes.data_as(C.POINTER(C.c_int32)), int(doc_base)))

    def heldout_log_likelihood(self, num_particles=100):
        doc_ll = np.zeros(getattr(self, "_test_docs", 0), np.float64)
        tot = C.c_double()
        self._chk(self._L.ggs_heldout_log_likelihood(self._h, int(num_particles), doc_ll.ctypes.data_as(C.POINTER(C.c_double)), C.byref(tot)))
        return tot.value, doc_ll

    def launch_info(self):
        c, l, b, nh, zp = C.c_int64(), C.c_int32(), C.c_int32(), C.c_int32(), C.c_int32()
        self._chk(self._L.ggs_get_launch_info(self._h, C.byref(c), C.byref(l), C.byref(b)))
        self._chk(self._L.ggs_get_num_hot_words(self._h, C.byref(nh)))
        self._chk(self._L.ggs_get_z_parts(self._h, C.byref(zp)))
        zk, zf, zc = C.c_int32(), C.c_int32(), C.c_int32()
        self._chk(self._L.ggs_get_z_form(self._h, C.byref(zk), C.byref(zf), C.byref(zc)))
        wt, ww, wd = C.c_int32(), C.c_int32(), C.c_int32()
        self._chk(self._L.ggs_get_warm_tiers(self._h, C.byref(wt), C.byref(ww), C.byref(wd)))
        return {"num_chunks": c.value, "lds_bytes_z": l.value, "docs_per_block_theta": b.value, "num_hot": nh.value, "z_parts": zp.value,
                "warm_tiers": wt.value, "num_warm": ww.value, "warm_docs_per_chunk": wd.value,
                "z_kernel": Z_KERNEL_NAMES.get(zk.value, str(zk.value)) + (" + z_warm_kernel (%d tiers)" % wt.value if wt.value else ""), "z_form": {0: "n/a", 1: "split", 2: "fused"}.get(zf.value, str(zf.value)),
                "z_form_calibrated": bool(zc.value)}


Z_KERNEL_NAMES = {0: "z_kernel (whole-row tiles)", 1: "z_sliced_kernel + z_hot_kernel (score registers)", 2: "z_stream1_kernel (one pass)",
                  3: "z_stream_kernel (two passes)", 4: "pcgs_sliced_kernel (lane per document)", 5: "pcgs_wave_kernel (wave per document)",
                  6: "spalias_wave_kernel (wave per document)", 7: "lightpc_wave_kernel (wave per document)",
                  8: "polyaurn_sparse_wave_kernel (wave per document)", 9: "lightcollapsed_wave_kernel (wave per document)",
                  10: "nzvs_wave_kernel (wave per document)", 11: "adlda_wave_kernel (wave per document)", 12: "lightpcw2_wave_kernel (wave per document)"}


class GGSGroup:

    @classmethod
    def adopt(cls, handles):
        self = cls.__new__(cls)
        self._L = _lib.load()
        n = len(handles)
        self._arr = (C.c_void_p * n)(*[h._h for h in handles])
        self.handles, self._owns = list(handles), False
        self._chk(self._L.ggs_group_adopt(self._arr, n))
        return self

    def __init__(self, num_topics, num_types, alpha, beta, seed, device_ids, flags=0, phi_burn_in=0, phi_mean_thin=1, alias_poisson_threshold=0):
        self._L = _lib.load()
        self._owns = True
        _lib.share_rccl_with_torch()
        cfg, keep = _make_config(num_topics, num_types, alpha, beta, seed, 0, flags, phi_burn_in, phi_mean_thin, alias_poisson_threshold)
        n = len(device_ids)
        devs = (C.c_int32 * n)(*[int(d) for d in device_ids])
        self._arr = (C.c_void_p * n)()
        rc = self._L.ggs_group_create(C.byref(cfg), n, devs, self._arr)
        if rc:
            raise GGSError(rc, "ggs_group_create failed")
        self.handles = [GGSHandle(num_topics, num_types, alpha, beta, seed, _adopt=C.c_void_p(self._arr[i])) for i in range(n)]

    def _chk(self, rc):
        if rc:
            msgs = [self._L.ggs_last_error(h._h).decode() for h in self.handles]
            raise GGSError(rc, next((m for m in msgs if m), ""))

    def set_z(self, z_list, redraw_phi=True):
        zs = [np.ascontiguousarray(z, np.int32) for z in z_list]
        ptrs = (C.POINTER(C.c_int32) * len(zs))(*[_ip(z) for z in zs])
        self._chk(self._L.ggs_group_set_z(self._arr, len(zs), ptrs, int(bool(redraw_phi))))

    def sweep(self, n=1):
        self._chk(self._L.ggs_group_sweep(self._arr, len(self.handles), int(n)))

    def gather_counts(self):
        self._chk(self._L.ggs_group_gather_counts(self._arr, len(self.handles)))

    def close(self):
        if getattr(self, "handles", None):
            if getattr(self, "_owns", True):
                for h in self.handles:
                    h._h = None
                self._L.ggs_group_destroy(self._arr, len(self.handles))
            self.handles = []

    def __del__(self):
        try:
            self.close()
        except Exception:
            pass


def debug_philox(ctr, key, device_id=0):
    L = _lib.load()
    ctr = np.ascontiguousarray(ctr, np.uint32).reshape(-1, 4)
    key = np.ascontiguousarray(key, np.uint32).reshape(-1, 2)
    out = np.empty_like(ctr)
# ... 189 lines not shown
```

Measured before the change: 17480.

## Load the last eight topics from a compact fp32 tail array instead of a ring slice

For topic counts whose padded width leaves exactly eight topics past a 32-topic slice boundary (e.g. K=100), the phi normalisation kernels now also write those last eight topics into a separate compact per-word fp32 tail array. A new cold-chunk z path uses it: it streams one fewer full ring slice per token and reads the tail as two 16-byte vector loads, prefetched one chunk ahead. The aim is to cut wasted bandwidth and latency from mostly-padding slices. The cost is extra device memory, a duplicated store in every phi writer, and a new specialised code path.

New measurement: 17640, median of 6. No clear change (+0.9%).

```diff
diff --git a/include/ggs_hip.h b/include/ggs_hip.h
--- a/include/ggs_hip.h
+++ b/include/ggs_hip.h
@@ -144,6 +144,7 @@
 int ggs_get_warm_tiers(ggs_handle *h, int32_t *tiers, int32_t *warm_words, int32_t *docs_per_chunk);
 int ggs_get_z_parts(ggs_handle *h, int32_t *parts);
 int ggs_get_z_form(ggs_handle *h, int32_t *kernel, int32_t *form, int32_t *calibrated);
+int ggs_debug_get_phi32(ggs_handle *h, int32_t which, float *out, int32_t *rows, int32_t *cols);
 int ggs_debug_philox(int32_t device_id, int64_t n, const uint32_t *ctr , const uint32_t *key , uint32_t *out );
 int ggs_debug_math(int32_t device_id, int32_t op , int64_t n, const double *x, const double *y, double *out);
 int ggs_debug_draw(int32_t device_id, int32_t kind , uint64_t seed, uint32_t iteration,
diff --git a/ldagroupedgibbssampler_amd/_lib.py b/ldagroupedgibbssampler_amd/_lib.py
--- a/ldagroupedgibbssampler_amd/_lib.py
+++ b/ldagroupedgibbssampler_amd/_lib.py
@@ -104,6 +104,7 @@
     "ggs_get_z_parts": (C.c_int, [_vp, _ip]),
     "ggs_get_z_form": (C.c_int, [_vp, _ip, _ip, _ip]),
     "ggs_get_warm_tiers": (C.c_int, [_vp, _ip, _ip, _ip]),
+    "ggs_debug_get_phi32": (C.c_int, [_vp, C.c_int32, C.POINTER(C.c_float), _ip, _ip]),
     "ggs_attach_exchange": (C.c_int, [_vp, C.c_int32, C.c_int32, C.POINTER(GGSExchangeOps)]),
     "ggs_rccl_unique_id": (C.c_int, [_vp]),
     "ggs_attach_rccl": (C.c_int, [_vp, C.c_int32, C.c_int32, _vp]),
diff --git a/ldagroupedgibbssampler_amd/csrc/ggs_api.hip b/ldagroupedgibbssampler_amd/csrc/ggs_api.hip
--- a/ldagroupedgibbssampler_amd/csrc/ggs_api.hip
+++ b/ldagroupedgibbssampler_amd/csrc/ggs_api.hip
@@ -82,6 +82,8 @@
   bool two_rows = false;
   KernelLaunch cold, hot, warm;
   bool f32 = false;
+  bool tail32 = false;
+  int32_t tail_off32 = 0;
   bool split = true, split_forced = false;
   int32_t wave_lds = 0, ring_base = 0, hot_wave_lds = 0, warm_wave_lds = 0, hot_pitch = 0, Kp32 = 0;
   int32_t hot_cap = 0, warm_cap = 0, warm_docs = 0;
@@ -341,6 +343,13 @@
   return GGS_OK;
 }
 
+Phi32Out phi32_out(const ggs_handle *h) {
+  Phi32Out o{};
+  o.phiT32 = h->d_phiT32; o.Kp32 = h->plan.Kp32;
+  if (h->d_phiT32 && h->plan.tail32) { o.tail = h->d_phiT32 + (size_t)h->plan.tail_off32 * kTailTopics; o.tail_k0 = sliced_kmax(h->K) - kTailTopics; }
+  return o;
+}
+
 template <typename T>
 int dev_alloc(ggs_handle *h, T **p, size_t count) {
   void **slot = reinterpret_cast<void **>(p);
@@ -670,7 +679,7 @@
 }
 int phi_apply_priors(ggs_handle *h) {
   hipLaunchKernelGGL(phi_apply_priors_kernel, dim3(grid_for((int64_t)h->K * h->V, 256, 2)), dim3(256), 0, h->stream, h->d_phiT, h->d_pr_mask, h->pr_pitch, h->K,
-                     h->Kp, h->V, h->d_phiT32, h->plan.Kp32);
+                     h->Kp, h->V, phi32_out(h));
   HIP_TRY(h, hipGetLastError());
   h->alias_stale = true;
   return GGS_OK;
@@ -757,7 +766,7 @@
     if ((rc = phi_slice_poisson(h, initial, cnt, cnt_pitch, Ks, k0, out, out_pitch, 0, h->sum_nseg, true)) || (rc = phi_slice_poisson_totals(h, Ks, tot, n_k)))
       return rc;
     hipLaunchKernelGGL(phi_normalise_polyaurn_kernel, dim3(grid_for((int64_t)Ks * h->V, 256, 2)), dim3(256), 0, h->stream, out, tot, Ks, out_pitch, h->V,
-                       phi_mean, out == h->d_phiT ? h->d_phiT32 : nullptr, h->plan.Kp32);
+                       phi_mean, out == h->d_phiT ? phi32_out(h) : Phi32Out{});
     HIP_TRY(h, hipGetLastError());
     return GGS_OK;
   }
@@ -766,13 +775,13 @@
     return rc;
   if (vs_phi(h, initial))
     hipLaunchKernelGGL(phi_normalise_polyaurn_kernel, dim3(grid_for((int64_t)Ks * h->V, 256, 2)), dim3(256), 0, h->stream, out, tot, Ks, out_pitch, h->V,
-                       static_cast<double *>(nullptr), out == h->d_phiT ? h->d_phiT32 : nullptr, h->plan.Kp32);
+                       static_cast<double *>(nullptr), out == h->d_phiT ? phi32_out(h) : Phi32Out{});
   else if (conditional_phi(h, initial))
     hipLaunchKernelGGL(phi_normalise_conditional_kernel, dim3(grid_for((int64_t)Ks * h->V, 256, 2)), dim3(256), 0, h->stream, out, tot, h->d_pr_sum_phi, Ks,
-                       out_pitch, h->V, phi_mean, out == h->d_phiT ? h->d_phiT32 : nullptr, h->plan.Kp32);
+                       out_pitch, h->V, phi_mean, out == h->d_phiT ? phi32_out(h) : Phi32Out{});
   else
     hipLaunchKernelGGL(phi_normalise_kernel, dim3(grid_for((int64_t)Ks * h->V, 256, 2)), dim3(256), 0, h->stream, out, tot, Ks, out_pitch, h->V, phi_mean,
-                       out == h->d_phiT ? h->d_phiT32 : nullptr, h->plan.Kp32);
+                       out == h->d_phiT ? phi32_out(h) : Phi32Out{});
   HIP_TRY(h, hipGetLastError());
   return GGS_OK;
 }
@@ -826,7 +835,7 @@
   rp.all0 = h->d_phi_all0; rp.all1 = h->d_phi_all1; rp.krank = h->d_krank; rp.kcol = h->d_kcol; rp.phiT = h->d_phiT;
   rp.phi_mean = accumulate_mean ? h->d_phi_mean : nullptr;
   rp.c0 = (int64_t)half0_elems(h); rp.c1 = (int64_t)half1_elems(h); rp.K = h->K; rp.Kp = h->Kp; rp.V = h->V; rp.Ksm = h->Ksm; rp.v_split = h->v_split;
-  rp.phiT32 = h->d_phiT32; rp.Kp32 = h->plan.Kp32; rp.sum_phi = h->d_pr_sum_phi;
+  rp.o32 = phi32_out(h); rp.sum_phi = h->d_pr_sum_phi;
   if (vs_phi(h, initial)) {
     rp.phi_mean = nullptr;
     hipLaunchKernelGGL(vs_mask_gathered_kernel, dim3(grid_for((int64_t)h->V * h->vs_pitch, 256)), dim3(256), 0, h->stream, rp, h->d_vs_mask, h->vs_pitch);
@@ -1025,6 +1034,10 @@
     } else if (sliced) {
       pl.f32 = !kn.phi64.is(1);
       pl.Kp32 = round_up(K, kSlice32Topics);
+      const int64_t tail_off = ((int64_t)V * pl.Kp32 * 4 + kPhiTailPadBytes) / (kTailTopics * 4);
+      pl.tail32 = pl.f32 && sliced_tail_class(sliced_kmax(K));
+      if (pl.tail32 && tail_off > INT32_MAX) return GGS_ERR_UNSUPPORTED;
+      pl.tail_off32 = pl.tail32 ? (int32_t)tail_off : 0;
       pl.ring_base = sliced_ring_base(K); pl.wave_lds = sliced_wave_lds(K); pl.hot_pitch = table_row_pitch(K);
       pl.hot_wave_lds = hot_wave_lds(K); pl.warm_wave_lds = warm_wave_lds(K);
       if (kn.split.set) { pl.split = kn.split.v != 0; pl.split_forced = kn.split.v == 2; }
@@ -1200,7 +1213,7 @@
   zp.ht_pack = reinterpret_cast<const int4 *>(h->d_ht_pack); zp.h_docs = h->d_h_docs;
   zp.wt_pack = reinterpret_cast<const int4 *>(h->d_wt_pack); zp.w_docs = h->d_w_docs; zp.warm_words = h->d_warm_words;
   zp.warm_meta = h->d_warm_meta; zp.warm_tiers = h->warm_tiers; zp.warm_rows = pl.warm_cap;
-  zp.phiT32 = h->d_phiT32; zp.Kp32 = pl.Kp32; zp.replays = h->d_replays; zp.margin_scale32 = h->margin_scale32;
+  zp.phiT32 = h->d_phiT32; zp.Kp32 = pl.Kp32; zp.tail_off32 = pl.tail_off32; zp.replays = h->d_replays; zp.margin_scale32 = h->margin_scale32;
   void *args[] = {&zp};
   if (!pl.sliced()) {
     if (c1 < 0) c1 = h->C;
@@ -1675,7 +1688,8 @@
     return bail(rc);
   if ((h->flags & GGS_FLAG_SAVE_PHI_MEAN) && (rc = dev_alloc_zeroed(h, &h->d_phi_mean, kv))) return bail(rc);
   if (h->plan.sliced() && h->plan.f32) {
-    if ((rc = dev_alloc_zeroed(h, &h->d_phiT32, (size_t)h->V * h->plan.Kp32 + kPhiTailPadBytes / 4))) return bail(rc);
+    if ((rc = dev_alloc_zeroed(h, &h->d_phiT32, (size_t)h->V * h->plan.Kp32 + kPhiTailPadBytes / 4 + (h->plan.tail32 ? (size_t)h->V * kTailTopics : 0))))
+      return bail(rc);
     if (kn.replays.is(1) && (rc = dev_alloc_zeroed(h, &h->d_replays, 1))) return bail(rc);
   }
   if (h->exact_sum && ((rc = dev_alloc(h, &h->d_sum_pref, ((size_t)h->sum_nseg + 1) * h->K)) ||
@@ -2380,7 +2394,7 @@
   if ((rc = ensure_scratch(h, kv * sizeof(double)))) return rc;
   HIP_TRY(h, hipMemcpyAsync(h->d_scratch, phi, kv * sizeof(double), hipMemcpyHostToDevice, h->stream));
   hipLaunchKernelGGL(phi_to_phiT_kernel, dim3(grid_for((int64_t)kv, 256)), dim3(256), 0, h->stream, static_cast<const double *>(h->d_scratch),
-                     h->d_phiT, h->K, h->Kp, h->V, h->d_phiT32, h->plan.Kp32);
+                     h->d_phiT, h->K, h->Kp, h->V, phi32_out(h));
   HIP_TRY(h, hipGetLastError());
   if (h->d_phi_mean) HIP_TRY(h, hipMemsetAsync(h->d_phi_mean, 0, kv * sizeof(double), h->stream));
   h->alias_stale = true;
@@ -3234,6 +3248,22 @@
   if (kernel) *kernel = own ? own : pcgs_family(h->scheme) ? (h->pcgs_wave ? 5 : 4) : h->plan.kernel;
   if (form) *form = h->plan.sliced() ? (splittable && h->z_split ? 1 : 2) : 0;
   if (calibrated) *calibrated = (splittable && h->z_split_tried && !h->plan.split_forced && h->plan.split) ? 1 : 0;
+  return GGS_OK;
+}
+
+int ggs_debug_get_phi32(ggs_handle *h, int32_t which, float *out, int32_t *rows, int32_t *cols) {
+  if (!h || which < 0 || which > 1) return GGS_ERR_BAD_ARG;
+  int rc = bind_device(h);
+  if (rc) return rc;
+  const Phi32Out o = phi32_out(h);
+  const float *src = which ? o.tail : o.phiT32;
+  const int32_t c = !src ? 0 : which ? kTailTopics : o.Kp32;
+  if (rows) *rows = src ? h->V : 0;
+  if (cols) *cols = c;
+  if (src && out) {
+    HIP_TRY(h, hipStreamSynchronize(h->stream));
+    HIP_TRY(h, hipMemcpy(out, src, (size_t)h->V * c * sizeof(float), hipMemcpyDeviceToHost));
+  }
   return GGS_OK;
 }
 
diff --git a/ldagroupedgibbssampler_amd/csrc/ggs_kernels.hpp b/ldagroupedgibbssampler_amd/csrc/ggs_kernels.hpp
--- a/ldagroupedgibbssampler_amd/csrc/ggs_kernels.hpp
+++ b/ldagroupedgibbssampler_amd/csrc/ggs_kernels.hpp
@@ -504,11 +504,23 @@
 __global__ __launch_bounds__(64) void phi_gamma_vs_kernel(PhiGammaParams p) { phi_gamma_body<kDrawVS>(p); }
 
 __device__ __forceinline__ float phi32_of(const double x) { return (x >= 0.0 && x <= 1.0) ? (float)x : __builtin_nanf(""); }
+struct Phi32Out {
+  float *phiT32 = nullptr;
+  int32_t Kp32 = 0;
+  float *tail = nullptr;
+  int32_t tail_k0 = 0;
+  __device__ __forceinline__ void store(const int v, const int k, const double x) const {
+    if (!phiT32) return;
+    const float f = phi32_of(x);
+    phiT32[(size_t)v * Kp32 + k] = f;
+    if (tail && k >= tail_k0) tail[(size_t)v * 8 + (k - tail_k0)] = f;
+  }
+};
 
 enum PhiNorm { kPhiDirichlet, kPhiPolyaurn, kPhiConditional, kPhiVS };
 template <int MODE>
-__device__ __forceinline__ void phi_normalise_body(double *phiT, const double *tot, int32_t K, int32_t Kp, int32_t V, double *phi_mean, float *phiT32,
-                                                   int32_t Kp32, const double *sum_phi = nullptr) {
+__device__ __forceinline__ void phi_normalise_body(double *phiT, const double *tot, int32_t K, int32_t Kp, int32_t V, double *phi_mean,
+                                                   const Phi32Out &o32, const double *sum_phi = nullptr) {
   __builtin_amdgcn_s_setprio(3);
   const int64_t n = (int64_t)V * K;
   const int64_t stride = (int64_t)gridDim.x * blockDim.x;
@@ -527,24 +539,24 @@
       if (x <= 0) x = kJavaMinValue;
       phiT[(size_t)v * Kp + k] = x;
     }
-    if (phiT32) phiT32[(size_t)v * Kp32 + k] = phi32_of(x);
+    o32.store(v, k, x);
     if (phi_mean) phi_mean[i] += x;
   }
 }
 __global__ __launch_bounds__(256) void phi_normalise_kernel(double *phiT, const double *tot, int32_t K, int32_t Kp, int32_t V,
-                                                            double *phi_mean , float *phiT32 , int32_t Kp32) {
-  phi_normalise_body<kPhiDirichlet>(phiT, tot, K, Kp, V, phi_mean, phiT32, Kp32);
+                                                            double *phi_mean , Phi32Out o32) {
+  phi_normalise_body<kPhiDirichlet>(phiT, tot, K, Kp, V, phi_mean, o32);
 }
 __global__ __launch_bounds__(256) void phi_normalise_polyaurn_kernel(double *phiT, const double *tot, int32_t K, int32_t Kp, int32_t V, double *phi_mean,
-                                                                     float *phiT32, int32_t Kp32) {
-  phi_normalise_body<kPhiPolyaurn>(phiT, tot, K, Kp, V, phi_mean, phiT32, Kp32);
+                                                                     Phi32Out o32) {
+  phi_normalise_body<kPhiPolyaurn>(phiT, tot, K, Kp, V, phi_mean, o32);
 }
 __global__ __launch_bounds__(256) void phi_normalise_conditional_kernel(double *phiT, const double *tot, const double *sum_phi, int32_t K, int32_t Kp, int32_t V,
-                                                                        double *phi_mean, float *phiT32, int32_t Kp32) {
-  phi_normalise_body<kPhiConditional>(phiT, tot, K, Kp, V, phi_mean, phiT32, Kp32, sum_phi);
+                                                                        double *phi_mean, Phi32Out o32) {
+  phi_normalise_body<kPhiConditional>(phiT, tot, K, Kp, V, phi_mean, o32, sum_phi);
 }
 __global__ __launch_bounds__(256) void phi_apply_priors_kernel(double *phiT, const uint32_t *zero_mask, int32_t mask_pitch, int32_t K, int32_t Kp, int32_t V,
-                                                               float *phiT32, int32_t Kp32) {
+                                                               Phi32Out o32) {
   const int64_t n = (int64_t)V * K;
   const int64_t stride = (int64_t)gridDim.x * blockDim.x;
   for (int64_t i = (int64_t)blockIdx.x * blockDim.x + threadIdx.x; i < n; i += stride) {
@@ -552,7 +564,7 @@
     const double prior = ((zero_mask[(size_t)v * mask_pitch + (k >> 5)] >> (k & 31)) & 1u) ? 0.0 : 1.0;
     const double x = phiT[(size_t)v * Kp + k] * prior;
     phiT[(size_t)v * Kp + k] = x;
-    if (phiT32) phiT32[(size_t)v * Kp32 + k] = phi32_of(x);
+    o32.store(v, k, x);
   }
 }
 
@@ -562,8 +574,7 @@
   double *phiT, *phi_mean;
   int64_t c0, c1;
   int32_t K, Kp, V, Ksm, v_split;
-  float *phiT32;
-  int32_t Kp32;
+  Phi32Out o32;
   const double *sum_phi;
 };
 template <int MODE>
@@ -589,7 +600,7 @@
       if (x <= 0) x = kJavaMinValue;
     }
     p.phiT[(size_t)v * p.Kp + k] = x;
-    if (p.phiT32) p.phiT32[(size_t)v * p.Kp32 + k] = phi32_of(x);
+    p.o32.store(v, k, x);
     if (p.phi_mean) p.phi_mean[i] += x;
   }
 }
@@ -640,14 +651,14 @@
     phi[i] = (scale == 1.0) ? x : x / scale;
   }
 }
-__global__ __launch_bounds__(256) void phi_to_phiT_kernel(const double *phi, double *phiT, int32_t K, int32_t Kp, int32_t V, float *phiT32, int32_t Kp32) {
+__global__ __launch_bounds__(256) void phi_to_phiT_kernel(const double *phi, double *phiT, int32_t K, int32_t Kp, int32_t V, Phi32Out o32) {
   const int64_t n = (int64_t)V * K;
   const int64_t stride = (int64_t)gridDim.x * blockDim.x;
   for (int64_t i = (int64_t)blockIdx.x * blockDim.x + threadIdx.x; i < n; i += stride) {
     const int v = (int)(i / K), k = (int)(i - (int64_t)v * K);
     const double x = phi[(size_t)k * V + v];
     phiT[(size_t)v * Kp + k] = x;
-    if (phiT32) phiT32[(size_t)v * Kp32 + k] = phi32_of(x);
+    o32.store(v, k, x);
   }
 }
 
diff --git a/ldagroupedgibbssampler_amd/csrc/ggs_z_kernel.hpp b/ldagroupedgibbssampler_amd/csrc/ggs_z_kernel.hpp
--- a/ldagroupedgibbssampler_amd/csrc/ggs_z_kernel.hpp
+++ b/ldagroupedgibbssampler_amd/csrc/ggs_z_kernel.hpp
@@ -61,6 +61,7 @@
   int32_t warm_tiers, warm_rows;
   const float *phiT32;
   int32_t Kp32;
+  int32_t tail_off32;
   unsigned long long *replays;
   double margin_scale32;
 };
diff --git a/ldagroupedgibbssampler_amd/csrc/ggs_z_sliced.hpp b/ldagroupedgibbssampler_amd/csrc/ggs_z_sliced.hpp
--- a/ldagroupedgibbssampler_amd/csrc/ggs_z_sliced.hpp
+++ b/ldagroupedgibbssampler_amd/csrc/ggs_z_sliced.hpp
@@ -36,6 +36,8 @@
 }
 
 constexpr int sliced_kmax(const int K) { return (K + 7) / 8 * 8; }
+constexpr int kTailTopics = 8, kTailMaxTopics = 104;
+constexpr bool sliced_tail_class(const int kmax) { return kmax % kSlice32Topics == kTailTopics && kmax > kSlice32Topics && kmax <= kTailMaxTopics; }
 constexpr int sliced_slices(const int K) { return (sliced_kmax(K) + kSliceTopics - 1) / kSliceTopics; }
 constexpr int sliced_ring_base(const int K) { return round_up(imax(kChunkDocs * sliced_kmax(K) * 8, sliced_slices(K) * 128), 256); }
 constexpr int sliced_wave_lds(const int K) { return sliced_ring_base(K) + kRingSlots * kSliceBytes; }
@@ -264,6 +266,235 @@
   }
 }
 
+template <int KMAX>
+__device__ __forceinline__ void cold_chunks32_tail(const ZParams &p, unsigned char *thb, unsigned char *ring, const int64_t wid, const int64_t stride, const int lane) {
+  static_assert(sliced_tail_class(KMAX), "the last 8 topics from phi32_tail, not from a ring slice");
+  constexpr int NS = KMAX / kSlice32Topics;
+  constexpr int kAhead = NS < kRingSlots - 1 ? NS : kRingSlots - 1;
+  constexpr int NT = (KMAX + 63) / 64;
+  constexpr int kThetaRow = KMAX * 4;
+  const int K = p.K;
+  const unsigned char *phib = reinterpret_cast<const unsigned char *>(p.phiT32);
+  const unsigned char *tailb = phib + (size_t)(unsigned)p.tail_off32 * (kTailTopics * 4);
+  const size_t rowbytes = (size_t)p.Kp32 * 4;
+  const const_i32_t *cdocs = (const const_i32_t *)p.c_docs;
+  double *prod = reinterpret_cast<double *>(thb + kChunkDocs * kThetaRow);
+  const int lrow = lane >> 3, lslot = lane & 7;
+  const unsigned char *my_row = ring + lane * 128;
+  const int rot = lane >> 1;
+  const float mscale = (float)p.margin_scale32;
+
+  auto load_theta = [&](const int d0, const int d1, double (&tv)[kChunkDocs][NT]) {
+    const double *t0 = p.theta + (size_t)d0 * K, *t1 = p.theta + (size_t)d1 * K;
+#pragma unroll
+    for (int t = 0; t < NT; ++t) {
+      tv[0][t] = (t * 64 + lane < K) ? t0[t * 64 + lane] : 0.0;
+      tv[1][t] = (t * 64 + lane < K) ? t1[t * 64 + lane] : 0.0;
+    }
+  };
+  auto stage_theta = [&](const double (&tv)[kChunkDocs][NT]) {
+#pragma unroll
+    for (int r = 0; r < kChunkDocs; ++r)
+#pragma unroll
+      for (int t = 0; t < NT; ++t)
+        if (t * 64 + lane < KMAX) reinterpret_cast<float *>(thb + r * kThetaRow)[t * 64 + lane] = phi32_of(tv[r][t]);
+  };
+  auto row_addresses = [&](const int w, const unsigned char *(&ra)[8]) {
+#pragma unroll
+    for (int m = 0; m < 8; ++m) {
+      const int row = 8 * m + lrow;
+      const int wm = __shfl(w, row) & ((1 << kSlotShift) - 1);
+      ra[m] = phib + (size_t)wm * rowbytes + (size_t)(((lslot - (row >> 1)) & 7) << 4);
+    }
+  };
+  auto issue_slice = [&](auto sc, const int slot, const unsigned char *const (&ra)[8]) {
+    constexpr int s = decltype(sc)::value;
+#pragma unroll
+    for (int m = 0; m < 8; ++m)
+      __builtin_amdgcn_global_load_lds((glb_cvoid_t *)ra[m], (lds_void_t *)(ring + slot * kSliceBytes + m * 1024 - s * 128), 16, s * 128, 0);
+  };
+  auto load_tail = [&](const int w, f4_t (&tl)[2]) {
+    const f4_t *src = reinterpret_cast<const f4_t *>(tailb + (size_t)(w & ((1 << kSlotShift) - 1)) * (kTailTopics * 4));
+    tl[0] = src[0];
+    tl[1] = src[1];
+  };
+  auto finish = [&](const float (&a)[KMAX], const int64_t c, const int idx, const int ip, const int w) {
+    const uint64_t gtok = (uint64_t)(p.tok_base + idx);
+    const double U = z_uniform(gtok, p.iteration, p.seed);
+    const float A = a[KMAX - 1];
+    const float t0 = (float)(U * (double)A);
+    const float delta = ((float)(2 * K + 8) * 0x1p-24f * A) * mscale;
+    const f2_t nt0 = {-t0, -t0};
+    int cnt = 0;
+    float m = t0;
+    bool live = true;
+#pragma unroll
+    for (int kb = 0; kb < KMAX; kb += 16) {
+      if (live) {
+        uint32_t bits = 0;
+        float dl = 0.0f;
+#pragma unroll
+        for (int j = 0; j < 16; j += 2)
+          if (kb + j < KMAX) {
+            const f2_t d = f2_t{a[kb + j], a[kb + j + 1]} + nt0;
+            bits = __builtin_amdgcn_alignbit(bits, __float_as_uint(d.x), 31);
+            bits = __builtin_amdgcn_alignbit(bits, __float_as_uint(d.y), 31);
+            m = fminf(m, fminf(fabsf(d.x), fabsf(d.y)));
+            dl = d.y;
+          }
+        cnt += __popc(bits);
+        live = __any(dl < 0.0f);
+      }
+    }
+    int new_topic = cnt;
+    const bool undecided = idx >= 0 && !(A >= 0x1p-60f && A <= 0x1.fffffep127f && m > delta && cnt < K);
+    uint64_t pend = __ballot(undecided);
+    if (pend) {
+      if (p.replays && lane == 0) atomicAdd(p.replays, (unsigned long long)__popcll(pend));
+      const int slot = (int)((unsigned)w >> kSlotShift);
+      const int d0 = cdocs[2 * c], d1 = cdocs[2 * c + 1];
+      while (pend) {
+        const int L = (int)__builtin_ctzll(pend);
+        pend &= pend - 1;
+        const int wl = __shfl(w, L) & ((1 << kSlotShift) - 1), dl = __shfl(slot, L) ? d1 : d0;
+        const double UL = __shfl(U, L);
+        const double *th = p.theta + (size_t)dl * K, *ph = p.phiT + (size_t)wl * p.Kp;
+        for (int k = lane; k < K; k += 64) prod[k] = th[k] * ph[k];
+        asm volatile("s_waitcnt lgkmcnt(0)" ::: "memory");
+        double sum = 0.0;
+        for (int k = 0; k < K; ++k) sum += prod[k];
+        double sample = UL * sum;
+        int nt = -1;
+        while (sample > 0.0) {
+          ++nt;
+          if (nt >= K) break;
+          sample -= prod[nt];
+        }
+        if (nt < 0 || nt >= K) {
+          if (lane == L) atomicOr(p.status, ST_INVALID_TOPIC);
+          nt = nt < 0 ? 0 : K - 1;
+        }
+        if (lane == L) new_topic = nt;
+        asm volatile("s_waitcnt lgkmcnt(0)" ::: "memory");
+      }
+    }
+    if (idx < 0) return;
+    p.z[idx] = new_topic;
+    p.zw[ip] = new_topic;
+    const int word = w & ((1 << kSlotShift) - 1);
+    if (p.cnt_send) __hip_atomic_fetch_add(&p.cnt_send[slice_cell(p.smap, new_topic, word)], 1, __ATOMIC_RELAXED, __HIP_MEMORY_SCOPE_AGENT);
+  };
+
+  const int64_t C = p.num_cold;
+  int64_t c = wid;
+  if (c >= C) return;
+  int w0 = p.ct_tok[c * 64 + lane], id0 = p.ct_idx[c * 64 + lane], ip0 = p.ct_ip[c * 64 + lane];
+  int w1 = 0, id1 = -1, ip1 = 0, w2 = 0, id2 = -1, ip2 = 0;
+  double tv0[kChunkDocs][NT], tv1[kChunkDocs][NT], tv2[kChunkDocs][NT];
+  load_theta(cdocs[2 * c], cdocs[2 * c + 1], tv0);
+  if (c + stride < C) {
+    const int64_t c1 = c + stride;
+    w1 = p.ct_tok[c1 * 64 + lane]; id1 = p.ct_idx[c1 * 64 + lane]; ip1 = p.ct_ip[c1 * 64 + lane];
+    load_theta(cdocs[2 * c1], cdocs[2 * c1 + 1], tv1);
+  } else {
+    load_theta(0, 0, tv1);
+  }
+#pragma unroll
+  for (int r = 0; r < kChunkDocs; ++r)
+#pragma unroll
+    for (int t = 0; t < NT; ++t) tv2[r][t] = 0.0;
+  const unsigned char *ra[8], *ran[8];
+  row_addresses(w0, ra);
+  row_addresses(w1, ran);
+  f4_t tl0[2], tl1[2];
+  load_tail(w0, tl0);
+  int g = 0;
+  static_for<0, kAhead>([&](auto sc) { issue_slice(sc, decltype(sc)::value % kRingSlots, ra); });
+
+  for (;;) {
+    const bool has1 = c + stride < C, has2 = c + 2 * stride < C;
+    g = __builtin_amdgcn_readfirstlane(g);
+    stage_theta(tv0);
+    const unsigned char *trow = thb + ((unsigned)w0 >> kSlotShift) * kThetaRow;
+
+    float a[KMAX];
+    float acc = 0.0f;
+    static_for<0, NS>([&](auto sidx) {
+      constexpr int s = decltype(sidx)::value;
+      const int cur = (g + s) % kRingSlots;
+      const int nxt = (g + s + kAhead) % kRingSlots;
+      if constexpr (s + kAhead < NS) issue_slice(std::integral_constant<int, s + kAhead>{}, nxt, ra);
+      else if (has1) issue_slice(std::integral_constant<int, s + kAhead - NS>{}, nxt, ran);
+      if (has1 || s + kAhead < NS) asm volatile("s_waitcnt vmcnt(%0)" ::"n"(8 * kAhead) : "memory");
+      else asm volatile("s_waitcnt vmcnt(%0)" ::"n"(8 * (NS - 1 - s)) : "memory");
+      {
+        const unsigned char *rb = my_row + cur * kSliceBytes;
+        f4_t ph[kSliceUnits], th[kSliceUnits];
+#pragma unroll
+        for (int u = 0; u < kSliceUnits; ++u)
+          if (s * kSlice32Topics + 4 * u < KMAX) {
+            ph[u] = *reinterpret_cast<const f4_t *>(rb + (((u + rot) & 7) << 4));
+            th[u] = *reinterpret_cast<const f4_t *>(trow + s * (kSlice32Topics * 4) + u * 16);
+          }
+#pragma unroll
+        for (int u = 0; u < kSliceUnits; ++u) {
+          constexpr int k0 = s * kSlice32Topics;
+          const int k = k0 + 4 * u;
+          if (k < KMAX) {
+            const f2_t q0 = f2_t{th[u].x, th[u].y} * f2_t{ph[u].x, ph[u].y};
+            const f2_t q1 = f2_t{th[u].z, th[u].w} * f2_t{ph[u].z, ph[u].w};
+            acc += q0.x; a[k] = acc;
+            acc += q0.y; a[k + 1] = acc;
+            acc += q1.x; a[k + 2] = acc;
+            acc += q1.y; a[k + 3] = acc;
+          }
+        }
+      }
+      asm volatile("s_waitcnt lgkmcnt(0)" ::: "memory");
+    });
+    g = (g + NS) % kRingSlots;
+    {
+      constexpr int k0 = KMAX - kTailTopics;
+      f4_t th[2];
+#pragma unroll
+      for (int u = 0; u < 2; ++u) th[u] = *reinterpret_cast<const f4_t *>(trow + k0 * 4 + u * 16);
+#pragma unroll
+      for (int u = 0; u < 2; ++u) {
+        const int k = k0 + 4 * u;
+        const f2_t q0 = f2_t{th[u].x, th[u].y} * f2_t{tl0[u].x, tl0[u].y};
+        const f2_t q1 = f2_t{th[u].z, th[u].w} * f2_t{tl0[u].z, tl0[u].w};
+        acc += q0.x; a[k] = acc;
+        acc += q0.y; a[k + 1] = acc;
+        acc += q1.x; a[k + 2] = acc;
+        acc += q1.y; a[k + 3] = acc;
+      }
+      load_tail(w1, tl1);
+    }
+
+    if (has2) {
+      const int64_t c2 = c + 2 * stride;
+      w2 = p.ct_tok[c2 * 64 + lane]; id2 = p.ct_idx[c2 * 64 + lane]; ip2 = p.ct_ip[c2 * 64 + lane];
+      load_theta(cdocs[2 * c2], cdocs[2 * c2 + 1], tv2);
+    } else {
+      w2 = 0; id2 = -1; ip2 = 0;
+    }
+
+    finish(a, c, id0, ip0, w0);
+    if (!has1) break;
+    c += stride;
+    w0 = w1; id0 = id1; ip0 = ip1;
+    w1 = w2; id1 = id2; ip1 = ip2;
+    tl0[0] = tl1[0]; tl0[1] = tl1[1];
+#pragma unroll
+    for (int r = 0; r < kChunkDocs; ++r)
+#pragma unroll
+      for (int t = 0; t < NT; ++t) { tv0[r][t] = tv1[r][t]; tv1[r][t] = tv2[r][t]; }
+#pragma unroll
+    for (int m = 0; m < 8; ++m) ra[m] = ran[m];
+    row_addresses(w1, ran);
+  }
+}
+
 template <int KMAX, bool F32>
 __device__ __forceinline__ void z_sliced_body(const ZParams &p) {
   constexpr int NS = (KMAX + kSliceTopics - 1) / kSliceTopics;
@@ -508,6 +739,7 @@
 #pragma unroll 1
   for (int phase = 0; phase < 2; ++phase) {
     if ((phase ^ wave) & 1) hot_chunks();
+    else if constexpr (F32 && sliced_tail_class(KMAX)) cold_chunks32_tail<KMAX>(p, thb, ring, wid, stride, lane);
     else if constexpr (F32) cold_chunks32<KMAX>(p, thb, ring, wid, stride, lane);
     else cold_chunks();
   }
diff --git a/ldagroupedgibbssampler_amd/native.py b/ldagroupedgibbssampler_amd/native.py
--- a/ldagroupedgibbssampler_amd/native.py
+++ b/ldagroupedgibbssampler_amd/native.py
@@ -432,6 +432,15 @@
         self._chk(self._L.ggs_heldout_log_likelihood(self._h, int(num_particles), doc_ll.ctypes.data_as(C.POINTER(C.c_double)), C.byref(tot)))
         return tot.value, doc_ll
 
+    def debug_phi32(self, which=0):
+        r, c = C.c_int32(), C.c_int32()
+        self._chk(self._L.ggs_debug_get_phi32(self._h, int(which), None, C.byref(r), C.byref(c)))
+        if r.value == 0 or c.value == 0:
+            return None
+        out = np.empty((r.value, c.value), np.float32)
+        self._chk(self._L.ggs_debug_get_phi32(self._h, int(which), out.ctypes.data_as(C.POINTER(C.c_float)), C.byref(r), C.byref(c)))
+        return out
+
     def launch_info(self):
         c, l, b, nh, zp = C.c_int64(), C.c_int32(), C.c_int32(), C.c_int32(), C.c_int32()
         self._chk(self._L.ggs_get_launch_info(self._h, C.byref(c), C.byref(l), C.byref(b)))
```
